# JiuTongBro/MultiView_Inpaint

Hardware: AMD Instinct MI355X
Metric: Mpix/s fwd+bwd @1.5M Gauss 1080p (higher is better)
Workload: dtype f32; 1 GPU; rasterizer-with-depth fwd+bwd, one 1920x1080 view per GPU per step, N=1500000 Gaussians, sh_degree 3 (BASELINE.json configs[2] size, SURVEY.md §8d scene); gaussians=1500000, visible=1312313, num_rendered_D=14779663, tiles=8160, tile_list_max=2266, parallelism=views x1

## Files before the change

### include/mvi_raster.h

```cpp
#ifndef MVI_RASTER_H
#define MVI_RASTER_H

#include <stddef.h>
#include <stdint.h>

#ifdef __cplusplus
extern "C" {
#endif

#define MVI_OK 0
#define MVI_EINVAL (-1)
#define MVI_EHIP (-2)
#define MVI_ENOMEM (-3)

#define MVI_TILE 16

typedef struct mvi_raster_settings {
    int32_t image_height;
    int32_t image_width;
    float tanfovx;
    float tanfovy;
    float scale_modifier;
    int32_t sh_degree;
    int32_t prefiltered;
    const float* bg;
    const float* viewmatrix;
    const float* projmatrix;
    const float* campos;
} mvi_raster_settings;

size_t mvi_raster_geom_bytes(int32_t P);
size_t mvi_raster_image_bytes(int32_t image_width, int32_t image_height);
size_t mvi_raster_binning_bytes(int64_t num_rendered, int32_t image_width, int32_t image_height);

int mvi_raster_forward_geom(const mvi_raster_settings* s, int32_t P, int32_t M,
                            const float* means3D, const float* shs, const float* colors_precomp,
                            const float* opacities, const float* scales, const float* rotations,
                            const float* cov3D_precomp, void* geom, size_t geom_bytes,
                            int32_t* radii, int64_t* num_rendered_host, void* stream);

int mvi_raster_forward_render(const mvi_raster_settings* s, int32_t P, int64_t num_rendered,
                              const int32_t* radii, void* geom, size_t geom_bytes, void* binning, size_t binning_bytes,
                              void* image, size_t image_bytes, float* out_color, float* out_depth,
                              void* stream);
int mvi_raster_forward_render_prepare(const mvi_raster_settings* s, int32_t P, int64_t num_rendered,
                                      const int32_t* radii, void* geom, size_t geom_bytes, void* binning,
                                      size_t binning_bytes, void* image, size_t image_bytes, float* out_color,
                                      float* out_depth, float* grad_rows_scratch, void* stream);

int mvi_raster_backward(const mvi_raster_settings* s, int32_t P, int32_t M, int64_t num_rendered,
                        const float* means3D, const float* shs, const float* colors_precomp,
                        const float* scales, const float* rotations, const float* cov3D_precomp,
                        const int32_t* radii, const void* geom, const void* binning,
                        const void* image, const float* dL_dout_color, float* dL_dmeans3D,
                        float* dL_dmeans2D, float* dL_dopacity, float* dL_dshs, float* dL_dcolors,
                        float* dL_dscales, float* dL_drotations, float* dL_dcov3D,
                        float* grad_rows_scratch, int32_t grad_rows_prezeroed, void* stream);

int mvi_raster_forward_geom_raw(const mvi_raster_settings* s, int32_t P, int32_t M, const float* xyz,
                                const float* features_dc, const float* features_rest, const float* raw_opacity,
                                const float* raw_scaling, const float* raw_rotation, void* geom, size_t geom_bytes,
                                int32_t* radii, int64_t* num_rendered_host, void* stream);
int mvi_raster_backward_raw(const mvi_raster_settings* s, int32_t P, int32_t M, int64_t num_rendered, const float* xyz,
                            const float* features_dc, const float* features_rest, const float* raw_opacity,
                            const float* raw_scaling, const float* raw_rotation, const int32_t* radii, const void* geom,
                            const void* binning, const void* image, const float* dL_dout_color, float* dL_dxyz,
                            float* dL_dmeans2D, float* dL_draw_opacity, float* dL_dfeatures_dc, float* dL_dfeatures_rest,
                            float* dL_draw_scaling, float* dL_draw_rotation, float* grad_rows_scratch, 
                            int32_t grad_rows_prezeroed, void* stream);
int mvi_raster_backward_raw_factor(const mvi_raster_settings* s, int32_t P, int32_t M, int64_t num_rendered, const float* xyz,
                                   const float* features_dc, const float* features_rest, const float* raw_opacity,
                                   const float* raw_scaling, const float* raw_rotation, const int32_t* radii, const void* geom,
                                   const void* binning, const void* image, const float* dL_dout_color, float* dL_dxyz,
                                   float* dL_dmeans2D, float* dL_draw_opacity, float* dL_dsh_color_factor,
                                   float* dL_draw_scaling, float* dL_draw_rotation, float* grad_rows_scratch,
                                   int32_t grad_rows_prezeroed, void* stream);

int mvi_raster_sh_backward_views(int32_t P, int32_t M, int32_t sh_degree, int32_t n_views, const float* means3D,
                                 const float* campos, int64_t campos_stride, const float* dL_dcolors,
                                 int64_t colors_view_stride, float* dL_dshs, void* stream);

int mvi_raster_mark_visible(int32_t P, const float* means3D, const float* viewmatrix,
                            const float* projmatrix, uint8_t* visible, void* stream);

int mvi_raster_backward_render(const mvi_raster_settings* s, int32_t P, int64_t num_rendered, const int32_t* radii,
                               const void* geom, const void* binning, const void* image, const float* dL_dout_color,
                               float* grad_rows_scratch, float* dL_dcolor_factor, int32_t sh_input,
                               int32_t grad_rows_prezeroed, void* stream);
int mvi_raster_backward_geom(const mvi_raster_settings* s, int32_t P, int32_t M, const float* means3D, const float* shs,
                             const float* colors_precomp, const float* scales, const float* rotations,
                             const float* cov3D_precomp, const int32_t* radii, const void* geom,
                             const float* grad_rows_scratch, float* dL_dmeans3D, float* dL_dmeans2D, float* dL_dopacity,
                             float* dL_dshs, float* dL_dcolors, float* dL_dscales, float* dL_drotations, float* dL_dcov3D,
                             void* stream);

int mvi_raster_backward_geom_range(const mvi_raster_settings* s, int32_t P, int32_t M, int32_t first, int32_t count,
                                   const float* means3D, const float* shs, const float* colors_precomp, const float* scales,
                                   const float* rotations, const float* cov3D_precomp, const int32_t* radii, const void* geom,
                                   const float* grad_rows_scratch, float* dL_dmeans3D, float* dL_dmeans2D, float* dL_dopacity,
                                   float* dL_dshs, float* dL_dcolors, float* dL_dscales, float* dL_drotations, float* dL_dcov3D,
                                   void* stream);

typedef struct mvi_raster_views {
    const float* depths;
    const float* means2D;
    const float* cov3D_a;
    const float* cov3D_b;
    const float* conic_opacity;
    const float* rgbd;
    const uint32_t* tiles_touched;
    const uint8_t* clamped;
    const void* tile_ids_sorted;
    const uint32_t* point_list;
    const uint32_t* ranges;
    const float* final_T;
    const uint32_t* n_contrib;
    int32_t tile_id_bytes;
    const uint8_t* grad_support;
} mvi_raster_views;
int mvi_raster_get_views(int32_t P, int64_t num_rendered, int32_t image_width, int32_t image_height,
                         const void* geom, const void* binning, const void* image,
                         mvi_raster_views* out);
int mvi_raster_materialize_tile_ids(int32_t P, int64_t num_rendered, int32_t image_width, int32_t image_height,
                                    void* binning, const void* image, void* stream);

#define MVI_RASTER_NSTAGES 8
int mvi_raster_timing_enable(int enable);
int mvi_raster_timing_enable_stages(uint32_t stage_mask);
int mvi_raster_timing_read(float* ms_sum_host, int32_t* calls_host);
const char* mvi_raster_stage_name(int stage);

int mvi_raster_color_mode(int deferred);
int mvi_raster_resolve_colors(const mvi_raster_settings* s, int32_t P, void* geom, size_t geom_bytes, void* stream);

int mvi_raster_binning_version(int version);
int mvi_raster_backward_mode(int dense);
int mvi_raster_dev_stamps(int pass, void* device_buffer);
int mvi_raster_dev_wave_sum9(const float* in, float* out, int n_waves, void* stream);

const char* mvi_raster_last_error(void);
const char* mvi_version(void);

#ifdef __cplusplus
}
#endif
#endif
```

### multiview_inpaint_amd/_lib.py

```python
import ctypes as C
import os
import re

_HERE = os.path.dirname(os.path.abspath(__file__))
LIB_PATH = os.environ.get("MVI_HIP_LIB") or os.path.join(_HERE, "csrc", "libmvi_hip.so")
LIB_OVERRIDDEN = bool(os.environ.get("MVI_HIP_LIB"))
if LIB_OVERRIDDEN:
    import sys as _sys
    _sys.stderr.write(f"[mvi] MVI_HIP_LIB is set: every kernel comes from {LIB_PATH}, not from the in-tree build\n")
INCLUDE_DIR = os.path.normpath(os.path.join(_HERE, "..", "include"))


class RasterSettings(C.Structure):
    _fields_ = [
        ("image_height", C.c_int32), ("image_width", C.c_int32),
        ("tanfovx", C.c_float), ("tanfovy", C.c_float), ("scale_modifier", C.c_float),
        ("sh_degree", C.c_int32), ("prefiltered", C.c_int32),
        ("bg", C.c_void_p), ("viewmatrix", C.c_void_p), ("projmatrix", C.c_void_p), ("campos", C.c_void_p),
    ]


class RasterViews(C.Structure):
    _fields_ = [(n, C.c_void_p) for n in (
        "depths", "means2D", "cov3D_a", "cov3D_b", "conic_opacity", "rgbd", "tiles_touched", "clamped",
        "tile_ids_sorted", "point_list", "ranges", "final_T", "n_contrib")] + [("tile_id_bytes", C.c_int32),
                                                                                   ("grad_support", C.c_void_p)]


class AdamGroup(C.Structure):
    _fields_ = [("param", C.c_void_p), ("grad", C.c_void_p), ("exp_avg", C.c_void_p), ("exp_avg_sq", C.c_void_p),
                ("n", C.c_int64), ("lr", C.c_float)]


class CompactTensor(C.Structure):
    _fields_ = [("in_", C.c_void_p), ("out", C.c_void_p), ("width", C.c_int32), ("packed_stride", C.c_int32)]


def declared_symbols():
    names = []
    for fn in sorted(os.listdir(INCLUDE_DIR)):
        if fn.endswith(".h"):
            src = open(os.path.join(INCLUDE_DIR, fn)).read()
            src = re.sub(r"/\*.*?\*/", "", src, flags=re.S)
            names += re.findall(r"\b(mvi_[a-z0-9_]+)\s*\(", src)
    return sorted(set(names))


def raster_source_digest():
    import hashlib
    h = hashlib.sha1()
    d = os.path.join(_HERE, "csrc")
    for fn in sorted(os.listdir(d)):
        if fn.startswith("raster_") and fn.endswith((".hip", ".h")):
            h.update(fn.encode())
            h.update(open(os.path.join(d, fn), "rb").read())
    return h.hexdigest()[:16]


_lib = None


def lib():
    global _lib
    if _lib is not None:
        return _lib
    if not os.path.exists(LIB_PATH):
        raise RuntimeError(
            f"{LIB_PATH} is missing: the HIP extension is not built. Run `python -m multiview_inpaint_amd.build` "
            "(hipcc --offload-arch=gfx950). There is no CPU or PyTorch fallback for this path.")
    L = C.CDLL(LIB_PATH)
    missing = [s for s in declared_symbols() if not hasattr(L, s)]
    if missing:
        raise RuntimeError(f"{LIB_PATH} does not export {missing}; rebuild it")
    vp, i32, i64, sz = C.c_void_p, C.c_int32, C.c_int64, C.c_size_t
    L.mvi_raster_last_error.restype = C.c_char_p
    L.mvi_version.restype = C.c_char_p
    L.mvi_raster_geom_bytes.restype = sz
    L.mvi_raster_geom_bytes.argtypes = [i32]
    L.mvi_raster_image_bytes.restype = sz
    L.mvi_raster_image_bytes.argtypes = [i32, i32]
    L.mvi_raster_binning_bytes.restype = sz
    L.mvi_raster_binning_bytes.argtypes = [i64, i32, i32]
    L.mvi_raster_forward_geom.restype = C.c_int
    L.mvi_raster_forward_geom.argtypes = [C.POINTER(RasterSettings), i32, i32] + [vp] * 7 + [vp, sz, vp, C.POINTER(i64), vp]
    L.mvi_raster_forward_render.restype = C.c_int
    L.mvi_raster_forward_render.argtypes = [C.POINTER(RasterSettings), i32, i64, vp, vp, sz, vp, sz, vp, sz, vp, vp, vp]
    L.mvi_raster_forward_render_prepare.restype = C.c_int
    L.mvi_raster_forward_render_prepare.argtypes = [C.POINTER(RasterSettings), i32, i64, vp, vp, sz, vp, sz, vp, sz, vp, vp, vp, vp]
    L.mvi_raster_backward.restype = C.c_int
    L.mvi_raster_backward.argtypes = [C.POINTER(RasterSettings), i32, i32, i64] + [vp] * 20 + [i32, vp]
    L.mvi_raster_backward_render.restype = C.c_int
    L.mvi_raster_backward_render.argtypes = [C.POINTER(RasterSettings), i32, i64] + [vp] * 7 + [i32, i32, vp]
    L.mvi_raster_backward_geom.restype = C.c_int
    L.mvi_raster_backward_geom.argtypes = [C.POINTER(RasterSettings), i32, i32] + [vp] * 18
    L.mvi_raster_backward_geom_range.restype = C.c_int
    L.mvi_raster_backward_geom_range.argtypes = [C.POINTER(RasterSettings), i32, i32, i32, i32] + [vp] * 18
    L.mvi_raster_forward_geom_raw.restype = C.c_int
    L.mvi_raster_forward_geom_raw.argtypes = [C.POINTER(RasterSettings), i32, i32] + [vp] * 6 + [vp, sz, vp, C.POINTER(i64), vp]
    L.mvi_raster_backward_raw.restype = C.c_int
    L.mvi_raster_backward_raw.argtypes = [C.POINTER(RasterSettings), i32, i32, i64] + [vp] * 19 + [i32, vp]
    L.mvi_raster_backward_raw_factor.restype = C.c_int
    L.mvi_raster_backward_raw_factor.argtypes = [C.POINTER(RasterSettings), i32, i32, i64] + [vp] * 18 + [i32, vp]
    L.mvi_raster_sh_backward_views.restype = C.c_int
    L.mvi_raster_sh_backward_views.argtypes = [i32, i32, i32, i32, vp, vp, i64, vp, i64, vp, vp]
    L.mvi_raster_mark_visible.restype = C.c_int
    L.mvi_raster_mark_visible.argtypes = [i32, vp, vp, vp, vp, vp]
    L.mvi_raster_get_views.restype = C.c_int
    L.mvi_raster_get_views.argtypes = [i32, i64, i32, i32, vp, vp, vp, C.POINTER(RasterViews)]
    L.mvi_raster_materialize_tile_ids.restype = C.c_int
    L.mvi_raster_materialize_tile_ids.argtypes = [i32, i64, i32, i32, vp, vp, vp]
    L.mvi_raster_timing_enable.restype = C.c_int
    L.mvi_raster_timing_enable.argtypes = [C.c_int]
    L.mvi_raster_timing_enable_stages.restype = C.c_int
    L.mvi_raster_timing_enable_stages.argtypes = [C.c_uint32]
    L.mvi_raster_timing_read.restype = C.c_int
    L.mvi_raster_timing_read.argtypes = [C.POINTER(C.c_float), C.POINTER(C.c_int32)]
    L.mvi_raster_stage_name.restype = C.c_char_p
    L.mvi_raster_stage_name.argtypes = [C.c_int]
    L.mvi_raster_binning_version.restype = C.c_int
    L.mvi_raster_binning_version.argtypes = [C.c_int]
    L.mvi_raster_backward_mode.restype = C.c_int
    L.mvi_raster_backward_mode.argtypes = [C.c_int]
    L.mvi_raster_color_mode.restype = C.c_int
    L.mvi_raster_color_mode.argtypes = [C.c_int]
    L.mvi_raster_resolve_colors.restype = C.c_int
    L.mvi_raster_resolve_colors.argtypes = [C.POINTER(RasterSettings), i32, vp, sz, vp]
    L.mvi_raster_dev_stamps.restype = C.c_int
    L.mvi_raster_dev_stamps.argtypes = [C.c_int, vp]
    L.mvi_raster_dev_wave_sum9.restype = C.c_int
    L.mvi_raster_dev_wave_sum9.argtypes = [vp, vp, C.c_int, vp]
    _bind_unet_ops(L)
    _bind_train_ops(L)
    _bind_box_region(L)
    _lib = L
    return L


def _bind_unet_ops(L):
    try:
        from . import _unet_ops_bind
    except ImportError:
        return
    _unet_ops_bind.bind(L)


def _bind_train_ops(L):
    vp, i32, sz, f32 = C.c_void_p, C.c_int32, C.c_size_t, C.c_float
    L.mvi_photometric_loss_workspace_bytes.restype = sz
    L.mvi_photometric_loss_workspace_bytes.argtypes = [i32, i32]
    L.mvi_photometric_loss.restype = C.c_int
    L.mvi_photometric_loss.argtypes = [vp, vp, vp, i32, i32, f32, f32, vp, vp, vp, sz, vp]
    L.mvi_photometric_loss_stats.restype = C.c_int
    L.mvi_photometric_loss_stats.argtypes = [vp, vp, vp, i32, i32, vp, vp, sz, vp]
    L.mvi_photometric_loss_grad2.restype = C.c_int
    L.mvi_photometric_loss_grad2.argtypes = [vp, vp, vp, i32, i32, vp, vp, vp, sz, vp]
    L.mvi_train_last_error.restype = C.c_char_p
    L.mvi_knn3_mean_dist2.restype = C.c_int
    L.mvi_knn3_mean_dist2.argtypes = [vp, i32, vp, vp]
    L.mvi_adam_step.restype = C.c_int
    L.mvi_adam_step.argtypes = [C.POINTER(AdamGroup), i32, C.c_double, C.c_double, C.c_double, i32, vp]
    L.mvi_compact_workspace_bytes.restype = sz
    L.mvi_compact_workspace_bytes.argtypes = [i32]
    L.mvi_compact_plan.restype = C.c_int
    L.mvi_compact_plan.argtypes = [vp, i32, vp, sz, vp, vp]
    L.mvi_compact_gather.restype = C.c_int
    L.mvi_compact_gather.argtypes = [C.POINTER(CompactTensor), i32, i32, C.c_uint32, vp, vp]
    L.mvi_support_pack_bits.restype = C.c_int
    L.mvi_support_pack_bits.argtypes = [vp, i32, vp, vp]
    L.mvi_support_union_bits.restype = C.c_int
    L.mvi_support_union_bits.argtypes = [vp, i32, i32, vp, vp]
    for f in (L.mvi_compact_gather_window, L.mvi_compact_scatter_window):
        f.restype = C.c_int
        f.argtypes = [C.POINTER(CompactTensor), i32, i32, vp, C.c_uint32, C.c_uint32, vp, vp]
    L.mvi_gaussian_activations.restype = C.c_int
    L.mvi_gaussian_activations.argtypes = [i32, i32] + [vp] * 10
    L.mvi_gaussian_activations_backward.restype = C.c_int
    L.mvi_gaussian_activations_backward.argtypes = [i32, i32] + [vp] * 13


def _bind_box_region(L):
    vp, i32, i64 = C.c_void_p, C.c_int32, C.c_int64
    L.mvi_box_region_last_error.restype = C.c_char_p
    L.mvi_mesh_intersect.restype = C.c_int
    L.mvi_mesh_intersect.argtypes = [vp, vp, i64, vp, i32, vp, vp, vp, vp, vp]
    L.mvi_mesh_points_inside.restype = C.c_int
    L.mvi_mesh_points_inside.argtypes = [vp, i64, vp, i32, vp, vp]
    L.mvi_mesh_view_masks.restype = C.c_int
    L.mvi_mesh_view_masks.argtypes = [vp, vp, vp, i32, i32, i32, vp, i32, vp, vp, vp, vp, vp, vp]


def check(rc, what):
    if rc != 0:
        msg = lib().mvi_raster_last_error().decode(errors="replace")
        if rc == -1:
            raise Exception(msg)
        raise RuntimeError(f"{what} failed ({rc}): {msg}")
```

### multiview_inpaint_amd/csrc/raster_api.hip

```cpp
#include <cstdio>
#include <cstdlib>
#include <cstring>
#include <mutex>
#include <vector>

#include "raster_common.h"

static thread_local char g_err[512] = "";
static int g_dense_backward = [] { const char* e = getenv("MVI_RASTER_DENSE_BACKWARD"); return (e && e[0] == '1') ? 1 : 0; }();
static int g_defer_colors = [] { const char* e = getenv("MVI_RASTER_EAGER_COLORS"); return (e && e[0] == '1') ? 0 : 1; }();
namespace {
struct SegmentHint { const void* geom; int32_t P; int64_t segments; uint64_t stamp; };
constexpr int kSegmentHints = 64;
SegmentHint g_seg_hints[kSegmentHints] = {};
uint64_t g_seg_clock = 0;
std::mutex g_seg_mutex;
void remember_segments(const void* geom, int32_t P, int64_t segments) {
    std::lock_guard<std::mutex> lock(g_seg_mutex);
    int slot = 0;
    for (int i = 0; i < kSegmentHints; ++i) {
        if (g_seg_hints[i].geom == geom) { slot = i; break; }
        if (g_seg_hints[i].stamp < g_seg_hints[slot].stamp) slot = i;
    }
    g_seg_hints[slot] = {geom, P, segments, ++g_seg_clock};
}
int64_t recall_segments(const void* geom, int32_t P) {
    std::lock_guard<std::mutex> lock(g_seg_mutex);
    for (int i = 0; i < kSegmentHints; ++i)
        if (g_seg_hints[i].geom == geom && g_seg_hints[i].stamp) return g_seg_hints[i].P == P ? g_seg_hints[i].segments : 0;
    return 0;
}
}

namespace {
struct Rec { int stage; hipEvent_t a, b; };
uint32_t g_timing_mask = 0;
std::vector<Rec> g_recs;
std::vector<hipEvent_t> g_pool;
hipEvent_t g_open[MVI_RASTER_NSTAGES];
hipEvent_t get_event() {
    if (!g_pool.empty()) { hipEvent_t e = g_pool.back(); g_pool.pop_back(); return e; }
    hipEvent_t e; (void)hipEventCreate(&e); return e;
}
}
namespace mvi {
void stage_begin(int stage, hipStream_t st) {
    if (!((g_timing_mask >> stage) & 1u)) return;
    g_open[stage] = get_event();
    (void)hipEventRecord(g_open[stage], st);
}
void stage_end(int stage, hipStream_t st) {
    if (!((g_timing_mask >> stage) & 1u)) return;
    hipEvent_t b = get_event();
    (void)hipEventRecord(b, st);
    g_recs.push_back({stage, g_open[stage], b});
}
}

static int fail(int code, const char* fmt, const char* a = "", long long b = 0, long long c = 0) {
    snprintf(g_err, sizeof(g_err), fmt, a, b, c);
    return code;
}
static int hip_fail(const char* where, hipError_t e) {
    snprintf(g_err, sizeof(g_err), "%s: %s", where, hipGetErrorString(e));
    return MVI_EHIP;
}

static int make_frame(const mvi_raster_settings* s, int P, int M, mvi::Frame& f) {
    if (!s) return fail(MVI_EINVAL, "settings is NULL%s");
    if (s->image_width < 0 || s->image_height < 0 || P < 0)
        return fail(MVI_EINVAL, "negative size%s (P=%lld, W=%lld)", "", P, s->image_width);
    if (s->sh_degree < 0 || s->sh_degree > 3) return fail(MVI_EINVAL, "sh_degree must be 0..3%s (got %lld)", "", s->sh_degree);
    if (!s->bg || !s->viewmatrix || !s->projmatrix || !s->campos)
        return fail(MVI_EINVAL, "bg/viewmatrix/projmatrix/campos must be device pointers%s");
    f.P = P; f.M = M; f.deg = s->sh_degree; f.W = s->image_width; f.H = s->image_height;
    f.gx = (f.W + mvi::kTile - 1) / mvi::kTile;
    f.gy = (f.H + mvi::kTile - 1) / mvi::kTile;
    f.tanfovx = s->tanfovx; f.tanfovy = s->tanfovy;
    f.fx = (float)f.W / (2.0f * s->tanfovx);
    f.fy = (float)f.H / (2.0f * s->tanfovy);
    f.scale_modifier = s->scale_modifier;
    f.view = s->viewmatrix; f.proj = s->projmatrix; f.campos = s->campos; f.bg = s->bg;
    f.bin_v2 = mvi::binning_v2_ok(f.gx, f.gy) ? 1 : 0;
    f.defer_colors = g_defer_colors;
    return MVI_OK;
}

extern "C" {

const char* mvi_raster_last_error(void) { return g_err; }

int mvi_raster_timing_enable(int enable) { g_timing_mask = enable ? (1u << MVI_RASTER_NSTAGES) - 1u : 0u; return MVI_OK; }
int mvi_raster_timing_enable_stages(uint32_t stage_mask) { g_timing_mask = stage_mask & ((1u << MVI_RASTER_NSTAGES) - 1u); return MVI_OK; }
int mvi_raster_timing_read(float* ms_sum, int32_t* calls) {
    if (!ms_sum || !calls) return fail(MVI_EINVAL, "NULL timing outputs%s");
    for (auto& r : g_recs) {
        hipError_t e = hipEventSynchronize(r.b);
        if (e != hipSuccess) return hip_fail("timing sync", e);
        float ms = 0.f;
        (void)hipEventElapsedTime(&ms, r.a, r.b);
        ms_sum[r.stage] += ms;
        calls[r.stage] += 1;
        g_pool.push_back(r.a);
        g_pool.push_back(r.b);
    }
    g_recs.clear();
    return MVI_OK;
}
const char* mvi_raster_stage_name(int i) {
    static const char* n[MVI_RASTER_NSTAGES] = {"preprocess_forward", "scan_block_sums", "duplicate_keys", "radix_sort",
                                                "tile_ranges", "render_forward", "render_backward", "preprocess_backward"};
    return (i >= 0 && i < MVI_RASTER_NSTAGES) ? n[i] : "";
}
int mvi_raster_dev_stamps(int pass, void* device_buffer) { mvi::set_dev_stamps(pass, device_buffer); return MVI_OK; }
int mvi_raster_dev_wave_sum9(const float* in, float* out, int n_waves, void* stream) {
    if (n_waves < 0 || (n_waves > 0 && (!in || !out))) return fail(MVI_EINVAL, "wave_sum9: NULL buffer or negative n_waves%s");
    if (mvi::launch_wave_sum9_probe(in, out, n_waves, (hipStream_t)stream)) return hip_fail("wave_sum9 probe", hipGetLastError());
    return MVI_OK;
}
int mvi_raster_backward_mode(int dense) {
    const int old = g_dense_backward;
    if (dense == 0 || dense == 1) g_dense_backward = dense;
    return old;
}
int mvi_raster_binning_version(int version) { return mvi::set_binning_version(version); }
int mvi_raster_color_mode(int deferred) {
    const int old = g_defer_colors;
    if (deferred == 0 || deferred == 1) g_defer_colors = deferred;
    return old;
}
int mvi_raster_resolve_colors(const mvi_raster_settings* s, int32_t P, void* geom, size_t geom_bytes, void* stream) {
    mvi::Frame f;
    if (int rc = make_frame(s, P, 0, f)) return rc;
    if (P == 0) return MVI_OK;
    if (!geom) return fail(MVI_EINVAL, "geom is NULL%s");
    mvi::GeomView g = mvi::carve_geom(geom, P);
    if (geom_bytes < g.bytes) return fail(MVI_ENOMEM, "geom scratch too small%s", "");
    if (mvi::launch_resolve_colors(f, g, (hipStream_t)stream)) return hip_fail("resolve_colors", hipGetLastError());
    return MVI_OK;
}
const char* mvi_version(void) { return "multiview_inpaint_amd 0.1.0 (gfx950)"; }

size_t mvi_raster_geom_bytes(int32_t P) { return mvi::carve_geom(nullptr, P).bytes; }
size_t mvi_raster_image_bytes(int32_t W, int32_t H) { return mvi::carve_image(nullptr, W, H).bytes; }
size_t mvi_raster_binning_bytes(int64_t D, int32_t W, int32_t H) { return mvi::carve_binning(nullptr, D, W, H).bytes; }

static int forward_geom_impl(const mvi_raster_settings* s, mvi::Frame& f, int32_t P, int32_t M, const float* means3D,
                             const float* shs, const float* colors_precomp, const float* opacities,
                             const float* scales, const float* rotations, const float* cov3D_precomp,
                             void* geom, size_t geom_bytes, int32_t* radii, int64_t* num_rendered_host,
                             void* stream);

int mvi_raster_forward_geom(const mvi_raster_settings* s, int32_t P, int32_t M, const float* means3D,
                            const float* shs, const float* colors_precomp, const float* opacities,
                            const float* scales, const float* rotations, const float* cov3D_precomp,
                            void* geom, size_t geom_bytes, int32_t* radii, int64_t* num_rendered_host,
                            void* stream) {
    mvi::Frame f;
    if (int rc = make_frame(s, P, M, f)) return rc;
    return forward_geom_impl(s, f, P, M, means3D, shs, colors_precomp, opacities, scales, rotations, cov3D_precomp, geom,
                             geom_bytes, radii, num_rendered_host, stream);
}

int mvi_raster_forward_geom_raw(const mvi_raster_settings* s, int32_t P, int32_t M, const float* xyz,
                                const float* features_dc, const float* features_rest, const float* raw_opacity,
                                const float* raw_scaling, const float* raw_rotation, void* geom, size_t geom_bytes,
                                int32_t* radii, int64_t* num_rendered_host, void* stream) {
    mvi::Frame f;
    if (int rc = make_frame(s, P, M, f)) return rc;
    if (P > 0 && (!features_dc || (M > 1 && !features_rest) || !raw_scaling || !raw_rotation))
        return fail(MVI_EINVAL, "NULL raw parameter pointer%s");
    f.raw = 1;
    f.shs_rest = features_rest;
    return forward_geom_impl(s, f, P, M, xyz, features_dc, nullptr, raw_opacity, raw_scaling, raw_rotation, nullptr, geom,
                             geom_bytes, radii, num_rendered_host, stream);
}

static int forward_geom_impl(const mvi_raster_settings* s, mvi::Frame& f, int32_t P, int32_t M, const float* means3D,
                             const float* shs, const float* colors_precomp, const float* opacities,
                             const float* scales, const float* rotations, const float* cov3D_precomp,
                             void* geom, size_t geom_bytes, int32_t* radii, int64_t* num_rendered_host,
                             void* stream) {
    if (!num_rendered_host) return fail(MVI_EINVAL, "num_rendered_host is NULL%s");
    *num_rendered_host = 0;
    if (P == 0) return MVI_OK;
    if ((shs == nullptr) == (colors_precomp == nullptr))
        return fail(MVI_EINVAL, "Please provide excatly one of either SHs or precomputed colors!%s");
    if (((scales == nullptr) || (rotations == nullptr)) == (cov3D_precomp == nullptr))
        return fail(MVI_EINVAL, "Please provide exactly one of either scale/rotation pair or precomputed 3D covariance!%s");
    if (!means3D || !opacities || !geom || !radii) return fail(MVI_EINVAL, "NULL means3D/opacities/geom/radii%s");
    if (shs && M < (s->sh_degree + 1) * (s->sh_degree + 1))
        return fail(MVI_EINVAL, "shs holds %s%lld coefficients per channel, sh_degree needs %lld", "", M,
                    (s->sh_degree + 1) * (s->sh_degree + 1));
    mvi::GeomView g = mvi::carve_geom(geom, P);
    if (geom_bytes < g.bytes) return fail(MVI_ENOMEM, "geom scratch too small%s: %lld < %lld", "", (long long)geom_bytes, (long long)g.bytes);
    hipStream_t st = (hipStream_t)stream;
    {
        mvi::StageTimer tm(mvi::kStPreFwd, st);
        if (mvi::launch_preprocess_forward(f, means3D, shs, colors_precomp, opacities, scales, rotations,
                                           cov3D_precomp, g, radii, st))
            return hip_fail("preprocess_forward", hipGetLastError());
    }
    struct Readback { unsigned long long* host = nullptr; unsigned long long* dev = nullptr; hipEvent_t ev = nullptr; };
    constexpr int kMaxDevices = 64;
    static thread_local Readback readbacks[kMaxDevices];
    hipError_t e;
    int device = -1;
    if ((e = hipGetDevice(&device)) != hipSuccess) return hip_fail("hipGetDevice", e);
    if (device < 0 || device >= kMaxDevices) return fail(MVI_EINVAL, "device index out of range%s: %lld", "", (long long)device);
    Readback& rb = readbacks[device];
    if (!rb.host) {
        unsigned long long* h = nullptr;
        if ((e = hipHostMalloc((void**)&h, 2 * sizeof(unsigned long long), hipHostMallocMapped | hipHostMallocPortable)) != hipSuccess) return hip_fail("hipHostMalloc", e);
        if ((e = hipHostGetDevicePointer((void**)&rb.dev, h, 0)) != hipSuccess) { (void)hipHostFree(h); return hip_fail("hipHostGetDevicePointer", e); }
        if ((e = hipEventCreateWithFlags(&rb.ev, hipEventDisableTiming)) != hipSuccess) { (void)hipHostFree(h); return hip_fail("hipEventCreate", e); }
        rb.host = h;
    }
    unsigned long long* const pinned = rb.host;
    unsigned long long* const pinned_dev = rb.dev;
    const hipEvent_t ev = rb.ev;
    {
        mvi::StageTimer tm(mvi::kStScan, st);
        if (f.bin_v2 ? mvi::launch_binning2_totals(g, P, pinned_dev, st) : mvi::launch_scan_block_sums(g, P, pinned_dev, st))
            return hip_fail("scan_block_sums", hipGetLastError());
    }
    if ((e = hipEventRecord(ev, st)) != hipSuccess) return hip_fail("event record", e);
    if (f.bin_v2 ? mvi::launch_binning2_level1(f, g, st) : mvi::launch_binning_level1(f, g, st))
        return hip_fail("binning level 1", hipGetLastError());
    e = hipEventSynchronize(ev);
    if (e != hipSuccess) return hip_fail("forward_geom sync", e);
    const unsigned long long total = *pinned;
    if (total > 0xFFFFFFFFull)
        return fail(MVI_EINVAL, "num_rendered exceeds the 32-bit pair offsets%s: %lld pairs", "", (long long)total);
    *num_rendered_host = (int64_t)total;
    if (f.bin_v2) remember_segments(geom, P, (int64_t)pinned[1]);
    return MVI_OK;
}

static int forward_render_impl(const mvi_raster_settings* s, int32_t P, int64_t D, const int32_t* radii,
                               void* geom, size_t geom_bytes, void* binning, size_t binning_bytes, void* image,
                               size_t image_bytes, float* out_color, float* out_depth, float* grad_rows_to_zero, void* stream) {
    mvi::Frame f;
    if (int rc = make_frame(s, P, 0, f)) return rc;
    if (!image || !out_color || !out_depth) return fail(MVI_EINVAL, "NULL image/out_color/out_depth%s");
    if (D < 0 || D > 0xFFFFFFFFll) return fail(MVI_EINVAL, "num_rendered out of range%s: %lld", "", D);
    if (D > 0 && (!geom || !binning || !radii)) return fail(MVI_EINVAL, "NULL geom/binning/radii with num_rendered > 0%s");
    mvi::GeomView g = mvi::carve_geom(geom, P);
    mvi::ImageView im = mvi::carve_image(image, f.W, f.H);
    mvi::BinningView b = mvi::carve_binning(binning, D, f.W, f.H);
    if (image_bytes < im.bytes) return fail(MVI_ENOMEM, "image scratch too small%s: %lld < %lld", "", (long long)image_bytes, (long long)im.bytes);
    if (D > 0 && binning_bytes < b.bytes) return fail(MVI_ENOMEM, "binning scratch too small%s: %lld < %lld", "", (long long)binning_bytes, (long long)b.bytes);
    if (D > 0 && geom_bytes < g.bytes) return fail(MVI_ENOMEM, "geom scratch too small%s", "");
    hipStream_t st = (hipStream_t)stream;
    const int64_t segments = recall_segments(geom, P);
    if (f.bin_v2 ? mvi::launch_binning2(f, g, b, im, D, segments, st) : mvi::launch_binning(f, g, b, im, D, st))
        return hip_fail("binning", hipGetLastError());
    {
        mvi::StageTimer tm(mvi::kStRenderFwd, st);
        if (mvi::launch_render_forward(f, g, b, im, D, out_color, out_depth, st, grad_rows_to_zero))
            return hip_fail("render_forward", hipGetLastError());
    }
    return MVI_OK;
}

int mvi_raster_forward_render(const mvi_raster_settings* s, int32_t P, int64_t D, const int32_t* radii,
                              void* geom, size_t geom_bytes, void* binning, size_t binning_bytes, void* image,
                              size_t image_bytes, float* out_color, float* out_depth, void* stream) {
    return forward_render_impl(s, P, D, radii, geom, geom_bytes, binning, binning_bytes, image, image_bytes, out_color, out_depth,
                               nullptr, stream);
}

int mvi_raster_forward_render_prepare(const mvi_raster_settings* s, int32_t P, int64_t D, const int32_t* radii,
                                      void* geom, size_t geom_bytes, void* binning, size_t binning_bytes, void* image,
                                      size_t image_bytes, float* out_color, float* out_depth, float* grad_rows_scratch,
                                      void* stream) {
    return forward_render_impl(s, P, D, radii, geom, geom_bytes, binning, binning_bytes, image, image_bytes, out_color, out_depth,
                               grad_rows_scratch, stream);
}

static int backward_render_impl(mvi::Frame& f, int32_t P, int64_t D, const int32_t* radii, const void* geom, const void* binning,
                                const void* image, const float* dL_dout_color, float* grad_rows, float* dL_dcolor_factor,
                                int sh_input, int rows_prezeroed, void* stream, const mvi::ZeroRegions* zero_outputs = nullptr);
static int backward_impl(mvi::Frame& f, int32_t P, int64_t D, const float* means3D, const float* shs,
                         const float* colors_precomp, const float* scales, const float* rotations,
                         const float* cov3D_precomp, const int32_t* radii, const void* geom, const void* binning,
                         const void* image, const float* dL_dout_color, float* dL_dmeans3D, float* dL_dmeans2D,
                         float* dL_dopacity, float* dL_dshs, float* dL_dcolors, float* dL_dscales, float* dL_drotations,
                         float* dL_dcov3D, float* dL_dconic_scratch, void* stream, mvi::RawBackwardExtra rawx);

int mvi_raster_backward(const mvi_raster_settings* s, int32_t P, int32_t M, int64_t D, const float* means3D,
                        const float* shs, const float* colors_precomp, const float* scales,
                        const float* rotations, const float* cov3D_precomp, const int32_t* radii,
                        const void* geom, const void* binning, const void* image,
                        const float* dL_dout_color, float* dL_dmeans3D, float* dL_dmeans2D,
                        float* dL_dopacity, float* dL_dshs, float* dL_dcolors, float* dL_dscales,
                        float* dL_drotations, float* dL_dcov3D, float* dL_dconic_scratch, int32_t grad_rows_prezeroed,
                        void* stream) {
    mvi::Frame f;
    if (int rc = make_frame(s, P, M, f)) return rc;
    mvi::RawBackwardExtra rawx;
    rawx.rows_prezeroed = grad_rows_prezeroed;
    return backward_impl(f, P, D, means3D, shs, colors_precomp, scales, rotations, cov3D_precomp, radii, geom, binning, image,
                         dL_dout_color, dL_dmeans3D, dL_dmeans2D, dL_dopacity, dL_dshs, dL_dcolors, dL_dscales, dL_drotations,
                         dL_dcov3D, dL_dconic_scratch, stream, rawx);
}

int mvi_raster_backward_raw(const mvi_raster_settings* s, int32_t P, int32_t M, int64_t D, const float* xyz,
                            const float* features_dc, const float* features_rest, const float* raw_opacity,
                            const float* raw_scaling, const float* raw_rotation, const int32_t* radii, const void* geom,
                            const void* binning, const void* image, const float* dL_dout_color, float* dL_dxyz,
                            float* dL_dmeans2D, float* dL_draw_opacity, float* dL_dfeatures_dc, float* dL_dfeatures_rest,
                            float* dL_draw_scaling, float* dL_draw_rotation, float* grad_rows_scratch,
                            int32_t grad_rows_prezeroed, void* stream) {
    mvi::Frame f;
    if (int rc = make_frame(s, P, M, f)) return rc;
    if (P > 0 && (!features_dc || (M > 1 && (!features_rest || !dL_dfeatures_rest)) || !raw_opacity || !dL_dfeatures_dc))
        return fail(MVI_EINVAL, "NULL raw parameter / gradient pointer%s");
    f.raw = 1;
    f.shs_rest = features_rest;
    mvi::RawBackwardExtra rawx;
    rawx.raw_opacity = raw_opacity;
    rawx.dL_dshs_rest = dL_dfeatures_rest;
    rawx.rows_prezeroed = grad_rows_prezeroed;
    return backward_impl(f, P, D, xyz, features_dc, nullptr, raw_scaling, raw_rotation, nullptr, radii, geom, binning, image,
                         dL_dout_color, dL_dxyz, dL_dmeans2D, dL_draw_opacity, dL_dfeatures_dc, nullptr, dL_draw_scaling,
                         dL_draw_rotation, nullptr, grad_rows_scratch, stream, rawx);
}

int mvi_raster_backward_raw_factor(const mvi_raster_settings* s, int32_t P, int32_t M, int64_t D, const float* xyz,
                                   const float* features_dc, const float* features_rest, const float* raw_opacity,
                                   const float* raw_scaling, const float* raw_rotation, const int32_t* radii, const void* geom,
                                   const void* binning, const void* image, const float* dL_dout_color, float* dL_dxyz,
                                   float* dL_dmeans2D, float* dL_draw_opacity, float* dL_dsh_color_factor, float* dL_draw_scaling,
                                   float* dL_draw_rotation, float* grad_rows_scratch, int32_t grad_rows_prezeroed, void* stream) {
    mvi::Frame f;
    if (int rc = make_frame(s, P, M, f)) return rc;
    if (P > 0 && (!features_dc || (M > 1 && !features_rest) || !raw_opacity || !dL_dsh_color_factor))
        return fail(MVI_EINVAL, "NULL raw parameter / colour factor pointer%s");
    f.raw = 1;
    f.shs_rest = features_rest;
    mvi::RawBackwardExtra rawx;
    rawx.raw_opacity = raw_opacity;
    rawx.dL_dshs_rest = nullptr;
    rawx.rows_prezeroed = grad_rows_prezeroed;
    return backward_impl(f, P, D, xyz, features_dc, nullptr, raw_scaling, raw_rotation, nullptr, radii, geom, binning, image,
                         dL_dout_color, dL_dxyz, dL_dmeans2D, dL_draw_opacity, nullptr, dL_dsh_color_factor, dL_draw_scaling,
                         dL_draw_rotation, nullptr, grad_rows_scratch, stream, rawx);
}

static int backward_impl(mvi::Frame& f, int32_t P, int64_t D, const float* means3D, const float* shs,
                         const float* colors_precomp, const float* scales, const float* rotations,
                         const float* cov3D_precomp, const int32_t* radii, const void* geom, const void* binning,
                         const void* image, const float* dL_dout_color, float* dL_dmeans3D, float* dL_dmeans2D,
                         float* dL_dopacity, float* dL_dshs, float* dL_dcolors, float* dL_dscales, float* dL_drotations,
                         float* dL_dcov3D, float* dL_dconic_scratch, void* stream, mvi::RawBackwardExtra rawx) {
    if (P == 0) return MVI_OK;
    if ((shs == nullptr) == (colors_precomp == nullptr))
        return fail(MVI_EINVAL, "Please provide excatly one of either SHs or precomputed colors!%s");
    if (((scales == nullptr) || (rotations == nullptr)) == (cov3D_precomp == nullptr))
        return fail(MVI_EINVAL, "Please provide exactly one of either scale/rotation pair or precomputed 3D covariance!%s");
    if (!means3D || !radii || !geom || !image || !dL_dout_color || !dL_dmeans3D || !dL_dmeans2D || !dL_dopacity ||
        !dL_dconic_scratch)
        return fail(MVI_EINVAL, "NULL required pointer in backward%s");
    if (shs && !dL_dshs && !dL_dcolors)
        return fail(MVI_EINVAL, "dL_dshs and dL_dcolors are both NULL but shs was a forward input%s");
    if (colors_precomp && !dL_dcolors) return fail(MVI_EINVAL, "dL_dcolors is NULL but colors_precomp was a forward input%s");
    if (cov3D_precomp ? !dL_dcov3D : (!dL_dscales || !dL_drotations))
        return fail(MVI_EINVAL, "missing covariance gradient output%s");
    if (D > 0 && !binning) return fail(MVI_EINVAL, "NULL binning with num_rendered > 0%s");
    const bool dense_bwd = g_dense_backward != 0;
    mvi::GeomView g = mvi::carve_geom(const_cast<void*>(geom), P);
    hipStream_t st = (hipStream_t)stream;
    if (!dense_bwd) {
        mvi::ZeroRegions z;
        const size_t n = (size_t)P, Mz = (size_t)f.M;
        z.add(dL_dmeans3D, 3 * n);
        z.add(dL_dmeans2D, 3 * n);
        z.add(dL_dopacity, n);
        if (dL_dcolors) z.add(dL_dcolors, 3 * n);
        if (shs && dL_dshs) z.add(dL_dshs, f.raw ? 3 * n : 3 * Mz * n);
        if (f.raw && rawx.dL_dshs_rest && Mz > 1) z.add(rawx.dL_dshs_rest, (3 * Mz - 3) * n);
        if (cov3D_precomp) z.add(dL_dcov3D, 6 * n);
        else { z.add(dL_dscales, 3 * n); z.add(dL_drotations, 4 * n); }
        if (z.overflow) return fail(MVI_EINVAL, "more gradient outputs than the render backward can zero on the side%s (kMaxZero)");
        if (int rc = backward_render_impl(f, P, D, radii, geom, binning, image, dL_dout_color, dL_dconic_scratch, nullptr, 0,
                                          rawx.rows_prezeroed, stream, &z)) return rc;
        mvi::StageTimer tm(mvi::kStPreBwd, st);
        if (mvi::launch_preprocess_backward_sparse(f, means3D, shs, scales, rotations, cov3D_precomp, g, dL_dconic_scratch,
                                                   dL_dmeans3D, dL_dmeans2D, dL_dopacity, dL_dcolors, dL_dshs, dL_dcov3D,
                                                   dL_dscales, dL_drotations, st, rawx))
            return hip_fail("preprocess_backward (sparse)", hipGetLastError());
        return MVI_OK;
    }
    if (int rc = backward_render_impl(f, P, D, radii, geom, binning, image, dL_dout_color, dL_dconic_scratch, nullptr, 0,
                                      rawx.rows_prezeroed, stream)) return rc;
    mvi::StageTimer tm(mvi::kStPreBwd, st);
    if (mvi::launch_preprocess_backward(f, means3D, shs, scales, rotations, cov3D_precomp, radii, g, dL_dconic_scratch,
                                        dL_dmeans3D, dL_dmeans2D, dL_dopacity, dL_dcolors,
                                        dL_dshs, dL_dcov3D, dL_dscales, dL_drotations, st, rawx))
        return hip_fail("preprocess_backward", hipGetLastError());
    return MVI_OK;
}

static int backward_render_impl(mvi::Frame& f, int32_t P, int64_t D, const int32_t* radii, const void* geom, const void* binning,
                                const void* image, const float* dL_dout_color, float* grad_rows, float* dL_dcolor_factor,
                                int sh_input, int rows_prezeroed, void* stream, const mvi::ZeroRegions* zero_outputs) {
    if (P == 0) return MVI_OK;
    if (!radii || !geom || !image || !dL_dout_color || !grad_rows) return fail(MVI_EINVAL, "NULL required pointer in backward%s");
    if (D > 0 && !binning) return fail(MVI_EINVAL, "NULL binning with num_rendered > 0%s");
    mvi::GeomView g = mvi::carve_geom(const_cast<void*>(geom), P);
    mvi::ImageView im = mvi::carve_image(const_cast<void*>(image), f.W, f.H);
    mvi::BinningView b = mvi::carve_binning(const_cast<void*>(binning), D, f.W, f.H);
    hipStream_t st = (hipStream_t)stream;
    if (!rows_prezeroed) {
        mvi::ZeroRegions z;
        z.add(grad_rows, (size_t)mvi::kGradRow * (size_t)P);
        z.add(g.touched, ((size_t)P + 15) / 16 * 4);
        z.add(g.touched_count, 1);
        if (mvi::launch_zero_regions(z, st)) return hip_fail("zero grad rows", hipGetLastError());
    }
    {
        mvi::StageTimer tm(mvi::kStRenderBwd, st);
        if (mvi::launch_render_backward(f, g, b, im, D, dL_dout_color, grad_rows, st, zero_outputs))
            return hip_fail("render_backward", hipGetLastError());
    }
    if (dL_dcolor_factor && mvi::launch_color_factors(P, radii, grad_rows, sh_input ? g.clamped : nullptr, dL_dcolor_factor, st))
        return hip_fail("color_factors", hipGetLastError());
    return MVI_OK;
}

int mvi_raster_backward_render(const mvi_raster_settings* s, int32_t P, int64_t D, const int32_t* radii, const void* geom,
                               const void* binning, const void* image, const float* dL_dout_color, float* grad_rows_scratch,
                               float* dL_dcolor_factor, int32_t sh_input, int32_t grad_rows_prezeroed, void* stream) {
    mvi::Frame f;
    if (int rc = make_frame(s, P, 0, f)) return rc;
    return backward_render_impl(f, P, D, radii, geom, binning, image, dL_dout_color, grad_rows_scratch, dL_dcolor_factor,
                                sh_input, grad_rows_prezeroed, stream);
}

static int backward_geom_range_impl(const mvi_raster_settings* s, int32_t P, int32_t M, int32_t first, int32_t count,
                                    const float* means3D, const float* shs, const float* colors_precomp, const float* scales,
                                    const float* rotations, const float* cov3D_precomp, const int32_t* radii, const void* geom,
                                    const float* grad_rows_scratch, float* dL_dmeans3D, float* dL_dmeans2D, float* dL_dopacity,
                                    float* dL_dshs, float* dL_dcolors, float* dL_dscales, float* dL_drotations, float* dL_dcov3D,
                                    void* stream) {
    mvi::Frame f;
    if (int rc = make_frame(s, P, M, f)) return rc;
    if (first < 0 || count < 0 || (int64_t)first + count > P || (first % 64) != 0)
        return fail(MVI_EINVAL, "backward range out of bounds or not 64-aligned%s: first %lld count %lld", "", (long long)first, (long long)count);
    if (P == 0 || count == 0) return MVI_OK;
    if ((shs == nullptr) == (colors_precomp == nullptr))
        return fail(MVI_EINVAL, "Please provide excatly one of either SHs or precomputed colors!%s");
    if (((scales == nullptr) || (rotations == nullptr)) == (cov3D_precomp == nullptr))
        return fail(MVI_EINVAL, "Please provide exactly one of either scale/rotation pair or precomputed 3D covariance!%s");
    if (!means3D || !radii || !geom || !grad_rows_scratch || !dL_dmeans3D || !dL_dmeans2D || !dL_dopacity)
        return fail(MVI_EINVAL, "NULL required pointer in backward%s");
    if (shs && !dL_dshs && !dL_dcolors)
        return fail(MVI_EINVAL, "dL_dshs and dL_dcolors are both NULL but shs was a forward input%s");
    if (colors_precomp && !dL_dcolors) return fail(MVI_EINVAL, "dL_dcolors is NULL but colors_precomp was a forward input%s");
    if (cov3D_precomp ? !dL_dcov3D : (!dL_dscales || !dL_drotations))
        return fail(MVI_EINVAL, "missing covariance gradient output%s");
    mvi::GeomView g = mvi::carve_geom(const_cast<void*>(geom), P);
    const size_t o = (size_t)first;
    g.depths += o; g.xy += o; g.cov_a += o; g.cov_b += o; g.conic_opacity += o; g.rgbd += o; g.tiles_touched += o; g.rect += o;
    g.clamped += o;
    auto at = [o](auto* p, size_t w) { return p ? p + o * w : p; };
    f.P = count;
    hipStream_t st = (hipStream_t)stream;
    mvi::StageTimer tm(mvi::kStPreBwd, st);
    if (mvi::launch_preprocess_backward(f, at(means3D, 3), at(shs, 3 * (size_t)M), at(scales, 3), at(rotations, 4), at(cov3D_precomp, 6),
                                        at(radii, 1), g, at(grad_rows_scratch, 16), at(dL_dmeans3D, 3), at(dL_dmeans2D, 3),
                                        at(dL_dopacity, 1), at(dL_dcolors, 3), at(dL_dshs, 3 * (size_t)M), at(dL_dcov3D, 6),
                                        at(dL_dscales, 3), at(dL_drotations, 4), st, mvi::RawBackwardExtra()))
        return hip_fail("preprocess_backward", hipGetLastError());
    return MVI_OK;
}

int mvi_raster_backward_geom(const mvi_raster_settings* s, int32_t P, int32_t M, const float* means3D, const float* shs,
                             const float* colors_precomp, const float* scales, const float* rotations,
                             const float* cov3D_precomp, const int32_t* radii, const void* geom,
                             const float* grad_rows_scratch, float* dL_dmeans3D, float* dL_dmeans2D, float* dL_dopacity,
                             float* dL_dshs, float* dL_dcolors, float* dL_dscales, float* dL_drotations, float* dL_dcov3D,
                             void* stream) {
    return backward_geom_range_impl(s, P, M, 0, P, means3D, shs, colors_precomp, scales, rotations, cov3D_precomp, radii, geom,
                                    grad_rows_scratch, dL_dmeans3D, dL_dmeans2D, dL_dopacity, dL_dshs, dL_dcolors, dL_dscales,
                                    dL_drotations, dL_dcov3D, stream);
}

int mvi_raster_backward_geom_range(const mvi_raster_settings* s, int32_t P, int32_t M, int32_t first, int32_t count,
                                   const float* means3D, const float* shs, const float* colors_precomp, const float* scales,
                                   const float* rotations, const float* cov3D_precomp, const int32_t* radii, const void* geom,
                                   const float* grad_rows_scratch, float* dL_dmeans3D, float* dL_dmeans2D, float* dL_dopacity,
                                   float* dL_dshs, float* dL_dcolors, float* dL_dscales, float* dL_drotations, float* dL_dcov3D,
                                   void* stream) {
    return backward_geom_range_impl(s, P, M, first, count, means3D, shs, colors_precomp, scales, rotations, cov3D_precomp, radii,
                                    geom, grad_rows_scratch, dL_dmeans3D, dL_dmeans2D, dL_dopacity, dL_dshs, dL_dcolors, dL_dscales,
                                    dL_drotations, dL_dcov3D, stream);
}

int mvi_raster_sh_backward_views(int32_t P, int32_t M, int32_t sh_degree, int32_t n_views, const float* means3D,
                                 const float* campos, int64_t campos_stride, const float* dL_dcolors,
                                 int64_t colors_view_stride, float* dL_dshs, void* stream) {
    if (P < 0 || M < 1 || M > 16 || sh_degree < 0 || (sh_degree + 1) * (sh_degree + 1) > M || n_views < 1)
        return fail(MVI_EINVAL, "bad shape for sh_backward_views (need 1 <= (deg+1)^2 <= M <= 16, n_views >= 1)%s");
    if (P == 0) return MVI_OK;
    if (!means3D || !campos || !dL_dcolors || !dL_dshs) return fail(MVI_EINVAL, "NULL pointer in sh_backward_views%s");
    if (campos_stride < 3 || colors_view_stride < 3 * (int64_t)P)
        return fail(MVI_EINVAL, "sh_backward_views: campos_stride must be >= 3 and colors_view_stride >= 3 P%s");
    if (mvi::launch_sh_backward_views(P, M, sh_degree, n_views, means3D, campos, campos_stride, dL_dcolors,
                                      colors_view_stride, dL_dshs, (hipStream_t)stream))
        return hip_fail("sh_backward_views", hipGetLastError());
    return MVI_OK;
}

int mvi_raster_mark_visible(int32_t P, const float* means3D, const float* viewmatrix, const float* projmatrix,
                            uint8_t* visible, void* stream) {
    if (P < 0 || (P > 0 && (!means3D || !viewmatrix || !visible))) return fail(MVI_EINVAL, "bad arguments to mark_visible%s");
    if (mvi::launch_mark_visible(P, means3D, viewmatrix, visible, (hipStream_t)stream)) return hip_fail("mark_visible", hipGetLastError());
    return MVI_OK;
}

int mvi_raster_get_views(int32_t P, int64_t D, int32_t W, int32_t H, const void* geom, const void* binning,
                         const void* image, mvi_raster_views* out) {
    if (!out) return fail(MVI_EINVAL, "views is NULL%s");
    memset(out, 0, sizeof(*out));
    if (geom) {
        mvi::GeomView g = mvi::carve_geom(const_cast<void*>(geom), P);
        out->depths = g.depths; out->means2D = reinterpret_cast<const float*>(g.xy);
        out->cov3D_a = reinterpret_cast<const float*>(g.cov_a); out->cov3D_b = reinterpret_cast<const float*>(g.cov_b);
        out->conic_opacity = reinterpret_cast<const float*>(g.conic_opacity); out->rgbd = reinterpret_cast<const float*>(g.rgbd);
        out->tiles_touched = g.tiles_touched; out->clamped = g.clamped;
        out->grad_support = g.touched;
    }
    if (binning) {
        mvi::BinningView b = mvi::carve_binning(const_cast<void*>(binning), D, W, H);
        int fin = b.passes & 1;
        out->tile_ids_sorted = b.keys[fin]; out->point_list = b.vals[fin];
        out->tile_id_bytes = b.key_bytes;
    }
    if (image) {
        mvi::ImageView im = mvi::carve_image(const_cast<void*>(image), W, H);
        out->ranges = im.ranges; out->final_T = im.final_T; out->n_contrib = im.n_contrib;
    }
    return MVI_OK;
}

int mvi_raster_materialize_tile_ids(int32_t P, int64_t D, int32_t W, int32_t H, void* binning, const void* image, void* stream) {
    if (P < 0 || D < 0 || W < 0 || H < 0) return fail(MVI_EINVAL, "negative size in materialize_tile_ids%s");
    if (P == 0 || D == 0) return MVI_OK;
    if (!binning || !image) return fail(MVI_EINVAL, "NULL scratch in materialize_tile_ids%s");
    const int tiles = ((W + mvi::kTile - 1) / mvi::kTile) * ((H + mvi::kTile - 1) / mvi::kTile);
    mvi::BinningView b = mvi::carve_binning(binning, D, W, H);
    mvi::ImageView im = mvi::carve_image(const_cast<void*>(image), W, H);
    if (mvi::launch_tile_ids_from_ranges(tiles, b, im, D, (hipStream_t)stream)) return hip_fail("materialize_tile_ids", hipGetLastError());
    return MVI_OK;
}

}
```

### multiview_inpaint_amd/csrc/raster_common.h

```cpp
#pragma once
#include <hip/hip_runtime.h>
#include <stdint.h>
#include <stddef.h>
#include <type_traits>

#include "../../include/mvi_raster.h"

namespace mvi {

constexpr int kTile = MVI_TILE;
constexpr int kBlock = 256;
constexpr int kPB = 64;
constexpr float kNearZ = 0.2f;
constexpr float kLowpass = 0.3f;
constexpr float kFrustumClamp = 1.3f;
constexpr float kLambdaFloor = 0.1f;
constexpr float kAlphaMax = 0.99f;
constexpr float kAlphaMin = 1.0f / 255.0f;
constexpr float kTEps = 0.0001f;
constexpr float kDepthSentinel = 15.0f;

constexpr int kSortItems = 8;
constexpr int kSortWavesP = 4;
constexpr int kSortWavesD = 8;
constexpr int kCountTiles = 4;
__host__ __device__ inline int sort_blocks(int64_t n, int waves) {
    const int tile = 512 * waves;
    int b = (int)((n + tile - 1) / tile);
    return (b + kCountTiles - 1) / kCountTiles * kCountTiles;
}

struct Frame {
    int P, M, deg, W, H, gx, gy;
    float tanfovx, tanfovy, fx, fy, scale_modifier;
    const float* view;
    const float* proj;
    const float* campos;
    const float* bg;
    const float* shs_rest = nullptr;
    int raw = 0;
    int bin_v2 = 0;
    int defer_colors = 0;
};

constexpr int kDsThreads = 256;
constexpr int kDsItems = 8;
constexpr int kDsTile = kDsThreads * kDsItems;
constexpr int kDsSuper = 16;
constexpr int kExThreads = 512;
constexpr int kExItems = 4;
constexpr int kExChunk = kExThreads * kExItems;
constexpr int kEx2Items = 3;
constexpr int kEx2Chunk = kExThreads * kEx2Items;
constexpr int kEx2SmallNB = 80;
constexpr int kEx2SmallCap = 7168;
bool binning_v2_enabled();
void set_dev_stamps(int pass, void* buf);
int set_binning_version(int v);
inline bool binning_v2_ok(int gx, int gy) { return gx <= 256 && gy <= 256 && binning_v2_enabled(); }

struct ColorSource {
    const float* means3D;
    const float* shs;
    const float* shs_rest;
    int32_t M, deg, raw;
    int32_t deferred;
    int32_t vec16;
};

struct GeomView {
    float* depths;
    float2* xy;
    float4* cov_a;
    float2* cov_b;
    float4* conic_opacity;
    float4* rgbd;
    uint32_t* tiles_touched;
    uint2* rect;
    uint8_t* clamped;
    uint8_t* front;
    struct ColorSource* color_src;
    uint32_t* touched_list;
    uint32_t* touched_count;
    uint8_t* touched;
    uint32_t* block_sums;
    uint32_t* block_offsets;
    uint32_t* dkeys[2];
    uint32_t* dvals[2];
    uint32_t* dhist;
    uint32_t* dtot;
    uint32_t* perm_sums;
    uint32_t* perm_offsets;
    uint2* rect_sorted;
    uint32_t* col_table;
    uint32_t* col_tot;
    uint32_t* seg_sums;
    uint32_t* chunk_first;
    uint32_t* col_start;
    uint32_t* arrivals;
    uint32_t* ds_table;
    uint32_t* ds_super[2];
    int nds, nsuper;
    int nblk1;
    int nsortP;
    size_t bytes;
};
struct ImageView {
    uint32_t* ranges;
    float* final_T;
    uint32_t* n_contrib;
    size_t bytes;
};
struct BinningView {
    void* keys[2];
    int key_bytes;
    uint32_t* vals[2];
    uint32_t* block_hist;
    uint32_t* digit_tot;
    int nsort;
    int passes;
    int key_bits;
    int v2;
    uint32_t* col_rel;
    size_t bytes;
};

inline size_t align256(size_t x) { return (x + 255) & ~size_t(255); }

inline GeomView carve_geom(void* base, int P) {
    GeomView g;
    char* p = (char*)base;
    size_t o = 0;
    size_t n = (size_t)(P > 0 ? P : 1);
    int nblk = (int)((n + kBlock - 1) / kBlock);
    auto take = [&](size_t b) { char* r = p ? p + o : nullptr; o += align256(b); return r; };
    g.depths = (float*)take(4 * n);
    g.xy = (float2*)take(8 * n);
    g.cov_a = (float4*)take(16 * n);
    g.cov_b = (float2*)take(8 * n);
    g.conic_opacity = (float4*)take(16 * n);
    g.rgbd = (float4*)take(16 * n);
    g.tiles_touched = (uint32_t*)take(4 * n);
    g.rect = (uint2*)take(8 * n);
    g.clamped = (uint8_t*)take(n);
    g.touched = (uint8_t*)take(n);
    g.touched_list = (uint32_t*)take(4 * n);
    g.touched_count = (uint32_t*)take(4);
    g.front = (uint8_t*)take(n);
    g.color_src = (ColorSource*)take(sizeof(ColorSource));
    const size_t npre = (n + kPB - 1) / kPB;
    g.block_sums = (uint32_t*)take(4 * npre);
    g.block_offsets = (uint32_t*)take(4 * (npre + 1));
    g.nsortP = sort_blocks(n, kSortWavesP);
    for (int i = 0; i < 2; ++i) { g.dkeys[i] = (uint32_t*)take(4 * n); g.dvals[i] = (uint32_t*)take(4 * n); }
    g.dhist = (uint32_t*)take(4 * 256 * (size_t)g.nsortP);
    g.dtot = (uint32_t*)take(4 * 256);
    g.perm_sums = (uint32_t*)take(4 * (size_t)nblk);
    g.perm_offsets = (uint32_t*)take(4 * (size_t)(nblk + 1));
    g.rect_sorted = (uint2*)take(8 * n);
    g.nblk1 = (int)((n + kExChunk - 1) / kExChunk);
    g.col_table = (uint32_t*)take(4 * 256 * (size_t)g.nblk1);
    g.col_tot = (uint32_t*)take(4 * 256);
    g.seg_sums = (uint32_t*)take(4 * npre);
    g.chunk_first = (uint32_t*)take(4 * 257);
    g.col_start = (uint32_t*)take(4 * 257);
    g.arrivals = (uint32_t*)take(4);
    g.nds = (int)((n + kDsTile - 1) / kDsTile);
    g.nsuper = (g.nds + kDsSuper - 1) / kDsSuper;
    g.ds_table = (uint32_t*)take(4 * 256 * (size_t)g.nds);
    g.ds_super[0] = (uint32_t*)take(4 * 256 * (size_t)g.nsuper);
    g.ds_super[1] = (uint32_t*)take(4 * 256 * (size_t)g.nsuper);
    g.bytes = o;
    return g;
}
inline ImageView carve_image(void* base, int W, int H) {
    ImageView v;
    char* p = (char*)base;
    size_t o = 0;
    size_t tiles = (size_t)((W + kTile - 1) / kTile) * ((H + kTile - 1) / kTile);
    size_t px = (size_t)W * H;
    auto take = [&](size_t b) { char* r = p ? p + o : nullptr; o += align256(b); return r; };
    v.ranges = (uint32_t*)take(8 * (tiles ? tiles : 1));
    v.final_T = (float*)take(4 * (px ? px : 1));
    v.n_contrib = (uint32_t*)take(4 * (px ? px : 1));
    v.bytes = o;
    return v;
}
inline int tile_bits(int W, int H) {
    unsigned tiles = (unsigned)(((W + kTile - 1) / kTile) * ((H + kTile - 1) / kTile));
    int b = 0;
    while ((1u << b) < tiles && b < 31) ++b;
    return b > 0 ? b : 1;
}
inline BinningView carve_binning(void* base, int64_t D, int W, int H) {
    BinningView v;
    char* p = (char*)base;
    size_t o = 0;
    size_t n = (size_t)(D > 0 ? D : 1);
    v.nsort = sort_blocks(n, kSortWavesD);
    v.key_bits = tile_bits(W, H);
    v.passes = (v.key_bits + 7) / 8;
    auto take = [&](size_t b) { char* r = p ? p + o : nullptr; o += align256(b); return r; };
    const unsigned tiles = (unsigned)(((W + kTile - 1) / kTile) * ((H + kTile - 1) / kTile));
    v.key_bytes = tiles <= 65536u ? 2 : 4;
    const int gx = (W + kTile - 1) / kTile, gy = (H + kTile - 1) / kTile;
    v.v2 = binning_v2_ok(gx, gy) ? 1 : 0;
    v.col_rel = nullptr;
    if (v.v2) {
        v.nsort = (int)((n / kEx2Chunk + (size_t)gx + 1 + 3) / 4 * 4);
        v.passes = 1;
        v.key_bytes = 2;
    }
    v.keys[0] = take((size_t)v.key_bytes * n);
    v.keys[1] = take((size_t)v.key_bytes * n);
    v.vals[0] = (uint32_t*)take(4 * n);
    v.vals[1] = (uint32_t*)take(4 * n);
    v.block_hist = (uint32_t*)take(4 * 256 * (size_t)v.nsort);
    v.digit_tot = (uint32_t*)take(4 * 256);
    if (v.v2) v.col_rel = (uint32_t*)take(4 * (size_t)gy * (size_t)(gx + 1));
    v.bytes = o;
    return v;
}

__device__ __forceinline__ float affine3(float m0, float m1, float m2, float m3, float x, float y, float z) {
    return __builtin_fmaf(m2, z, __builtin_fmaf(m1, y, __builtin_fmaf(m0, x, m3)));
}
__device__ __forceinline__ float dot3(float a0, float a1, float a2, float b0, float b1, float b2) {
#pragma clang fp contract(off)
    return __builtin_fmaf(a2, b2, __builtin_fmaf(a1, b1, a0 * b0));
}

__device__ __forceinline__ void tile_rect(float px, float py, int radius, int gx, int gy, int& x0,
                                          int& y0, int& x1, int& y1) {
#pragma clang fp contract(off)
    x0 = min(gx, max(0, (int)((px - (float)radius) / (float)kTile)));
    y0 = min(gy, max(0, (int)((py - (float)radius) / (float)kTile)));
    x1 = min(gx, max(0, (int)((px + (float)radius + (float)(kTile - 1)) / (float)kTile)));
    y1 = min(gy, max(0, (int)((py + (float)radius + (float)(kTile - 1)) / (float)kTile)));
}

__device__ constexpr float SH_C0 = 0.28209479177387814f;
__device__ constexpr float SH_C1 = 0.4886025119029199f;
__device__ constexpr float SH_C2[5] = {1.0925484305920792f, -1.0925484305920792f, 0.31539156525252005f,
                                       -1.0925484305920792f, 0.5462742152960396f};
__device__ constexpr float SH_C3[7] = {-0.5900435899266435f, 2.890611442640554f, -0.4570457994644658f,
                                       0.3731763325901154f,  -0.4570457994644658f, 1.445305721320277f,
                                       -0.5900435899266435f};

__device__ __forceinline__ void sh_basis(int deg, float x, float y, float z, float* b) {
#pragma clang fp contract(off)
    b[0] = SH_C0;
    if (deg > 0) {
        b[1] = -SH_C1 * y;
        b[2] = SH_C1 * z;
        b[3] = -SH_C1 * x;
        if (deg > 1) {
            float xx = x * x, yy = y * y, zz = z * z, xy = x * y, yz = y * z, xz = x * z;
            b[4] = SH_C2[0] * xy;
            b[5] = SH_C2[1] * yz;
            b[6] = SH_C2[2] * (2.0f * zz - xx - yy);
            b[7] = SH_C2[3] * xz;
            b[8] = SH_C2[4] * (xx - yy);
            if (deg > 2) {
                b[9] = SH_C3[0] * y * (3.0f * xx - yy);
                b[10] = SH_C3[1] * xy * z;
                b[11] = SH_C3[2] * y * (4.0f * zz - xx - yy);
                b[12] = SH_C3[3] * z * (2.0f * zz - 3.0f * xx - 3.0f * yy);
                b[13] = SH_C3[4] * x * (4.0f * zz - xx - yy);
                b[14] = SH_C3[5] * z * (xx - yy);
                b[15] = SH_C3[6] * x * (xx - 3.0f * yy);
            }
        }
    }
}

__device__ __forceinline__ void sh_direction(float px, float py, float pz, const float* __restrict__ campos, float& dx, float& dy,
                                             float& dz) {
#pragma clang fp contract(off)
    dx = px - campos[0]; dy = py - campos[1]; dz = pz - campos[2];
    const float len = sqrtf(dot3(dx, dy, dz, dx, dy, dz));
    dx = dx / len; dy = dy / len; dz = dz / len;
}
__device__ __forceinline__ void sh_first(float b0, float c0, float c1, float c2, float& r0, float& r1, float& r2) {
#pragma clang fp contract(off)
    r0 = b0 * c0; r1 = b0 * c1; r2 = b0 * c2;
}
__device__ __forceinline__ void sh_next(float bk, float c0, float c1, float c2, float& r0, float& r1, float& r2) {
    r0 = __builtin_fmaf(bk, c0, r0); r1 = __builtin_fmaf(bk, c1, r1); r2 = __builtin_fmaf(bk, c2, r2);
}
__device__ __forceinline__ void sh_finish(float& r0, float& r1, float& r2, uint32_t& clamp_bits) {
#pragma clang fp contract(off)
    r0 += 0.5f; r1 += 0.5f; r2 += 0.5f;
    clamp_bits = (r0 < 0.0f ? 1u : 0u) | (r1 < 0.0f ? 2u : 0u) | (r2 < 0.0f ? 4u : 0u);
    r0 = fmaxf(r0, 0.0f); r1 = fmaxf(r1, 0.0f); r2 = fmaxf(r2, 0.0f);
}
template <typename Coef>
__device__ __forceinline__ void sh_rgb(int deg, float px, float py, float pz, const float* __restrict__ campos, Coef coef,
                                       float& r0, float& r1, float& r2, uint32_t& clamp_bits) {
    float dx, dy, dz, bs[16];
    sh_direction(px, py, pz, campos, dx, dy, dz);
    sh_basis(deg, dx, dy, dz, bs);
    const int nb = (deg + 1) * (deg + 1);
    sh_first(bs[0], coef(0, 0), coef(0, 1), coef(0, 2), r0, r1, r2);
    for (int k = 1; k < nb; ++k) sh_next(bs[k], coef(k, 0), coef(k, 1), coef(k, 2), r0, r1, r2);
    sh_finish(r0, r1, r2, clamp_bits);
}

template <int DEG>
__device__ __forceinline__ float4 resolve_color_deg(const ColorSource& cs, const float* __restrict__ campos, uint32_t id, float depth,
                                                    float4* rgbd, uint8_t* clamped) {
    constexpr int NB = (DEG + 1) * (DEG + 1), KC = 8;
    const size_t si = (size_t)id;
    const float* row = cs.raw ? cs.shs_rest + si * (size_t)(3 * cs.M - 3) - 3 : cs.shs + si * (size_t)(3 * cs.M);
    float dx, dy, dz, bs[NB > 1 ? NB : 1], r0 = 0.f, r1 = 0.f, r2 = 0.f;
    sh_direction(cs.means3D[3 * si], cs.means3D[3 * si + 1], cs.means3D[3 * si + 2], campos, dx, dy, dz);
    {
        float b16[16];
        sh_basis(DEG, dx, dy, dz, b16);
#pragma unroll
        for (int k = 0; k < NB; ++k) bs[k] = b16[k];
    }
#pragma unroll
    for (int k0 = 0; k0 < NB; k0 += KC) {
        constexpr int kMaxF = 3 * KC;
        const int nk = NB - k0 < KC ? NB - k0 : KC;
        float v[kMaxF];
        if (!cs.raw && cs.vec16) {
#pragma unroll
            for (int q = 0; q < kMaxF / 4; ++q) {
                if (4 * q < 3 * nk) {
                    const float4 t = reinterpret_cast<const float4*>(row + 3 * k0)[q];
                    v[4 * q] = t.x; v[4 * q + 1] = t.y; v[4 * q + 2] = t.z; v[4 * q + 3] = t.w;
                }
            }
        } else {
#pragma unroll
            for (int j = 0; j < kMaxF; ++j)
                if (j < 3 * nk) v[j] = (cs.raw && k0 == 0 && j < 3) ? cs.shs[3 * si + j] : row[3 * k0 + j];
        }
#pragma unroll
        for (int k = 0; k < KC; ++k) {
            if (k < nk) {
                if (k0 + k == 0) sh_first(bs[0], v[0], v[1], v[2], r0, r1, r2);
                else sh_next(bs[k0 + k], v[3 * k], v[3 * k + 1], v[3 * k + 2], r0, r1, r2);
            }
        }
        __builtin_amdgcn_sched_barrier(0);
    }
    uint32_t bits;
    sh_finish(r0, r1, r2, bits);
    const float4 out = make_float4(r0, r1, r2, depth);
    rgbd[si] = out;
    clamped[si] = (uint8_t)bits;
    return out;
}
__device__ __forceinline__ float4 resolve_color(const ColorSource& cs, const float* __restrict__ campos, uint32_t id, float depth,
                                             float4* rgbd, uint8_t* clamped) {
    switch (cs.deg) {
        case 0: return resolve_color_deg<0>(cs, campos, id, depth, rgbd, clamped);
        case 1: return resolve_color_deg<1>(cs, campos, id, depth, rgbd, clamped);
        case 2: return resolve_color_deg<2>(cs, campos, id, depth, rgbd, clamped);
        default: return resolve_color_deg<3>(cs, campos, id, depth, rgbd, clamped);
    }
}
__device__ __forceinline__ float4 resolve_color_small(const ColorSource& cs, const float* __restrict__ campos, uint32_t id,
                                                      float depth, float4* rgbd, uint8_t* clamped) {
    const size_t si = (size_t)id;
    const float* c0p = cs.shs + (cs.raw ? 3 * si : si * (size_t)(3 * cs.M));
    const float* row = cs.raw ? cs.shs_rest + si * (size_t)(3 * cs.M - 3) - 3 : cs.shs + si * (size_t)(3 * cs.M);
    float dx, dy, dz, bs[16], r0, r1, r2;
    sh_direction(cs.means3D[3 * si], cs.means3D[3 * si + 1], cs.means3D[3 * si + 2], campos, dx, dy, dz);
    sh_basis(cs.deg, dx, dy, dz, bs);
    struct F3 { float a, b, c; };
    {
        const F3 t = *reinterpret_cast<const F3*>(c0p);
        sh_first(bs[0], t.a, t.b, t.c, r0, r1, r2);
    }
    auto band = [&](auto first_c, auto last_c) __attribute__((always_inline)) {
        constexpr int kFirst = decltype(first_c)::value, kLast = decltype(last_c)::value;
        F3 t[kLast - kFirst + 1];
#pragma unroll
        for (int k = kFirst; k <= kLast; ++k) t[k - kFirst] = *reinterpret_cast<const F3*>(row + 3 * k);
#pragma unroll
        for (int k = kFirst; k <= kLast; ++k) sh_next(bs[k], t[k - kFirst].a, t[k - kFirst].b, t[k - kFirst].c, r0, r1, r2);
    };
    using std::integral_constant;
    if (cs.deg > 0) {
        band(integral_constant<int, 1>{}, integral_constant<int, 3>{});
        if (cs.deg > 1) {
            band(integral_constant<int, 4>{}, integral_constant<int, 6>{});
            __builtin_amdgcn_sched_barrier(0);
            band(integral_constant<int, 7>{}, integral_constant<int, 8>{});
            if (cs.deg > 2) {
                band(integral_constant<int, 9>{}, integral_constant<int, 12>{});
                __builtin_amdgcn_sched_barrier(0);
                band(integral_constant<int, 13>{}, integral_constant<int, 15>{});
            }
        }
    }
    uint32_t bits;
    sh_finish(r0, r1, r2, bits);
    const float4 out = make_float4(r0, r1, r2, depth);
    rgbd[si] = out;
    clamped[si] = (uint8_t)bits;
    return out;
}
__device__ __forceinline__ bool color_pending(float4 cd) { return cd.x < 0.0f || cd.y < 0.0f || cd.z < 0.0f; }

template <int CTRL, int ROW_MASK>
__device__ __forceinline__ float dpp_add(float v) {
    int t = __builtin_amdgcn_update_dpp(0, __float_as_int(v), CTRL, ROW_MASK, 0xf, true);
    return v + __int_as_float(t);
}
__device__ __forceinline__ float wave_sum_to_lane63(float v) {
    v = dpp_add<0xb1, 0xf>(v);
    v = dpp_add<0x4e, 0xf>(v);
    v = dpp_add<0x114, 0xf>(v);
    v = dpp_add<0x118, 0xf>(v);
    v = dpp_add<0x142, 0xa>(v);
    v = dpp_add<0x143, 0xc>(v);
    return v;
}
__device__ __forceinline__ float row_sum_to_lane15(float v) {
    v = dpp_add<0xb1, 0xf>(v);
    v = dpp_add<0x4e, 0xf>(v);
    v = dpp_add<0x114, 0xf>(v);
    v = dpp_add<0x118, 0xf>(v);
    return v;
}
__device__ __forceinline__ uint32_t wave_sum_u32(uint32_t v) {
    for (int o = 32; o > 0; o >>= 1) v += __shfl_xor(v, o);
    return v;
}

enum Stage { kStPreFwd = 0, kStScan, kStDup, kStSort, kStRanges, kStRenderFwd, kStRenderBwd, kStPreBwd };
void stage_begin(int stage, hipStream_t st);
void stage_end(int stage, hipStream_t st);
struct StageTimer {
    int stage; hipStream_t st;
    StageTimer(int s, hipStream_t q) : stage(s), st(q) { stage_begin(stage, st); }
    ~StageTimer() { stage_end(stage, st); }
};

constexpr int kMaxZero = 10;
struct ZeroRegions {
    float* head[kMaxZero];
    uint4* body[kMaxZero];
    float* tail[kMaxZero];
    uint32_t n_head[kMaxZero], n_body[kMaxZero], n_tail[kMaxZero];
    int n = 0;
    bool overflow = false;
    void add(void* ptr, size_t words) {
        if (!ptr || !words) return;
        if (n >= kMaxZero) { overflow = true; return; }
        float* p = (float*)ptr;
        const size_t mis = ((uintptr_t)p & 15u) / 4u;
        size_t h = mis ? 4 - mis : 0;
        if (h > words) h = words;
        const size_t b = (words - h) / 4, t = words - h - 4 * b;
        head[n] = p; n_head[n] = (uint32_t)h;
        body[n] = (uint4*)(p + h); n_body[n] = (uint32_t)b;
        tail[n] = p + h + 4 * b; n_tail[n] = (uint32_t)t;
        ++n;
    }
};
__device__ __forceinline__ void zero_share(const ZeroRegions& z, int tid, int nthreads) {
    for (int r = 0; r < z.n; ++r) {
        const uint32_t per = (z.n_body[r] + gridDim.x - 1) / gridDim.x;
        const size_t z0 = (size_t)blockIdx.x * per;
        typedef uint32_t zero_u32x4 __attribute__((ext_vector_type(4)));
        const zero_u32x4 zz = {0u, 0u, 0u, 0u};
        for (uint32_t i = tid; i < per && z0 + i < z.n_body[r]; i += nthreads)
            asm volatile("global_store_dwordx4 %0, %1, off sc1" ::"v"(z.body[r] + z0 + i), "v"(zz) : "memory");
        if (blockIdx.x == 0) {
            if (tid < (int)z.n_head[r]) z.head[r][tid] = 0.f;
            if (tid < (int)z.n_tail[r]) z.tail[r][tid] = 0.f;
        }
    }
}
int launch_zero_regions(const ZeroRegions& z, hipStream_t st);

int launch_preprocess_forward(const Frame& f, const float* means3D, const float* shs,
                              const float* colors_precomp, const float* opacities, const float* scales,
                              const float* rotations, const float* cov3D_precomp, GeomView g,
                              int32_t* radii, hipStream_t st);
struct RawBackwardExtra { const float* raw_opacity = nullptr; float* dL_dshs_rest = nullptr; int rows_prezeroed = 0; };
int launch_preprocess_backward_sparse(const Frame& f, const float* means3D, const float* shs, const float* scales,
                                      const float* rotations, const float* cov3D_precomp, GeomView g, const float* grad_rows,
                                      float* dL_dmeans3D, float* dL_dmeans2D, float* dL_dopacity, float* dL_dcolors,
                                      float* dL_dshs, float* dL_dcov3D, float* dL_dscales, float* dL_drots, hipStream_t st,
                                      RawBackwardExtra raw);
int launch_preprocess_backward(const Frame& f, const float* means3D, const float* shs,
                               const float* scales, const float* rotations, const float* cov3D_precomp,
                               const int32_t* radii, GeomView g, const float* grad_rows, float* dL_dmeans3D,
                               float* dL_dmeans2D, float* dL_dopacity, float* dL_dcolors, float* dL_dshs,
                               float* dL_dcov3D, float* dL_dscales, float* dL_drots, hipStream_t st,
                               RawBackwardExtra raw = RawBackwardExtra());
int launch_scan_block_sums(GeomView g, int P, unsigned long long* total_host_devptr, hipStream_t st);
int launch_binning_level1(const Frame& f, GeomView g, hipStream_t st);
int launch_binning(const Frame& f, GeomView g, BinningView b, ImageView im, int64_t D, hipStream_t st);
int launch_zero_fill(void* p, size_t bytes, hipStream_t st);
int launch_tile_ids_from_ranges(int tiles, BinningView b, ImageView im, int64_t D, hipStream_t st);
int launch_binning2_totals(GeomView g, int P, unsigned long long* totals_host_devptr, hipStream_t st);
int launch_binning2_level1(const Frame& f, GeomView g, hipStream_t st);
int launch_binning2(const Frame& f, GeomView g, BinningView b, ImageView im, int64_t D, int64_t segments, hipStream_t st);
int launch_render_forward(const Frame& f, GeomView g, BinningView b, ImageView im, int64_t D,
                          float* out_color, float* out_depth, hipStream_t st, float* zero_rows = nullptr);
int launch_resolve_colors(const Frame& f, GeomView g, hipStream_t st);
int launch_render_backward(const Frame& f, GeomView g, BinningView b, ImageView im, int64_t D,
                           const float* dL_dpix, float* grad_rows, hipStream_t st, const ZeroRegions* zero = nullptr);
int launch_wave_sum9_probe(const float* in, float* out, int n_waves, hipStream_t st);
constexpr int kGradRow = 16;
int launch_sh_backward_views(int P, int M, int deg, int n_views, const float* means3D, const float* campos,
                             int64_t campos_stride, const float* gcol, int64_t gcol_stride, float* dL_dshs, hipStream_t st);
int launch_mark_visible(int P, const float* means3D, const float* view, uint8_t* visible, hipStream_t st);
int launch_color_factors(int P, const int32_t* radii, const float* grad_rows, const uint8_t* clamped, float* out, hipStream_t st);

}
```

### multiview_inpaint_amd/csrc/raster_preprocess.hip

```cpp
#include "raster_common.h"
#include "raster_scan.h"

namespace mvi {

__device__ __forceinline__ void stage_in(const float* __restrict__ src, float* lds, int n_rec, int rec, int stride) {
    const int total = n_rec * rec;
    if ((rec & 3) == 0) {
        constexpr int kStageUnroll = 6;
        const int rv = rec >> 2;
        const int nvec = total >> 2;
        const float4* s4 = reinterpret_cast<const float4*>(src);
        for (int v0 = threadIdx.x; v0 < nvec; v0 += kPB * kStageUnroll) {
            float4 x[kStageUnroll];
#pragma unroll
            for (int u = 0; u < kStageUnroll; ++u) {
                const int v = v0 + u * kPB;
                if (v < nvec) x[u] = s4[v];
            }
#pragma unroll
            for (int u = 0; u < kStageUnroll; ++u) {
                const int v = v0 + u * kPB;
                if (v < nvec) {
                    float* d = lds + (v / rv) * stride + (v % rv) * 4;
                    d[0] = x[u].x; d[1] = x[u].y; d[2] = x[u].z; d[3] = x[u].w;
                }
            }
        }
    } else {
        for (int e = threadIdx.x; e < total; e += kPB) lds[(e / rec) * stride + (e % rec)] = src[e];
    }
}
__device__ __forceinline__ void stage_out(float* __restrict__ dst, const float* lds, int n_rec, int rec, int stride) {
    const int total = n_rec * rec;
    if ((rec & 3) == 0) {
        const int rv = rec >> 2;
        float4* d4 = reinterpret_cast<float4*>(dst);
        for (int v = threadIdx.x; v < (total >> 2); v += kPB) {
            const float* s_ = lds + (v / rv) * stride + (v % rv) * 4;
            d4[v] = make_float4(s_[0], s_[1], s_[2], s_[3]);
        }
    } else {
        for (int e = threadIdx.x; e < total; e += kPB) dst[e] = lds[(e / rec) * stride + (e % rec)];
    }
}
__device__ __forceinline__ void stage_in_split(const float* __restrict__ src, float* lds, int n_rec, int rec, int stride) {
    const int total = n_rec * rec, nvec = total >> 2;
    const float inv = 1.0f / (float)rec;
    auto put = [&](int e, float v) {
        const int r = (int)(((float)e + 0.5f) * inv);
        lds[r * stride + (e - r * rec)] = v;
    };
    constexpr int kU = 6;
    const float4* s4 = reinterpret_cast<const float4*>(src);
    for (int v0 = threadIdx.x; v0 < nvec; v0 += kPB * kU) {
        float4 x[kU];
#pragma unroll
        for (int u = 0; u < kU; ++u) { const int v = v0 + u * kPB; if (v < nvec) x[u] = s4[v]; }
#pragma unroll
        for (int u = 0; u < kU; ++u) {
            const int v = v0 + u * kPB;
            if (v < nvec) { put(4 * v, x[u].x); put(4 * v + 1, x[u].y); put(4 * v + 2, x[u].z); put(4 * v + 3, x[u].w); }
        }
    }
    for (int e = 4 * nvec + threadIdx.x; e < total; e += kPB) put(e, src[e]);
}
__device__ __forceinline__ void stage_out_split(float* __restrict__ dst, const float* lds, int n_rec, int rec, int stride) {
    const int total = n_rec * rec, nvec = total >> 2;
    const float inv = 1.0f / (float)rec;
    auto get = [&](int e) {
        const int r = (int)(((float)e + 0.5f) * inv);
        return lds[r * stride + (e - r * rec)];
    };
    float4* d4 = reinterpret_cast<float4*>(dst);
    for (int v = threadIdx.x; v < nvec; v += kPB) d4[v] = make_float4(get(4 * v), get(4 * v + 1), get(4 * v + 2), get(4 * v + 3));
    for (int e = 4 * nvec + threadIdx.x; e < total; e += kPB) dst[e] = get(e);
}
__device__ __forceinline__ void stage_sh_in(const Frame& f, const float* shs, float* s_sh, int blk0, int n_rec, int stride) {
    if (!f.raw) { stage_in(shs + (size_t)blk0 * f.M * 3, s_sh, n_rec, 3 * f.M, stride); return; }
    stage_in(shs + (size_t)blk0 * 3, s_sh, n_rec, 3, stride);
    if (f.M > 1) stage_in_split(f.shs_rest + (size_t)blk0 * (3 * f.M - 3), s_sh + 3, n_rec, 3 * f.M - 3, stride);
}
__device__ __forceinline__ float sigmoidf_(float x) { return 1.0f / (1.0f + expf(-x)); }

__host__ __device__ inline int sh_stride(int M) { return 3 * M + 1 - ((3 * M) & 1); }


__device__ __forceinline__ void quat_to_rot(float r, float x, float y, float z, float R[3][3]) {
#pragma clang fp contract(off)
    R[0][0] = __builtin_fmaf(-2.0f, __builtin_fmaf(y, y, z * z), 1.0f);
    R[0][1] = 2.0f * __builtin_fmaf(x, y, -(r * z));
    R[0][2] = 2.0f * __builtin_fmaf(x, z, r * y);
    R[1][0] = 2.0f * __builtin_fmaf(x, y, r * z);
    R[1][1] = __builtin_fmaf(-2.0f, __builtin_fmaf(x, x, z * z), 1.0f);
    R[1][2] = 2.0f * __builtin_fmaf(y, z, -(r * x));
    R[2][0] = 2.0f * __builtin_fmaf(x, z, -(r * y));
    R[2][1] = 2.0f * __builtin_fmaf(y, z, r * x);
    R[2][2] = __builtin_fmaf(-2.0f, __builtin_fmaf(x, x, y * y), 1.0f);
}

struct Ewa {
    float Tm[2][3];
    float tx, ty, tz, xmul, ymul;
};

__device__ __forceinline__ void ewa_setup(const Frame& f, const float* V, float vx, float vy, float vz, Ewa& e) {
#pragma clang fp contract(off)
    float limx = kFrustumClamp * f.tanfovx, limy = kFrustumClamp * f.tanfovy;
    float txtz = vx / vz, tytz = vy / vz;
    e.xmul = (txtz < -limx || txtz > limx) ? 0.0f : 1.0f;
    e.ymul = (tytz < -limy || tytz > limy) ? 0.0f : 1.0f;
    e.tx = fminf(limx, fmaxf(-limx, txtz)) * vz;
    e.ty = fminf(limy, fmaxf(-limy, tytz)) * vz;
    e.tz = vz;
    float J00 = f.fx / vz, J02 = -(f.fx * e.tx) / (vz * vz);
    float J11 = f.fy / vz, J12 = -(f.fy * e.ty) / (vz * vz);
#pragma unroll
    for (int j = 0; j < 3; ++j) {
        e.Tm[0][j] = __builtin_fmaf(J02, V[2 + 4 * j], J00 * V[0 + 4 * j]);
        e.Tm[1][j] = __builtin_fmaf(J12, V[2 + 4 * j], J11 * V[1 + 4 * j]);
    }
}

__device__ __forceinline__ void cov2d_from_cov3d(const Ewa& e, const float* c6, float& a, float& b, float& c) {
#pragma clang fp contract(off)
    float S[3][3] = {{c6[0], c6[1], c6[2]}, {c6[1], c6[3], c6[4]}, {c6[2], c6[4], c6[5]}};
    float t0[3], t1[3];
#pragma unroll
    for (int j = 0; j < 3; ++j) {
        t0[j] = dot3(e.Tm[0][0], e.Tm[0][1], e.Tm[0][2], S[0][j], S[1][j], S[2][j]);
        t1[j] = dot3(e.Tm[1][0], e.Tm[1][1], e.Tm[1][2], S[0][j], S[1][j], S[2][j]);
    }
    a = dot3(t0[0], t0[1], t0[2], e.Tm[0][0], e.Tm[0][1], e.Tm[0][2]) + kLowpass;
    b = dot3(t0[0], t0[1], t0[2], e.Tm[1][0], e.Tm[1][1], e.Tm[1][2]);
    c = dot3(t1[0], t1[1], t1[2], e.Tm[1][0], e.Tm[1][1], e.Tm[1][2]) + kLowpass;
}

__global__ __launch_bounds__(kPB) void preprocess_forward_kernel(
    Frame f, const float* __restrict__ means3D, const float* __restrict__ shs,
    const float* __restrict__ colors_precomp, const float* __restrict__ opacities,
    const float* __restrict__ scales, const float* __restrict__ rotations,
    const float* __restrict__ cov3D_precomp, GeomView g, int32_t* __restrict__ radii, int defer_colors, int sh_vec16) {
#pragma clang fp contract(off)
    extern __shared__ __attribute__((aligned(16))) float s_dyn[];
    __shared__ uint32_t s_sum;
    const int tid = threadIdx.x;
    const int blk0 = blockIdx.x * kPB;
    const int i = blk0 + tid;
    const int n_rec = min(kPB, f.P - blk0);
    const bool eager_sh = shs && !defer_colors;
    const int shs_w = eager_sh ? sh_stride(f.M) : 0;
    float* s_sh = s_dyn;
    float* s_mean = s_dyn + (size_t)kPB * shs_w;
    float* s_scale = s_mean + 3 * kPB;
    if (tid == 0) s_sum = 0;
    if (blockIdx.x == 0 && tid == 0) {
        ColorSource cs;
        cs.means3D = means3D; cs.shs = shs; cs.shs_rest = f.shs_rest; cs.M = f.M; cs.deg = f.deg; cs.raw = f.raw;
        cs.deferred = (shs && defer_colors) ? 1 : 0; cs.vec16 = sh_vec16;
        *g.color_src = cs;
    }
    if (eager_sh) stage_sh_in(f, shs, s_sh, blk0, n_rec, shs_w);
    stage_in(means3D + (size_t)blk0 * 3, s_mean, n_rec, 3, 3);
    if (scales) stage_in(scales + (size_t)blk0 * 3, s_scale, n_rec, 3, 3);
    float4 q = make_float4(1.f, 0.f, 0.f, 0.f);
    float opac = 0.f;
    if (i < f.P) {
        if (!cov3D_precomp) q = *reinterpret_cast<const float4*>(rotations + 4 * (size_t)i);
        opac = opacities[i];
        if (f.raw) {
            const float nq = fmaxf(sqrtf(q.x * q.x + q.y * q.y + q.z * q.z + q.w * q.w), 1e-12f);
            q = make_float4(q.x / nq, q.y / nq, q.z / nq, q.w / nq);
            opac = sigmoidf_(opac);
        }
    }
    __syncthreads();
    float V[16], PM[16];
#pragma unroll
    for (int k = 0; k < 16; ++k) { V[k] = f.view[k]; PM[k] = f.proj[k]; }

    uint32_t touched = 0;
    uint2 rect = make_uint2(0u, 0u);
    float depth_key = 0.0f;
    int rad_out = 0;
    if (i < f.P) {
        do {
            float px = s_mean[3 * tid], py = s_mean[3 * tid + 1], pz = s_mean[3 * tid + 2];
            float vx = affine3(V[0], V[4], V[8], V[12], px, py, pz);
            float vy = affine3(V[1], V[5], V[9], V[13], px, py, pz);
            float vz = affine3(V[2], V[6], V[10], V[14], px, py, pz);
            if (vz <= kNearZ) break;
            float hx = affine3(PM[0], PM[4], PM[8], PM[12], px, py, pz);
            float hy = affine3(PM[1], PM[5], PM[9], PM[13], px, py, pz);
            float hw = affine3(PM[3], PM[7], PM[11], PM[15], px, py, pz);
            float pw = 1.0f / (hw + 0.0000001f);
            float ndx = hx * pw, ndy = hy * pw;

            float c6[6];
            if (cov3D_precomp) {
#pragma unroll
                for (int k = 0; k < 6; ++k) c6[k] = cov3D_precomp[6 * (size_t)i + k];
            } else {
                float R[3][3], Mx[3][3];
                quat_to_rot(q.x, q.y, q.z, q.w, R);
                float sa[3] = {s_scale[3 * tid], s_scale[3 * tid + 1], s_scale[3 * tid + 2]};
                if (f.raw) { sa[0] = expf(sa[0]); sa[1] = expf(sa[1]); sa[2] = expf(sa[2]); }
                float s[3] = {f.scale_modifier * sa[0], f.scale_modifier * sa[1], f.scale_modifier * sa[2]};
#pragma unroll
                for (int r = 0; r < 3; ++r)
#pragma unroll
                    for (int j = 0; j < 3; ++j) Mx[r][j] = R[r][j] * s[j];
                c6[0] = dot3(Mx[0][0], Mx[0][1], Mx[0][2], Mx[0][0], Mx[0][1], Mx[0][2]);
                c6[1] = dot3(Mx[0][0], Mx[0][1], Mx[0][2], Mx[1][0], Mx[1][1], Mx[1][2]);
                c6[2] = dot3(Mx[0][0], Mx[0][1], Mx[0][2], Mx[2][0], Mx[2][1], Mx[2][2]);
                c6[3] = dot3(Mx[1][0], Mx[1][1], Mx[1][2], Mx[1][0], Mx[1][1], Mx[1][2]);
                c6[4] = dot3(Mx[1][0], Mx[1][1], Mx[1][2], Mx[2][0], Mx[2][1], Mx[2][2]);
                c6[5] = dot3(Mx[2][0], Mx[2][1], Mx[2][2], Mx[2][0], Mx[2][1], Mx[2][2]);
            }
            g.cov_a[i] = make_float4(c6[0], c6[1], c6[2], c6[3]);
            g.cov_b[i] = make_float2(c6[4], c6[5]);

            Ewa e;
            ewa_setup(f, V, vx, vy, vz, e);
            float a, b, c;
            cov2d_from_cov3d(e, c6, a, b, c);
            float det = __builtin_fmaf(a, c, -(b * b));
            if (det == 0.0f) break;
            float det_inv = 1.0f / det;
            float mid = 0.5f * (a + c);
            float disc = sqrtf(fmaxf(kLambdaFloor, __builtin_fmaf(mid, mid, -det)));
            float lam1 = mid + disc, lam2 = mid - disc;
            int rad = (int)ceilf(3.0f * sqrtf(fmaxf(lam1, lam2)));
            if (rad <= 0) break;
            float pix_x = ((ndx + 1.0f) * (float)f.W - 1.0f) * 0.5f;
            float pix_y = ((ndy + 1.0f) * (float)f.H - 1.0f) * 0.5f;
            int x0, y0, x1, y1;
            tile_rect(pix_x, pix_y, rad, f.gx, f.gy, x0, y0, x1, y1);
            if ((x1 - x0) * (y1 - y0) == 0) break;

            float r0, r1, r2;
            uint32_t clamp_bits = 0;
            if (colors_precomp) {
                r0 = colors_precomp[3 * (size_t)i]; r1 = colors_precomp[3 * (size_t)i + 1]; r2 = colors_precomp[3 * (size_t)i + 2];
            } else if (eager_sh) {
                const float* sh = s_sh + (size_t)tid * shs_w;
                sh_rgb(f.deg, px, py, pz, f.campos, [&](int k, int c) { return sh[3 * k + c]; }, r0, r1, r2, clamp_bits);
            } else {
                r0 = r1 = r2 = -1.0f;
            }
            g.clamped[i] = (uint8_t)clamp_bits;
            g.rgbd[i] = make_float4(r0, r1, r2, vz);
            g.depths[i] = vz;
            depth_key = vz;
            g.xy[i] = make_float2(pix_x, pix_y);
            g.conic_opacity[i] = make_float4(c * det_inv, -b * det_inv, a * det_inv, opac);
            rad_out = rad;
            touched = (uint32_t)((x1 - x0) * (y1 - y0));
            rect = make_uint2((uint32_t)x0 | ((uint32_t)y0 << 16), (uint32_t)(x1 - x0) | ((uint32_t)(y1 - y0) << 16));
        } while (false);
        radii[i] = rad_out;
        if (defer_colors) g.front[i] = 0;
        g.tiles_touched[i] = touched;
        g.rect[i] = rect;
        g.dkeys[0][i] = touched ? __float_as_uint(depth_key) : 0xFFFFFFFFu;
        if (!f.bin_v2) g.dvals[0][i] = (uint32_t)i;
    }
    uint32_t wsum = wave_sum_u32(touched);
    if ((tid & 63) == 0 && wsum) atomicAdd(&s_sum, wsum);
    if (f.bin_v2) {
        const uint32_t segs = wave_sum_u32(touched ? (rect.y & 0xFFFFu) : 0u);
        static_assert(kPB == 64, "one wave per block");
        if (tid == 0) g.seg_sums[blockIdx.x] = segs;
    }
    __syncthreads();
    if (tid == 0) g.block_sums[blockIdx.x] = s_sum;
}

int launch_preprocess_forward(const Frame& f, const float* means3D, const float* shs,
                              const float* colors_precomp, const float* opacities, const float* scales,
                              const float* rotations, const float* cov3D_precomp, GeomView g,
                              int32_t* radii, hipStream_t st) {
    if (f.P <= 0) return 0;
    int nblk = (f.P + kPB - 1) / kPB;
    const int defer = (shs && f.defer_colors) ? 1 : 0;
    const int vec16 = (shs && !f.raw && (f.M & 3) == 0 && ((uintptr_t)shs & 15u) == 0) ? 1 : 0;
    size_t lds = sizeof(float) * ((size_t)kPB * ((shs && !defer) ? sh_stride(f.M) : 0) + 6 * kPB);
    if (lds > 64 * 1024 &&
        hipFuncSetAttribute((const void*)preprocess_forward_kernel, hipFuncAttributeMaxDynamicSharedMemorySize, (int)lds) != hipSuccess)
        return MVI_EHIP;
    hipLaunchKernelGGL(preprocess_forward_kernel, dim3(nblk), dim3(kPB), lds, st, f, means3D, shs,
                       colors_precomp, opacities, scales, rotations, cov3D_precomp, g, radii, defer, vec16);
    return hipGetLastError() == hipSuccess ? 0 : MVI_EHIP;
}

__device__ __forceinline__ void sh_basis_grad(int deg, float x, float y, float z, float* dx, float* dy, float* dz) {
#pragma unroll
    for (int k = 0; k < 16; ++k) dx[k] = dy[k] = dz[k] = 0.0f;
    if (deg > 0) {
        dy[1] = -SH_C1; dz[2] = SH_C1; dx[3] = -SH_C1;
        if (deg > 1) {
            float xx = x * x, yy = y * y, zz = z * z;
            dx[4] = SH_C2[0] * y; dy[4] = SH_C2[0] * x;
            dy[5] = SH_C2[1] * z; dz[5] = SH_C2[1] * y;
            dx[6] = SH_C2[2] * (-2.0f * x); dy[6] = SH_C2[2] * (-2.0f * y); dz[6] = SH_C2[2] * (4.0f * z);
            dx[7] = SH_C2[3] * z; dz[7] = SH_C2[3] * x;
            dx[8] = SH_C2[4] * (2.0f * x); dy[8] = SH_C2[4] * (-2.0f * y);
            if (deg > 2) {
                dx[9] = SH_C3[0] * (6.0f * x * y); dy[9] = SH_C3[0] * (3.0f * xx - 3.0f * yy);
                dx[10] = SH_C3[1] * (y * z); dy[10] = SH_C3[1] * (x * z); dz[10] = SH_C3[1] * (x * y);
                dx[11] = SH_C3[2] * (-2.0f * x * y); dy[11] = SH_C3[2] * (4.0f * zz - xx - 3.0f * yy);
                dz[11] = SH_C3[2] * (8.0f * y * z);
                dx[12] = SH_C3[3] * (-6.0f * x * z); dy[12] = SH_C3[3] * (-6.0f * y * z);
                dz[12] = SH_C3[3] * (6.0f * zz - 3.0f * xx - 3.0f * yy);
                dx[13] = SH_C3[4] * (4.0f * zz - 3.0f * xx - yy); dy[13] = SH_C3[4] * (-2.0f * x * y);
                dz[13] = SH_C3[4] * (8.0f * x * z);
                dx[14] = SH_C3[5] * (2.0f * x * z); dy[14] = SH_C3[5] * (-2.0f * y * z);
                dz[14] = SH_C3[5] * (xx - yy);
                dx[15] = SH_C3[6] * (3.0f * xx - 3.0f * yy); dy[15] = SH_C3[6] * (-6.0f * x * y);
            }
        }
    }
}

__device__ __forceinline__ void backward_cov_and_mean(const Frame& f, float px, float py, float pz, const float* gr,
                                                  float4 ca, float2 cb, float* dm, float* g6) {
    float V[16], PM[16];
#pragma unroll
    for (int k = 0; k < 16; ++k) { V[k] = f.view[k]; PM[k] = f.proj[k]; }
    float vx = affine3(V[0], V[4], V[8], V[12], px, py, pz);
    float vy = affine3(V[1], V[5], V[9], V[13], px, py, pz);
    float vz = affine3(V[2], V[6], V[10], V[14], px, py, pz);
    float c6[6] = {ca.x, ca.y, ca.z, ca.w, cb.x, cb.y};
    Ewa e;
    ewa_setup(f, V, vx, vy, vz, e);
    float a, b, c;
    cov2d_from_cov3d(e, c6, a, b, c);
    float denom = a * c - b * b;
    float d2inv = 1.0f / (denom * denom + 0.0000001f);
    const float4 gc = make_float4(gr[2], gr[3], gr[4], gr[5]);
    float da = 0, db = 0, dc = 0;
    if (d2inv != 0.0f) {
        da = d2inv * (-c * c * gc.x + b * c * gc.y + (denom - a * c) * gc.z);
        dc = d2inv * (-a * a * gc.z + a * b * gc.y + (denom - a * c) * gc.x);
        db = d2inv * (2.0f * b * c * gc.x - (denom + 2.0f * b * b) * gc.y + 2.0f * a * b * gc.z);
        const float(*Tm)[3] = e.Tm;
        g6[0] = Tm[0][0] * Tm[0][0] * da + Tm[0][0] * Tm[1][0] * db + Tm[1][0] * Tm[1][0] * dc;
        g6[3] = Tm[0][1] * Tm[0][1] * da + Tm[0][1] * Tm[1][1] * db + Tm[1][1] * Tm[1][1] * dc;
        g6[5] = Tm[0][2] * Tm[0][2] * da + Tm[0][2] * Tm[1][2] * db + Tm[1][2] * Tm[1][2] * dc;
        g6[1] = 2 * Tm[0][0] * Tm[0][1] * da + (Tm[0][0] * Tm[1][1] + Tm[0][1] * Tm[1][0]) * db +
                2 * Tm[1][0] * Tm[1][1] * dc;
        g6[2] = 2 * Tm[0][0] * Tm[0][2] * da + (Tm[0][0] * Tm[1][2] + Tm[0][2] * Tm[1][0]) * db +
                2 * Tm[1][0] * Tm[1][2] * dc;
        g6[4] = 2 * Tm[0][2] * Tm[0][1] * da + (Tm[0][1] * Tm[1][2] + Tm[0][2] * Tm[1][1]) * db +
                2 * Tm[1][1] * Tm[1][2] * dc;
    }
    float S[3][3] = {{c6[0], c6[1], c6[2]}, {c6[1], c6[3], c6[4]}, {c6[2], c6[4], c6[5]}};
    float dJ00 = 0, dJ02 = 0, dJ11 = 0, dJ12 = 0;
#pragma unroll
    for (int k = 0; k < 3; ++k) {
        float st0 = S[k][0] * e.Tm[0][0] + S[k][1] * e.Tm[0][1] + S[k][2] * e.Tm[0][2];
        float st1 = S[k][0] * e.Tm[1][0] + S[k][1] * e.Tm[1][1] + S[k][2] * e.Tm[1][2];
        float dT0 = 2.0f * da * st0 + db * st1;
        float dT1 = 2.0f * dc * st1 + db * st0;
        dJ00 += dT0 * V[0 + 4 * k];
        dJ02 += dT0 * V[2 + 4 * k];
        dJ11 += dT1 * V[1 + 4 * k];
        dJ12 += dT1 * V[2 + 4 * k];
    }
    float tz = 1.0f / e.tz, tz2 = tz * tz, tz3 = tz2 * tz;
    float dtx = e.xmul * -f.fx * tz2 * dJ02;
    float dty = e.ymul * -f.fy * tz2 * dJ12;
    float dtz = -f.fx * tz2 * dJ00 - f.fy * tz2 * dJ11 + (2 * f.fx * e.tx) * tz3 * dJ02 +
                (2 * f.fy * e.ty) * tz3 * dJ12;
    dm[0] = V[0] * dtx + V[1] * dty + V[2] * dtz;
    dm[1] = V[4] * dtx + V[5] * dty + V[6] * dtz;
    dm[2] = V[8] * dtx + V[9] * dty + V[10] * dtz;

    float hx = affine3(PM[0], PM[4], PM[8], PM[12], px, py, pz);
    float hy = affine3(PM[1], PM[5], PM[9], PM[13], px, py, pz);
    float hw = affine3(PM[3], PM[7], PM[11], PM[15], px, py, pz);
    float mw = 1.0f / (hw + 0.0000001f);
    float mul1 = hx * mw * mw, mul2 = hy * mw * mw;
    float g2x = gr[0], g2y = gr[1];
    dm[0] += (PM[0] * mw - PM[3] * mul1) * g2x + (PM[1] * mw - PM[3] * mul2) * g2y;
    dm[1] += (PM[4] * mw - PM[7] * mul1) * g2x + (PM[5] * mw - PM[7] * mul2) * g2y;
    dm[2] += (PM[8] * mw - PM[11] * mul1) * g2x + (PM[9] * mw - PM[11] * mul2) * g2y;

}

__device__ __forceinline__ void backward_scale_rot(const Frame& f, const float* g6, float4 qrot, const float* sa_in, float* ds,
                                                   float* dq) {
    float4 q = qrot;
    float nq = 1.0f;
    if (f.raw) {
        nq = fmaxf(sqrtf(q.x * q.x + q.y * q.y + q.z * q.z + q.w * q.w), 1e-12f);
        q = make_float4(q.x / nq, q.y / nq, q.z / nq, q.w / nq);
    }
    float R[3][3];
    quat_to_rot(q.x, q.y, q.z, q.w, R);
    float sa[3] = {sa_in[0], sa_in[1], sa_in[2]};
    if (f.raw) { sa[0] = expf(sa[0]); sa[1] = expf(sa[1]); sa[2] = expf(sa[2]); }
    float s[3] = {f.scale_modifier * sa[0], f.scale_modifier * sa[1], f.scale_modifier * sa[2]};
    float Gf[3][3] = {{g6[0], 0.5f * g6[1], 0.5f * g6[2]},
                      {0.5f * g6[1], g6[3], 0.5f * g6[4]},
                      {0.5f * g6[2], 0.5f * g6[4], g6[5]}};
    float dR[3][3];
#pragma unroll
    for (int j = 0; j < 3; ++j) {
        float acc_s = 0;
#pragma unroll
        for (int r = 0; r < 3; ++r) {
            float dMrj = 2.0f * (Gf[r][0] * R[0][j] + Gf[r][1] * R[1][j] + Gf[r][2] * R[2][j]) * s[j];
            acc_s += dMrj * R[r][j];
            dR[r][j] = dMrj * s[j];
        }
        ds[j] = acc_s * f.scale_modifier;
    }
    float qr = q.x, qx = q.y, qy = q.z, qz = q.w;
    dq[0] = 2.0f * (-qz * dR[0][1] + qy * dR[0][2] + qz * dR[1][0] - qx * dR[1][2] - qy * dR[2][0] + qx * dR[2][1]);
    dq[1] = 2.0f * (qy * dR[0][1] + qz * dR[0][2] + qy * dR[1][0] - 2 * qx * dR[1][1] - qr * dR[1][2] +
                    qz * dR[2][0] + qr * dR[2][1] - 2 * qx * dR[2][2]);
    dq[2] = 2.0f * (-2 * qy * dR[0][0] + qx * dR[0][1] + qr * dR[0][2] + qx * dR[1][0] + qz * dR[1][2] -
                    qr * dR[2][0] + qz * dR[2][1] - 2 * qy * dR[2][2]);
    dq[3] = 2.0f * (-2 * qz * dR[0][0] - qr * dR[0][1] + qx * dR[0][2] + qr * dR[1][0] - 2 * qz * dR[1][1] +
                    qy * dR[1][2] + qx * dR[2][0] + qy * dR[2][1]);
    if (f.raw) {
        ds[0] *= sa[0]; ds[1] *= sa[1]; ds[2] *= sa[2];
        const float dot = q.x * dq[0] + q.y * dq[1] + q.z * dq[2] + q.w * dq[3];
        const float inq = 1.0f / nq;
        dq[0] = (dq[0] - q.x * dot) * inq; dq[1] = (dq[1] - q.y * dot) * inq;
        dq[2] = (dq[2] - q.z * dot) * inq; dq[3] = (dq[3] - q.w * dot) * inq;
    }
}

__global__ __launch_bounds__(kPB) void preprocess_backward_kernel(
    Frame f, const float* __restrict__ means3D, const float* __restrict__ shs,
    const float* __restrict__ scales, const float* __restrict__ rotations,
    const float* __restrict__ cov3D_precomp, const int32_t* __restrict__ radii, GeomView g,
    const float* __restrict__ grad_rows, float* __restrict__ dL_dmeans3D, float* __restrict__ dL_dmeans2D,
    float* __restrict__ dL_dopacity, float* __restrict__ dL_dcolors, float* __restrict__ dL_dshs,
    float* __restrict__ dL_dcov3D, float* __restrict__ dL_dscales, float* __restrict__ dL_drots, RawBackwardExtra rawx) {
    extern __shared__ __attribute__((aligned(16))) float s_dyn[];
    const int tid = threadIdx.x;
    const int blk0 = blockIdx.x * kPB;
    const int i = blk0 + tid;
    const int n_rec = min(kPB, f.P - blk0);
    const int shs_w = shs ? sh_stride(f.M) : 0;
    float* s_sh = s_dyn;
    float* s_mean = s_dyn + (size_t)kPB * shs_w;
    float* s_scale = s_mean + 3 * kPB;
    float* s_dmean = s_scale + 3 * kPB;
    float* s_dm2d = s_dmean + 3 * kPB;
    float* s_dscale = s_dm2d + 3 * kPB;
    if (shs) stage_sh_in(f, shs, s_sh, blk0, n_rec, shs_w);
    stage_in(means3D + (size_t)blk0 * 3, s_mean, n_rec, 3, 3);
    if (scales) stage_in(scales + (size_t)blk0 * 3, s_scale, n_rec, 3, 3);
    const bool in_range = i < f.P;
    const float raw_o = (f.raw && in_range) ? rawx.raw_opacity[i] : 0.0f;
    const bool live = in_range && radii[i] > 0;
    float gr[9] = {0, 0, 0, 0, 0, 0, 0, 0, 0};
    float4 ca = make_float4(0.f, 0.f, 0.f, 0.f), qrot = make_float4(1.f, 0.f, 0.f, 0.f);
    float2 cb = make_float2(0.f, 0.f);
    uint32_t cl_bits = 0;
    if (live) {
        const float4* row = reinterpret_cast<const float4*>(grad_rows + (size_t)i * kGradRow);
        float4 a = row[0], b4 = row[1];
        gr[0] = a.x; gr[1] = a.y; gr[2] = a.z; gr[3] = a.w; gr[4] = b4.x; gr[5] = b4.y; gr[6] = b4.z; gr[7] = b4.w;
        gr[8] = grad_rows[(size_t)i * kGradRow + 8];
        ca = g.cov_a[i];
        cb = g.cov_b[i];
        if (!cov3D_precomp) qrot = *reinterpret_cast<const float4*>(rotations + 4 * (size_t)i);
        if (shs) cl_bits = g.clamped[i];
    }
    __syncthreads();
    s_dm2d[3 * tid] = gr[0]; s_dm2d[3 * tid + 1] = gr[1]; s_dm2d[3 * tid + 2] = 0.0f;
    if (in_range) {
        float go = gr[5];
        if (f.raw) { const float o = sigmoidf_(raw_o); go *= o * (1.0f - o); }
        dL_dopacity[i] = go;
        if (dL_dcolors) {
            const uint32_t cl = cl_bits;
            dL_dcolors[3 * (size_t)i] = (cl & 1u) ? 0.0f : gr[6];
            dL_dcolors[3 * (size_t)i + 1] = (cl & 2u) ? 0.0f : gr[7];
            dL_dcolors[3 * (size_t)i + 2] = (cl & 4u) ? 0.0f : gr[8];
        }
    }
    float dm[3] = {0, 0, 0};
    float g6[6] = {0, 0, 0, 0, 0, 0};
    const int nb = (f.deg + 1) * (f.deg + 1);
    if (live) {
        const float px = s_mean[3 * tid], py = s_mean[3 * tid + 1], pz = s_mean[3 * tid + 2];
        backward_cov_and_mean(f, px, py, pz, gr, ca, cb, dm, g6);

        if (shs) {
            float ox = px - f.campos[0], oy = py - f.campos[1], oz = pz - f.campos[2];
            float len = sqrtf(ox * ox + oy * oy + oz * oz);
            float dx = ox / len, dy = oy / len, dz = oz / len;
            float bs[16], bx[16], by[16], bz[16];
            sh_basis(f.deg, dx, dy, dz, bs);
            sh_basis_grad(f.deg, dx, dy, dz, bx, by, bz);
            float* sh = s_sh + (size_t)tid * shs_w;
            const uint32_t cl = cl_bits;
            float gcol[3];
#pragma unroll
            for (int ch = 0; ch < 3; ++ch) gcol[ch] = ((cl >> ch) & 1u) ? 0.0f : gr[6 + ch];
            float ddx = 0, ddy = 0, ddz = 0;
            for (int k = 0; k < nb; ++k) {
#pragma unroll
                for (int ch = 0; ch < 3; ++ch) {
                    float w = sh[3 * k + ch] * gcol[ch];
                    sh[3 * k + ch] = bs[k] * gcol[ch];
                    ddx += bx[k] * w; ddy += by[k] * w; ddz += bz[k] * w;
                }
            }
            for (int k = 3 * nb; k < 3 * f.M; ++k) sh[k] = 0.0f;
            float dotp = dx * ddx + dy * ddy + dz * ddz;
            dm[0] += (ddx - dx * dotp) / len;
            dm[1] += (ddy - dy * dotp) / len;
            dm[2] += (ddz - dz * dotp) / len;
        }
    } else if (shs) {
        float* dsh = s_sh + (size_t)tid * shs_w;
        for (int k = 0; k < 3 * f.M; ++k) dsh[k] = 0.0f;
    }
    s_dmean[3 * tid] = dm[0]; s_dmean[3 * tid + 1] = dm[1]; s_dmean[3 * tid + 2] = dm[2];

    if (cov3D_precomp) {
        if (in_range) {
#pragma unroll
            for (int k = 0; k < 6; ++k) dL_dcov3D[6 * (size_t)i + k] = g6[k];
        }
    } else {
        float ds[3] = {0, 0, 0}, dq[4] = {0, 0, 0, 0};
        if (live) {
            const float sa_in[3] = {s_scale[3 * tid], s_scale[3 * tid + 1], s_scale[3 * tid + 2]};
            backward_scale_rot(f, g6, qrot, sa_in, ds, dq);
        }
        s_dscale[3 * tid] = ds[0]; s_dscale[3 * tid + 1] = ds[1]; s_dscale[3 * tid + 2] = ds[2];
        if (in_range) *reinterpret_cast<float4*>(dL_drots + 4 * (size_t)i) = make_float4(dq[0], dq[1], dq[2], dq[3]);
    }
    __syncthreads();
    stage_out(dL_dmeans3D + (size_t)blk0 * 3, s_dmean, n_rec, 3, 3);
    stage_out(dL_dmeans2D + (size_t)blk0 * 3, s_dm2d, n_rec, 3, 3);
    if (!cov3D_precomp) stage_out(dL_dscales + (size_t)blk0 * 3, s_dscale, n_rec, 3, 3);
    if (shs && dL_dshs) {
        if (!f.raw) {
            stage_out(dL_dshs + (size_t)blk0 * f.M * 3, s_sh, n_rec, 3 * f.M, shs_w);
        } else {
            stage_out(dL_dshs + (size_t)blk0 * 3, s_sh, n_rec, 3, shs_w);
            if (f.M > 1) stage_out_split(rawx.dL_dshs_rest + (size_t)blk0 * (3 * f.M - 3), s_sh + 3, n_rec, 3 * f.M - 3, shs_w);
        }
    }
}

constexpr int kSparseBlock = 64;
__global__ __launch_bounds__(kSparseBlock) void preprocess_backward_sparse_kernel(
    Frame f, const float* __restrict__ means3D, const float* __restrict__ shs, const float* __restrict__ scales,
    const float* __restrict__ rotations, const float* __restrict__ cov3D_precomp, GeomView g,
    const float* __restrict__ grad_rows, float* __restrict__ dL_dmeans3D, float* __restrict__ dL_dmeans2D,
    float* __restrict__ dL_dopacity, float* __restrict__ dL_dcolors, float* __restrict__ dL_dshs,
    float* __restrict__ dL_dcov3D, float* __restrict__ dL_dscales, float* __restrict__ dL_drots, RawBackwardExtra rawx,
    int vec_ok) {
    const uint32_t n_touched = *g.touched_count;
    for (uint32_t slot = blockIdx.x * (uint32_t)kSparseBlock + threadIdx.x; slot < n_touched; slot += gridDim.x * (uint32_t)kSparseBlock) {
    const int i = (int)g.touched_list[slot];
    const size_t si = (size_t)i;
    float gr[9];
    {
        const float4* row = reinterpret_cast<const float4*>(grad_rows + si * kGradRow);
        const float4 a = row[0], b4 = row[1];
        gr[0] = a.x; gr[1] = a.y; gr[2] = a.z; gr[3] = a.w; gr[4] = b4.x; gr[5] = b4.y; gr[6] = b4.z; gr[7] = b4.w;
        gr[8] = grad_rows[si * kGradRow + 8];
    }
    const float4 ca = g.cov_a[i];
    const float2 cb = g.cov_b[i];
    const uint32_t cl = shs ? g.clamped[i] : 0u;
    const float px = means3D[3 * si], py = means3D[3 * si + 1], pz = means3D[3 * si + 2];
    dL_dmeans2D[3 * si] = gr[0];
    dL_dmeans2D[3 * si + 1] = gr[1];
    {
        float go = gr[5];
        if (f.raw) { const float o = sigmoidf_(rawx.raw_opacity[i]); go *= o * (1.0f - o); }
        dL_dopacity[i] = go;
    }
    if (dL_dcolors) {
        dL_dcolors[3 * si] = (cl & 1u) ? 0.0f : gr[6];
        dL_dcolors[3 * si + 1] = (cl & 2u) ? 0.0f : gr[7];
        dL_dcolors[3 * si + 2] = (cl & 4u) ? 0.0f : gr[8];
    }
    float dm[3] = {0, 0, 0};
    float g6[6] = {0, 0, 0, 0, 0, 0};
    backward_cov_and_mean(f, px, py, pz, gr, ca, cb, dm, g6);
    if (shs) {
        const int M = f.M, nb = (f.deg + 1) * (f.deg + 1);
        float ox = px - f.campos[0], oy = py - f.campos[1], oz = pz - f.campos[2];
        float len = sqrtf(ox * ox + oy * oy + oz * oz);
        float dx = ox / len, dy = oy / len, dz = oz / len;
        float bs[16], bx[16], by[16], bz[16];
        sh_basis(f.deg, dx, dy, dz, bs);
        sh_basis_grad(f.deg, dx, dy, dz, bx, by, bz);
        float gcol[3];
#pragma unroll
        for (int ch = 0; ch < 3; ++ch) gcol[ch] = ((cl >> ch) & 1u) ? 0.0f : gr[6 + ch];
        const float* in0 = f.raw ? shs + 3 * si : shs + si * M * 3;
        const float* in_rest = f.raw ? f.shs_rest + si * (3 * M - 3) - 3 : in0;
        float* out0 = dL_dshs ? (f.raw ? dL_dshs + 3 * si : dL_dshs + si * M * 3) : nullptr;
        float* out_rest = dL_dshs ? (f.raw ? rawx.dL_dshs_rest + si * (3 * M - 3) - 3 : out0) : nullptr;
        float ddx = 0, ddy = 0, ddz = 0;
        auto row16 = [&](float (&rowv)[48]) __attribute__((always_inline)) {
#pragma unroll
            for (int k = 0; k < 16; ++k) {
#pragma unroll
                for (int ch = 0; ch < 3; ++ch) {
                    const float w = k < nb ? rowv[3 * k + ch] * gcol[ch] : 0.f;
                    rowv[3 * k + ch] = k < nb ? bs[k] * gcol[ch] : 0.f;
                    ddx += bx[k] * w; ddy += by[k] * w; ddz += bz[k] * w;
                }
            }
        };
        if (!f.raw && M == 16 && (vec_ok & 1)) {
            float rowv[48];
            const float4* in4 = reinterpret_cast<const float4*>(in0);
#pragma unroll
            for (int v = 0; v < 12; ++v) { const float4 t = in4[v]; rowv[4 * v] = t.x; rowv[4 * v + 1] = t.y; rowv[4 * v + 2] = t.z; rowv[4 * v + 3] = t.w; }
            row16(rowv);
            if (out0) {
                float4* out4 = reinterpret_cast<float4*>(out0);
#pragma unroll
                for (int v = 0; v < 12; ++v) out4[v] = make_float4(rowv[4 * v], rowv[4 * v + 1], rowv[4 * v + 2], rowv[4 * v + 3]);
            }
        } else if (!f.raw && M == 16) {
            struct W4 { float a, b, c, d; };
            float rowv[48];
#pragma unroll
            for (int v = 0; v < 12; ++v) {
                const W4 t = *reinterpret_cast<const W4*>(in0 + 4 * v);
                rowv[4 * v] = t.a; rowv[4 * v + 1] = t.b; rowv[4 * v + 2] = t.c; rowv[4 * v + 3] = t.d;
            }
            row16(rowv);
            if (out0) {
#pragma unroll
                for (int v = 0; v < 12; ++v) *reinterpret_cast<W4*>(out0 + 4 * v) = W4{rowv[4 * v], rowv[4 * v + 1], rowv[4 * v + 2], rowv[4 * v + 3]};
            }
        } else if (f.raw && M == 16) {
            struct W3 { float a, b, c; };
            struct W4 { float a, b, c, d; };
            float rowv[48];
            const float* rp = f.shs_rest + si * 45;
            const W3 t0 = *reinterpret_cast<const W3*>(in0);
            rowv[0] = t0.a; rowv[1] = t0.b; rowv[2] = t0.c;
#pragma unroll
            for (int v = 0; v < 11; ++v) {
                const W4 t = *reinterpret_cast<const W4*>(rp + 4 * v);
                rowv[3 + 4 * v] = t.a; rowv[4 + 4 * v] = t.b; rowv[5 + 4 * v] = t.c; rowv[6 + 4 * v] = t.d;
            }
            rowv[47] = rp[44];
            row16(rowv);
            if (out0) {
                float* op = rawx.dL_dshs_rest + si * 45;
                *reinterpret_cast<W3*>(out0) = W3{rowv[0], rowv[1], rowv[2]};
#pragma unroll
                for (int v = 0; v < 11; ++v)
                    *reinterpret_cast<W4*>(op + 4 * v) = W4{rowv[3 + 4 * v], rowv[4 + 4 * v], rowv[5 + 4 * v], rowv[6 + 4 * v]};
                op[44] = rowv[47];
            }
        } else {
#pragma unroll
            for (int k = 0; k < 16; ++k) {
                if (k < nb) {
                    const float* in = k == 0 ? in0 : in_rest + 3 * k;
                    float* out = k == 0 ? out0 : out_rest + 3 * k;
#pragma unroll
                    for (int ch = 0; ch < 3; ++ch) {
                        const float w = in[ch] * gcol[ch];
                        if (out0) out[ch] = bs[k] * gcol[ch];
                        ddx += bx[k] * w; ddy += by[k] * w; ddz += bz[k] * w;
                    }
                }
            }
        }
        float dotp = dx * ddx + dy * ddy + dz * ddz;
        dm[0] += (ddx - dx * dotp) / len;
        dm[1] += (ddy - dy * dotp) / len;
        dm[2] += (ddz - dz * dotp) / len;
    }
    dL_dmeans3D[3 * si] = dm[0]; dL_dmeans3D[3 * si + 1] = dm[1]; dL_dmeans3D[3 * si + 2] = dm[2];
    if (cov3D_precomp) {
#pragma unroll
        for (int k = 0; k < 6; ++k) dL_dcov3D[6 * si + k] = g6[k];
    } else {
        const float4 qrot = (vec_ok & 2) ? *reinterpret_cast<const float4*>(rotations + 4 * si)
                                         : make_float4(rotations[4 * si], rotations[4 * si + 1], rotations[4 * si + 2], rotations[4 * si + 3]);
        const float sa_in[3] = {scales[3 * si], scales[3 * si + 1], scales[3 * si + 2]};
        float ds[3] = {0, 0, 0}, dq[4] = {0, 0, 0, 0};
        backward_scale_rot(f, g6, qrot, sa_in, ds, dq);
        dL_dscales[3 * si] = ds[0]; dL_dscales[3 * si + 1] = ds[1]; dL_dscales[3 * si + 2] = ds[2];
        dL_drots[4 * si] = dq[0]; dL_drots[4 * si + 1] = dq[1]; dL_drots[4 * si + 2] = dq[2]; dL_drots[4 * si + 3] = dq[3];
    }
    }
}

constexpr int kCompactThreads = 1024, kCompactPer = 16;
__global__ __launch_bounds__(kCompactThreads) void compact_touched_kernel(int P, const uint8_t* __restrict__ touched,
                                                                         uint32_t* __restrict__ list, uint32_t* __restrict__ count) {
    __shared__ uint32_t s_wave[kCompactThreads / 64];
    __shared__ uint32_t s_base;
    const int tid = threadIdx.x;
    const int i0 = (blockIdx.x * kCompactThreads + tid) * kCompactPer;
    uint4 w = make_uint4(0u, 0u, 0u, 0u);
    if (i0 < P) w = *reinterpret_cast<const uint4*>(touched + i0);
    const uint32_t ww[4] = {w.x, w.y, w.z, w.w};
    uint32_t mine = 0;
#pragma unroll
    for (int q = 0; q < 4; ++q)
        mine += ((ww[q] & 0xFFu) != 0) + ((ww[q] & 0xFF00u) != 0) + ((ww[q] & 0xFF0000u) != 0) + ((ww[q] >> 24) != 0);
    uint32_t total;
    const uint32_t off = block_excl_scan<kCompactThreads / 64>(mine, tid, s_wave, &total);
    if (total == 0) return;
    if (tid == 0) s_base = atomicAdd(count, total);
    __syncthreads();
    uint32_t dst = s_base + off;
#pragma unroll
    for (int q = 0; q < 4; ++q)
#pragma unroll
        for (int k = 0; k < 4; ++k)
            if (((ww[q] >> (8 * k)) & 0xFFu) && i0 + 4 * q + k < P) list[dst++] = (uint32_t)(i0 + 4 * q + k);
}

int launch_preprocess_backward_sparse(const Frame& f, const float* means3D, const float* shs, const float* scales,
                                      const float* rotations, const float* cov3D_precomp, GeomView g, const float* grad_rows,
                                      float* dL_dmeans3D, float* dL_dmeans2D, float* dL_dopacity, float* dL_dcolors,
                                      float* dL_dshs, float* dL_dcov3D, float* dL_dscales, float* dL_drots, hipStream_t st,
                                      RawBackwardExtra rawx) {
    if (f.P <= 0) return 0;
    constexpr int kPerBlock = kCompactThreads * kCompactPer;
    hipLaunchKernelGGL(compact_touched_kernel, dim3((f.P + kPerBlock - 1) / kPerBlock), dim3(kCompactThreads), 0, st, f.P, g.touched,
                       g.touched_list, g.touched_count);
    const int sparse_blocks = min((f.P + kSparseBlock - 1) / kSparseBlock, 2048);
    auto al16 = [](const void* p) { return ((uintptr_t)p & 15u) == 0; };
    const int vec_ok = ((al16(shs) && al16(dL_dshs)) ? 1 : 0) | (al16(rotations) ? 2 : 0);
    hipLaunchKernelGGL(preprocess_backward_sparse_kernel, dim3(sparse_blocks), dim3(kSparseBlock), 0, st, f, means3D, shs, scales,
                       rotations, cov3D_precomp, g, grad_rows, dL_dmeans3D, dL_dmeans2D, dL_dopacity, dL_dcolors, dL_dshs,
                       dL_dcov3D, dL_dscales, dL_drots, rawx, vec_ok);
    return hipGetLastError() == hipSuccess ? 0 : MVI_EHIP;
}

int launch_preprocess_backward(const Frame& f, const float* means3D, const float* shs,
                               const float* scales, const float* rotations, const float* cov3D_precomp,
                               const int32_t* radii, GeomView g, const float* grad_rows, float* dL_dmeans3D,
                               float* dL_dmeans2D, float* dL_dopacity, float* dL_dcolors, float* dL_dshs,
                               float* dL_dcov3D, float* dL_dscales, float* dL_drots, hipStream_t st, RawBackwardExtra rawx) {
    if (f.P <= 0) return 0;
    int nblk = (f.P + kPB - 1) / kPB;
    size_t lds = sizeof(float) * ((size_t)kPB * (shs ? sh_stride(f.M) : 0) + 15 * kPB);
    if (lds > 64 * 1024 &&
        hipFuncSetAttribute((const void*)preprocess_backward_kernel, hipFuncAttributeMaxDynamicSharedMemorySize, (int)lds) != hipSuccess)
        return MVI_EHIP;
    hipLaunchKernelGGL(preprocess_backward_kernel, dim3(nblk), dim3(kPB), lds, st, f, means3D, shs, scales,
                       rotations, cov3D_precomp, radii, g, grad_rows, dL_dmeans3D, dL_dmeans2D, dL_dopacity,
                       dL_dcolors, dL_dshs, dL_dcov3D, dL_dscales, dL_drots, rawx);
    return hipGetLastError() == hipSuccess ? 0 : MVI_EHIP;
}

__global__ __launch_bounds__(kPB) void sh_backward_views_kernel(int P, int M, int deg, int n_views,
                                                                    const float* __restrict__ means3D,
                                                                    const float* __restrict__ campos,
                                                                    int64_t campos_stride,
                                                                    const float* __restrict__ gcol,
                                                                    int64_t gcol_stride,
                                                                    float* __restrict__ dL_dshs) {
    extern __shared__ __attribute__((aligned(16))) float s_dyn[];
    const int tid = threadIdx.x;
    const int blk0 = blockIdx.x * kPB;
    const int i = blk0 + tid;
    const int n_rec = min(kPB, P - blk0);
    const int w = sh_stride(M);
    const int nb = (deg + 1) * (deg + 1);
    float acc[16][3];
#pragma unroll
    for (int k = 0; k < 16; ++k) acc[k][0] = acc[k][1] = acc[k][2] = 0.0f;
    if (i < P) {
        const float px = means3D[3 * (size_t)i], py = means3D[3 * (size_t)i + 1], pz = means3D[3 * (size_t)i + 2];
        for (int v = 0; v < n_views; ++v) {
            const float* gc = gcol + (size_t)v * gcol_stride + (size_t)i * 3;
            const float* cp = campos + (size_t)v * campos_stride;
            const float c0 = gc[0], c1 = gc[1], c2 = gc[2];
            if (c0 == 0.0f && c1 == 0.0f && c2 == 0.0f) continue;
            const float ox = px - cp[0], oy = py - cp[1], oz = pz - cp[2];
            const float len = sqrtf(ox * ox + oy * oy + oz * oz);
            float bs[16];
            sh_basis(deg, ox / len, oy / len, oz / len, bs);
#pragma unroll
            for (int k = 0; k < 16; ++k)
                if (k < nb) { acc[k][0] += bs[k] * c0; acc[k][1] += bs[k] * c1; acc[k][2] += bs[k] * c2; }
        }
    }
    float* row = s_dyn + (size_t)tid * w;
#pragma unroll
    for (int k = 0; k < 16; ++k)
        if (k < M) { row[3 * k] = acc[k][0]; row[3 * k + 1] = acc[k][1]; row[3 * k + 2] = acc[k][2]; }
    __syncthreads();
    stage_out(dL_dshs + (size_t)blk0 * M * 3, s_dyn, n_rec, 3 * M, w);
}

int launch_sh_backward_views(int P, int M, int deg, int n_views, const float* means3D, const float* campos,
                             int64_t campos_stride, const float* gcol, int64_t gcol_stride, float* dL_dshs, hipStream_t st) {
    if (P <= 0) return 0;
    const size_t lds = sizeof(float) * (size_t)kPB * sh_stride(M);
    hipLaunchKernelGGL(sh_backward_views_kernel, dim3((P + kPB - 1) / kPB), dim3(kPB), lds, st, P, M, deg, n_views,
                       means3D, campos, campos_stride, gcol, gcol_stride, dL_dshs);
    return hipGetLastError() == hipSuccess ? 0 : MVI_EHIP;
}

__global__ void mark_visible_kernel(int P, const float* __restrict__ means3D, const float* __restrict__ view,
                                    uint8_t* __restrict__ visible) {
    int i = blockIdx.x * kPB + threadIdx.x;
    if (i >= P) return;
    float vz = affine3(view[2], view[6], view[10], view[14], means3D[3 * i], means3D[3 * i + 1], means3D[3 * i + 2]);
    visible[i] = vz > kNearZ;
}
__global__ __launch_bounds__(256) void color_factor_kernel(int P, const int32_t* __restrict__ radii,
                                                           const float* __restrict__ grad_rows,
                                                           const uint8_t* __restrict__ clamped, float* __restrict__ out) {
    const int i = blockIdx.x * 256 + threadIdx.x;
    if (i >= P) return;
    float r = 0.f, g_ = 0.f, b = 0.f;
    if (radii[i] > 0) {
        const float* row = grad_rows + (size_t)i * kGradRow;
        const uint32_t cl = clamped ? clamped[i] : 0u;
        r = (cl & 1u) ? 0.0f : row[6];
        g_ = (cl & 2u) ? 0.0f : row[7];
        b = (cl & 4u) ? 0.0f : row[8];
    }
    out[3 * (size_t)i] = r; out[3 * (size_t)i + 1] = g_; out[3 * (size_t)i + 2] = b;
}
__global__ __launch_bounds__(256) void resolve_colors_kernel(Frame f, GeomView g) {
    const ColorSource cs = *g.color_src;
    if (!cs.deferred) return;
    const int i = blockIdx.x * 256 + threadIdx.x;
    if (i >= f.P || g.tiles_touched[i] == 0) return;
    const float4 cd = g.rgbd[i];
    if (color_pending(cd)) resolve_color(cs, f.campos, (uint32_t)i, cd.w, g.rgbd, g.clamped);
}
int launch_resolve_colors(const Frame& f, GeomView g, hipStream_t st) {
    if (f.P <= 0) return 0;
    hipLaunchKernelGGL(resolve_colors_kernel, dim3((f.P + 255) / 256), dim3(256), 0, st, f, g);
    return hipGetLastError() == hipSuccess ? 0 : MVI_EHIP;
}

int launch_color_factors(int P, const int32_t* radii, const float* grad_rows, const uint8_t* clamped, float* out, hipStream_t st) {
    if (P <= 0) return 0;
    hipLaunchKernelGGL(color_factor_kernel, dim3((P + 255) / 256), dim3(256), 0, st, P, radii, grad_rows, clamped, out);
    return hipGetLastError() == hipSuccess ? 0 : MVI_EHIP;
}

int launch_mark_visible(int P, const float* means3D, const float* view, uint8_t* visible, hipStream_t st) {
    if (P <= 0) return 0;
    hipLaunchKernelGGL(mark_visible_kernel, dim3((P + kPB - 1) / kPB), dim3(kPB), 0, st, P, means3D, view, visible);
    return hipGetLastError() == hipSuccess ? 0 : MVI_EHIP;
}

}
```

### multiview_inpaint_amd/csrc/raster_render.hip

```cpp
#include <cstdlib>

#include "raster_common.h"

namespace mvi {

__device__ __forceinline__ unsigned long long ballot64(bool p) { return __builtin_amdgcn_ballot_w64(p); }


__device__ __forceinline__ float active_t2(float4 co) {
    float t2 = 2.0f * __logf(255.0f * co.w);
    return t2 > 0.0f ? t2 * 1.001f + 0.01f : -1.0f;
}

__device__ __forceinline__ bool quad_overlap(float2 c, float4 co, float t2, float qx0, float qy0, float bw = 7.0f,
                                             float bh = 7.0f) {
    const float dxl = qx0 - c.x, dxr = dxl + bw, dyl = qy0 - c.y, dyr = dyl + bh;
    const float px = fminf(fmaxf(0.0f, dxl), dxr), py = fminf(fmaxf(0.0f, dyl), dyr);
    const float dy1 = fminf(fmaxf(-co.y * px * __builtin_amdgcn_rcpf(co.z), dyl), dyr);
    const float dx2 = fminf(fmaxf(-co.y * py * __builtin_amdgcn_rcpf(co.x), dxl), dxr);
    const float f1 = co.x * px * px + 2.0f * co.y * px * dy1 + co.z * dy1 * dy1;
    const float f2 = co.x * dx2 * dx2 + 2.0f * co.y * dx2 * py + co.z * py * py;
    const float f = px == 0.0f ? (py == 0.0f ? 0.0f : f2) : (py == 0.0f ? f1 : fminf(f1, f2));
    return f <= t2;
}

__device__ __forceinline__ int xcd_band_tile(int bid, int tiles) {
    const int q = tiles >> 3, r = tiles & 7, x = bid & 7, i = bid >> 3;
    return x * q + (x < r ? x : r) + i;
}

typedef float f2 __attribute__((ext_vector_type(2)));
__device__ __forceinline__ f2 pk_fma(f2 a, f2 b, f2 c) { return __builtin_elementwise_fma(a, b, c); }
__device__ __forceinline__ f2 splat(float v) { return f2{v, v}; }
constexpr int kB2 = 128;

__device__ __forceinline__ f2 gauss_power(float4 co, float dx, f2 dy) {
#pragma clang fp contract(off)
    const float ax = co.x * dx, bx = co.y * dx;
    const f2 cyy = (co.z * dy) * dy;
    const f2 sq = pk_fma(splat(dx), splat(ax), cyy);
    const f2 bxy = bx * dy;
    return pk_fma(sq, splat(-0.5f), -bxy);
}

__device__ __forceinline__ float gauss_power1(float4 co, float dx, float dy) {
#pragma clang fp contract(off)
    const float ax = co.x * dx, bx = co.y * dx;
    const float cyy = (co.z * dy) * dy;
    const float sq = __builtin_fmaf(dx, ax, cyy);
    const float bxy = bx * dy;
    return __builtin_fmaf(sq, -0.5f, -bxy);
}

__global__ __launch_bounds__(kBlock) void render_forward_kernel(
    Frame f, const uint32_t* __restrict__ ranges, const uint32_t* __restrict__ point_list,
    const float2* __restrict__ xy, float4* rgbd, const float4* __restrict__ conic_opacity,
    float* __restrict__ final_T, uint32_t* __restrict__ n_contrib, float* __restrict__ out_color,
    float* __restrict__ out_depth, ZeroRegions zero, const ColorSource* __restrict__ color_src, uint8_t* clamped) {
    __shared__ float2 s_xy[kBlock];
    __shared__ float s_t2[kBlock];
    __shared__ float4 s_co[kBlock];
    __shared__ float4 s_cd[kBlock];
    __shared__ float4 w_s[4][3][64];
    const int tid = threadIdx.x, wave = tid >> 6, lane = tid & 63;
    zero_share(zero, tid, kBlock);
    const int tile = xcd_band_tile(blockIdx.x, f.gx * f.gy);
    const int tile_y = tile / f.gx, tile_x = tile - tile_y * f.gx;
    const int qx0 = tile_x * kTile + 8 * (wave & 1), qy0 = tile_y * kTile + 8 * (wave >> 1);
    const int pxi = qx0 + (lane & 7), pyi = qy0 + (lane >> 3);
    const bool inside = pxi < f.W && pyi < f.H;
    const float pfx = (float)pxi, pfy = (float)pyi;
    const uint32_t r0 = ranges[2 * tile], r1 = ranges[2 * tile + 1];
    int todo = (int)(r1 - r0);
    const int rounds = (todo + kBlock - 1) / kBlock;

    float T = inside ? 1.0f : 0.0f;
    float T_out = 1.0f, C2 = 0.f, Dp = kDepthSentinel, Tc = 1.0f;
    f2 C01 = {0.f, 0.f};
    uint32_t last = 0;

    const ColorSource cs = *color_src;
    float2 n_xy = make_float2(0.f, 0.f);
    float4 n_co = make_float4(0.f, 0.f, 0.f, 0.f), n_cd = n_co;
    uint32_t n_id = 0;
    auto fetch = [&](int r) {
        const uint32_t q = r0 + (uint32_t)(r * kBlock + tid);
        if (q < r1) {
            n_id = point_list[q];
            n_xy = xy[n_id]; n_co = conic_opacity[n_id]; n_cd = rgbd[n_id];
        }
    };
    if (rounds > 0) fetch(0);
    for (int r = 0; r < rounds; ++r, todo -= kBlock) {
        if (__syncthreads_count(T <= 0.0f) == kBlock) break;
        if (cs.deferred && tid < todo && color_pending(n_cd)) n_cd = resolve_color_small(cs, f.campos, n_id, n_cd.w, rgbd, clamped);
        s_xy[tid] = n_xy;
        s_co[tid] = n_co;
        s_t2[tid] = active_t2(n_co);
        s_cd[tid] = n_cd;
        __syncthreads();
        if (r + 1 < rounds) fetch(r + 1);
        const int n = todo < kBlock ? todo : kBlock;
        for (int c = 0; c < n; c += 64) {
            if (ballot64(T > 0.0f) == 0ull) break;
            const int e = c + lane;
            const bool keep = e < n && quad_overlap(s_xy[e], s_co[e], s_t2[e], (float)qx0, (float)qy0);
            const unsigned long long mask = ballot64(keep);
            if (mask == 0ull) continue;
            if (keep) {
                const int pos = __builtin_amdgcn_mbcnt_hi((uint32_t)(mask >> 32), __builtin_amdgcn_mbcnt_lo((uint32_t)mask, 0u));
                const float2 q = s_xy[e];
                w_s[wave][0][pos] = make_float4(q.x, q.y, __uint_as_float((uint32_t)(r * kBlock + e + 1)), 0.f);
                w_s[wave][1][pos] = s_co[e];
                w_s[wave][2][pos] = s_cd[e];
            }
            const int cnt = __popcll(mask);
            float4 a = w_s[wave][0][0], co = w_s[wave][1][0], cd = w_s[wave][2][0];
            for (int k = 0; k < cnt; ++k) {
                const int kn = k + 1 < 64 ? k + 1 : 63;
                const float4* nx = &w_s[wave][0][kn];
                const float4 an = nx[0], con = nx[64], cdn = nx[128];
                float dx = a.x - pfx, dy = a.y - pfy;
                float power = gauss_power1(co, dx, dy);
                float alpha = fminf(kAlphaMax, co.w * __expf(power));
                alpha = power <= 0.0f ? alpha : 0.0f;
                const float test_T = T * (1.0f - alpha);
                const bool valid = alpha >= kAlphaMin;
                const bool contrib = valid && test_T >= kTEps;
                const float w = contrib ? alpha * T : 0.0f;
                C01 = pk_fma(f2{cd.x, cd.y}, splat(w), C01);
                C2 = __builtin_fmaf(cd.z, w, C2);
                const bool above = contrib && T > 0.5f;
                Dp = above ? cd.w : Dp;
                Tc = above ? test_T : Tc;
                T_out = contrib ? test_T : T_out;
                last = contrib ? __float_as_uint(a.z) : last;
                T = contrib ? test_T : (valid ? 0.0f : T);
                a = an; co = con; cd = cdn;
            }
        }
    }
    if (inside) {
        size_t pix = (size_t)pyi * f.W + pxi, hw = (size_t)f.H * f.W;
        final_T[pix] = T_out;
        n_contrib[pix] = last;
        out_color[pix] = C01.x + T_out * f.bg[0];
        out_color[hw + pix] = C01.y + T_out * f.bg[1];
        out_color[2 * hw + pix] = C2 + T_out * f.bg[2];
        out_depth[pix] = Tc < 0.5f ? Dp : kDepthSentinel;
    }
}

constexpr int kFrontTiles = 4;
constexpr int kFrontMax = 1024;
__global__ __launch_bounds__(kBlock) void mark_front_kernel(int tiles, const uint32_t* __restrict__ ranges,
                                                            const uint32_t* __restrict__ point_list, uint8_t* __restrict__ front,
                                                            int n_front, const ColorSource* __restrict__ color_src, int gx,
                                                            int every) {
    if (!color_src->deferred) return;
    const int tid = threadIdx.x;
    const int sx = (gx + every - 1) / every;
#pragma unroll
    for (int t = 0; t < kFrontTiles; ++t) {
        const int j = blockIdx.x * kFrontTiles + t;
        const int tile = every == 1 ? j : (j / sx) * every * gx + (j % sx) * every;
        if (tile >= tiles) break;
        const uint32_t r0 = ranges[2 * tile], r1 = ranges[2 * tile + 1];
        const uint32_t n = min(r1 - r0, (uint32_t)n_front);
        for (uint32_t e = tid; e < n; e += kBlock) front[point_list[r0 + e]] = 1;
    }
}
constexpr int kMarkedPer = 4;
__global__ __launch_bounds__(kBlock) void resolve_marked_kernel(Frame f, GeomView g) {
    const ColorSource cs = *g.color_src;
    if (!cs.deferred) return;
    __shared__ uint32_t s_id[kBlock * kMarkedPer];
    __shared__ uint32_t s_n;
    const int tid = threadIdx.x;
    if (tid == 0) s_n = 0;
    __syncthreads();
    const int i0 = (blockIdx.x * kBlock + tid) * kMarkedPer;
    if (i0 < f.P) {
        const uint32_t w = *reinterpret_cast<const uint32_t*>(g.front + i0);
#pragma unroll
        for (int k = 0; k < kMarkedPer; ++k)
            if (((w >> (8 * k)) & 0xFFu) && i0 + k < f.P) s_id[atomicAdd(&s_n, 1u)] = (uint32_t)(i0 + k);
    }
    __syncthreads();
    const uint32_t total = s_n;
    for (uint32_t i = tid; i < total; i += kBlock) {
        const uint32_t id = s_id[i];
        const float4 cd = g.rgbd[id];
        if (color_pending(cd)) resolve_color(cs, f.campos, id, cd.w, g.rgbd, g.clamped);
    }
}

int launch_zero_fill(void* p, size_t bytes, hipStream_t st);
int launch_render_forward(const Frame& f, GeomView g, BinningView b, ImageView im, int64_t D,
                          float* out_color, float* out_depth, hipStream_t st, float* zero_rows) {
    ZeroRegions z;
    if (zero_rows) {
        z.add(zero_rows, (size_t)f.P * kGradRow);
        z.add(g.touched, ((size_t)f.P + 15) / 16 * 4);
        z.add(g.touched_count, 1);
    }
    if (f.W <= 0 || f.H <= 0) return launch_zero_regions(z, st);
    const uint32_t* plist = b.vals[b.passes & 1];
    const unsigned blocks = (unsigned)(f.gx * f.gy);
    if (f.defer_colors && D > 0) {
        static const int n_front = [] { const char* e = getenv("MVI_RASTER_FRONT_ENTRIES"); const int v = e ? atoi(e) : kBlock;
                                        return v < 0 ? 0 : (v > kFrontMax ? kFrontMax : v); }();
        static const int every = [] { const char* e = getenv("MVI_RASTER_FRONT_EVERY"); const int v = e ? atoi(e) : 2; return v < 1 ? 1 : v; }();
        if (n_front > 0) {
            const unsigned sampled = (unsigned)(((f.gx + every - 1) / every) * ((f.gy + every - 1) / every));
            hipLaunchKernelGGL(mark_front_kernel, dim3((sampled + kFrontTiles - 1) / kFrontTiles), dim3(kBlock), 0, st, (int)blocks,
                               im.ranges, plist, g.front, n_front, g.color_src, f.gx, every);
            hipLaunchKernelGGL(resolve_marked_kernel, dim3((f.P + kBlock * kMarkedPer - 1) / (kBlock * kMarkedPer)), dim3(kBlock), 0, st,
                               f, g);
        }
    }
    hipLaunchKernelGGL(render_forward_kernel, dim3(blocks), dim3(kBlock), 0, st, f, im.ranges, plist, g.xy,
                       g.rgbd, g.conic_opacity, im.final_T, im.n_contrib, out_color, out_depth, z, g.color_src, g.clamped);
    return hipGetLastError() == hipSuccess ? 0 : MVI_EHIP;
}

__global__ __launch_bounds__(256) void zero_regions_kernel(ZeroRegions z) { zero_share(z, threadIdx.x, 256); }
int launch_zero_regions(const ZeroRegions& z, hipStream_t st) {
    if (z.n == 0) return 0;
    hipLaunchKernelGGL(zero_regions_kernel, dim3(2048), dim3(256), 0, st, z);
    return hipGetLastError() == hipSuccess ? 0 : MVI_EHIP;
}

constexpr int kRow = 16;

__device__ __forceinline__ constexpr int wave_sum9_moment(int lane) { return lane < 32 ? lane >> 2 : 8; }
__device__ __forceinline__ constexpr bool wave_sum9_owner(int lane) { return (lane & 3) == 0 && lane <= 32; }
#define MVI_FOLD(a, b, lo, hi, mlo, mhi)                                                                  \
    "v_add_f32_dpp " a ", " a ", " a " row_ror:" lo " row_mask:0xf bank_mask:" mlo "\n\t"                  \
    "v_add_f32_dpp " a ", " b ", " b " row_ror:" hi " row_mask:0xf bank_mask:" mhi "\n\t"
#define MVI_FULL(a, n) "v_add_f32_dpp " a ", " a ", " a " row_ror:" n " row_mask:0xf bank_mask:0xf\n\t"
__device__ __forceinline__ float wave_sum9(float m0, float m1, float m2, float m3, float m4, float m5, float m6, float m7,
                                           float m8) {
    asm("s_nop 1\n\t"
        MVI_FOLD("%0", "%2", "8", "8", "0x3", "0xc") MVI_FOLD("%1", "%3", "8", "8", "0x3", "0xc")
        MVI_FOLD("%4", "%6", "8", "8", "0x3", "0xc") MVI_FOLD("%5", "%7", "8", "8", "0x3", "0xc") MVI_FULL("%8", "8")
        MVI_FOLD("%0", "%1", "12", "4", "0x5", "0xa") MVI_FOLD("%4", "%5", "12", "4", "0x5", "0xa") MVI_FULL("%8", "4")
        : "+v"(m0), "+v"(m1), "+v"(m2), "+v"(m3), "+v"(m4), "+v"(m5), "+v"(m6), "+v"(m7), "+v"(m8));
    const auto a = __builtin_amdgcn_permlane16_swap(__float_as_uint(m0), __float_as_uint(m4), false, false);
    const auto b = __builtin_amdgcn_permlane16_swap(__float_as_uint(m8), __float_as_uint(m8), false, false);
    const float lo = __uint_as_float(a[0]) + __uint_as_float(a[1]), hi = __uint_as_float(b[0]) + __uint_as_float(b[1]);
    const auto c = __builtin_amdgcn_permlane32_swap(__float_as_uint(lo), __float_as_uint(hi), false, false);
    float s = __uint_as_float(c[0]) + __uint_as_float(c[1]);
    asm("s_nop 1\n\t"
        "v_add_f32_dpp %0, %0, %0 quad_perm:[1,0,3,2] row_mask:0xf bank_mask:0xf\n\t"
        "s_nop 1\n\t"
        "v_add_f32_dpp %0, %0, %0 quad_perm:[2,3,0,1] row_mask:0xf bank_mask:0xf"
        : "+v"(s));
    return s;
}
#undef MVI_FOLD
#undef MVI_FULL

__global__ __launch_bounds__(64) void wave_sum9_probe_kernel(const float* __restrict__ in, float* __restrict__ out) {
    const int lane = threadIdx.x;
    const float* x = in + (size_t)blockIdx.x * 9 * 64 + lane;
    const float s = wave_sum9(x[0], x[64], x[128], x[192], x[256], x[320], x[384], x[448], x[512]);
    if (wave_sum9_owner(lane)) out[blockIdx.x * 9 + wave_sum9_moment(lane)] = s;
}
int launch_wave_sum9_probe(const float* in, float* out, int n_waves, hipStream_t st) {
    if (n_waves <= 0) return 0;
    hipLaunchKernelGGL(wave_sum9_probe_kernel, dim3(n_waves), dim3(64), 0, st, in, out);
    return hipGetLastError() == hipSuccess ? 0 : MVI_EHIP;
}

#ifndef MVI_RB_WAVES
#define MVI_RB_WAVES 5
#endif
__global__ __launch_bounds__(kB2) __attribute__((amdgpu_waves_per_eu(MVI_RB_WAVES, MVI_RB_WAVES))) void render_backward_kernel(
    Frame f, const uint32_t* __restrict__ ranges, const uint32_t* __restrict__ point_list,
    const float2* __restrict__ xy, const float4* __restrict__ rgbd, const float4* __restrict__ conic_opacity,
    const float* __restrict__ final_T, const uint32_t* __restrict__ n_contrib,
    const float* __restrict__ dL_dpix, float* __restrict__ grad_rows, uint8_t* __restrict__ touched, ZeroRegions zero) {
#pragma clang fp contract(off)
    zero_share(zero, threadIdx.x, kB2);
    __shared__ float4 s_ent[3][kB2];
    __shared__ float s_acc[kB2][9];
    __shared__ uint32_t s_blast[2];
    const int tid = threadIdx.x, wave = tid >> 6, lane = tid & 63;
    const int tile = xcd_band_tile(blockIdx.x, f.gx * f.gy);
    const int tile_y = tile / f.gx, tile_x = tile - tile_y * f.gx;
    const int hx0 = tile_x * kTile, hy0 = tile_y * kTile + 8 * wave;
    const int pxi = hx0 + (lane & 15), py0 = hy0 + 2 * (lane >> 4), py1 = py0 + 1;
    const bool in0 = pxi < f.W && py0 < f.H, in1 = pxi < f.W && py1 < f.H;
    const float pfx = (float)pxi;
    const f2 pfy = {(float)py0, (float)py1};
    const uint32_t r0 = ranges[2 * tile];
    const size_t hw = (size_t)f.H * f.W, pix0 = (size_t)py0 * f.W + pxi, pix1 = pix0 + f.W;

    const f2 T_final = {in0 ? final_T[pix0] : 0.0f, in1 ? final_T[pix1] : 0.0f};
    f2 T = T_final;
    const uint32_t last0 = in0 ? n_contrib[pix0] : 0u, last1 = in1 ? n_contrib[pix1] : 0u;
    f2 A_dot = {0.f, 0.f};
    f2 dp0 = {0.f, 0.f}, dp1 = {0.f, 0.f}, dp2 = {0.f, 0.f};
    if (in0) { dp0.x = dL_dpix[pix0]; dp1.x = dL_dpix[hw + pix0]; dp2.x = dL_dpix[2 * hw + pix0]; }
    if (in1) { dp0.y = dL_dpix[pix1]; dp1.y = dL_dpix[hw + pix1]; dp2.y = dL_dpix[2 * hw + pix1]; }
    const f2 bg_dot = f.bg[0] * dp0 + f.bg[1] * dp1 + f.bg[2] * dp2;
    const f2 bg_term = -T_final * bg_dot;
    uint32_t wave_last = max(last0, last1);
    for (int o = 32; o > 0; o >>= 1) wave_last = max(wave_last, (uint32_t)__shfl_xor((int)wave_last, o));
    if (lane == 0) s_blast[wave] = wave_last;
    __syncthreads();
    const int total = (int)max(s_blast[0], s_blast[1]);
    const int rounds = (total + kB2 - 1) / kB2;
    const bool owner = wave_sum9_owner(lane);
    typedef __attribute__((address_space(3))) float lds_float;
    const uint32_t acc_lane = (uint32_t)(uintptr_t)(lds_float*)&s_acc[0][wave_sum9_moment(lane)];

    uint32_t n_id = 0;
    float2 n_xy = make_float2(0.f, 0.f);
    float4 n_co = make_float4(0.f, 0.f, 0.f, 0.f), n_cd = n_co;
    auto fetch = [&](int r) {
        const int hi_ = total - r * kB2;
        if (tid < hi_) {
            n_id = point_list[r0 + (uint32_t)(hi_ - 1 - tid)];
            n_xy = xy[n_id]; n_co = conic_opacity[n_id]; n_cd = rgbd[n_id];
        }
    };
    if (rounds > 0) fetch(0);
    for (int r = 0; r < rounds; ++r) {
        const int hi = total - r * kB2;
        const int n = hi < kB2 ? hi : kB2;
        __syncthreads();
        s_ent[0][tid] = make_float4(n_xy.x, n_xy.y, active_t2(n_co), __uint_as_float(n_id));
        s_ent[1][tid] = n_co;
        s_ent[2][tid] = n_cd;
#pragma unroll
        for (int c = 0; c < 9; ++c) s_acc[tid][c] = 0.0f;
        __syncthreads();
        if (r + 1 < rounds) fetch(r + 1);
        for (int c = 0; c < n; c += 64) {
            const int e = c + lane;
            const float4 ce = s_ent[0][e];
            const bool keep = e < n && (uint32_t)(hi - 1 - e) < wave_last &&
                              quad_overlap(make_float2(ce.x, ce.y), s_ent[1][e], ce.z, (float)hx0, (float)hy0, 15.0f, 7.0f);
            unsigned long long mask = ballot64(keep);
            while (mask != 0ull) {
                const int jc = c + __builtin_ctzll(mask);
                mask &= mask - 1;
                const float4* rec = &s_ent[0][jc];
                const float2 p = *reinterpret_cast<const float2*>(rec);
                const float4 co = rec[kB2], col = rec[2 * kB2];
                const uint32_t pos = (uint32_t)(hi - 1 - jc);
                const float dx = p.x - pfx;
                const f2 dy = splat(p.y) - pfy;
                const f2 power = gauss_power(co, dx, dy);
                const f2 G = {__expf(power.x), __expf(power.y)};
                const f2 oG = co.w * G;
                const bool act0 = pos < last0 && power.x <= 0.0f && oG.x >= kAlphaMin;
                const bool act1 = pos < last1 && power.y <= 0.0f && oG.y >= kAlphaMin;
                const f2 gm = {act0 ? oG.x : 0.0f, act1 ? oG.y : 0.0f};
                const f2 am = __builtin_elementwise_min(splat(kAlphaMax), gm);
                const unsigned long long any_active = ballot64((__float_as_uint(gm.x) | __float_as_uint(gm.y)) != 0u);
                const f2 om = splat(1.0f) - am;
                const f2 inv = {__builtin_amdgcn_rcpf(om.x), __builtin_amdgcn_rcpf(om.y)};
                const f2 Tn = T * inv;
                const f2 c_dot = pk_fma(splat(col.z), dp2, pk_fma(splat(col.y), dp1, col.x * dp0));
                const f2 dL_dalpha = pk_fma(c_dot - A_dot, Tn, bg_term * inv);
                const f2 dch = am * Tn, mw = gm * dL_dalpha;
                T = Tn;
                A_dot = pk_fma(am, c_dot, om * A_dot);
                if (any_active != 0ull) {
                    const f2 vr = dch * dp0, vg = dch * dp1, vb = dch * dp2;
                    const f2 vx = mw * dx, vy = mw * dy;
                    const f2 vxx = vx * dx, vxy = vx * dy, vyy = vy * dy;
                    float m_w = mw.x + mw.y, m_x = vx.x + vx.y, m_y = vy.x + vy.y, m_xx = vxx.x + vxx.y,
                          m_xy = vxy.x + vxy.y, m_yy = vyy.x + vyy.y, m_r = vr.x + vr.y, m_g = vg.x + vg.y, m_b = vb.x + vb.y;
                    const float sum = wave_sum9(m_w, m_x, m_y, m_xx, m_xy, m_yy, m_r, m_g, m_b);
                    uint32_t row = 36u * (uint32_t)jc;
                    asm("" : "+s"(row));
                    if (owner) __hip_atomic_fetch_add((lds_float*)(uintptr_t)(acc_lane + row), sum, __ATOMIC_RELAXED, __HIP_MEMORY_SCOPE_WORKGROUP);
                }
            }
        }
        __syncthreads();
        {
            const int e1 = wave * 64 + lane;
            if (e1 < n) {
                float* a = s_acc[e1];
                const float a0 = a[0], a1 = a[1], a2 = a[2], a3 = a[3], a4 = a[4], a5 = a[5], a6 = a[6], a7 = a[7], a8 = a[8];
                const bool any = (((__float_as_uint(a0) | __float_as_uint(a1) | __float_as_uint(a2)) |
                                   (__float_as_uint(a3) | __float_as_uint(a4) | __float_as_uint(a5)) |
                                   (__float_as_uint(a6) | __float_as_uint(a7) | __float_as_uint(a8))) & 0x7FFFFFFFu) != 0u;
                if (any) {
                    const float4 co = s_ent[1][e1];
                    a[0] = -0.5f * (float)f.W * (co.x * a1 + co.y * a2);
                    a[1] = -0.5f * (float)f.H * (co.z * a2 + co.y * a1);
                    a[2] = -0.5f * a3;
                    a[3] = -a4;
                    a[4] = -0.5f * a5;
                    a[5] = a0 / co.w;
                } else {
                    s_ent[0][e1].w = __uint_as_float(0xFFFFFFFFu);
                }
            }
            asm volatile("s_waitcnt lgkmcnt(0)" ::: "memory");
            __builtin_amdgcn_wave_barrier();
            const int comp = lane & 15;
#pragma unroll 4
            for (int it = 0; it < 16; ++it) {
                const int e = wave * 64 + it * 4 + (lane >> 4);
                const uint32_t id = e < n ? __float_as_uint(s_ent[0][e].w) : 0xFFFFFFFFu;
                if (id == 0xFFFFFFFFu || comp >= 9) continue;
                atomicAdd(&grad_rows[(size_t)id * kRow + comp], s_acc[e][comp]);
                if (comp == 0) touched[id] = 1;
            }
        }
    }
}

int launch_render_backward(const Frame& f, GeomView g, BinningView b, ImageView im, int64_t D,
                           const float* dL_dpix, float* grad_rows, hipStream_t st, const ZeroRegions* zero) {
    ZeroRegions z;
    if (zero) z = *zero;
    if (f.W <= 0 || f.H <= 0 || D <= 0) return launch_zero_regions(z, st);
    const uint32_t* plist = b.vals[b.passes & 1];
    hipLaunchKernelGGL(render_backward_kernel, dim3(f.gx * f.gy), dim3(kB2), 0, st, f, im.ranges, plist, g.xy,
                       g.rgbd, g.conic_opacity, im.final_T, im.n_contrib, dL_dpix, grad_rows, g.touched, z);
    return hipGetLastError() == hipSuccess ? 0 : MVI_EHIP;
}

}
```

### multiview_inpaint_amd/raster/__init__.py

```python
import ctypes as C
from typing import NamedTuple, Optional

import torch

from .. import _lib


class GaussianRasterizationSettings(NamedTuple):
    image_height: int
    image_width: int
    tanfovx: float
    tanfovy: float
    bg: torch.Tensor
    scale_modifier: float
    viewmatrix: torch.Tensor
    projmatrix: torch.Tensor
    sh_degree: int
    campos: torch.Tensor
    prefiltered: bool


def _ptr(t: Optional[torch.Tensor]):
    return None if t is None or t.numel() == 0 else C.c_void_p(t.data_ptr())


def _dev_f32(t: torch.Tensor, what: str) -> torch.Tensor:
    if not t.is_cuda:
        raise RuntimeError(f"{what} must be on the GPU (got {t.device}); the rasterizer has no CPU path")
    return t.detach().to(torch.float32).contiguous()


class _Frame:

    def __init__(self, rs: GaussianRasterizationSettings):
        self.keep = [_dev_f32(rs.bg, "bg").reshape(-1), _dev_f32(rs.viewmatrix, "viewmatrix").reshape(-1),
                     _dev_f32(rs.projmatrix, "projmatrix").reshape(-1), _dev_f32(rs.campos, "campos").reshape(-1)]
        if self.keep[0].numel() != 3 or self.keep[1].numel() != 16 or self.keep[2].numel() != 16 or self.keep[3].numel() != 3:
            raise Exception("bg/campos must have 3 elements, viewmatrix/projmatrix 16")
        s = _lib.RasterSettings()
        s.image_height, s.image_width = int(rs.image_height), int(rs.image_width)
        s.tanfovx, s.tanfovy, s.scale_modifier = float(rs.tanfovx), float(rs.tanfovy), float(rs.scale_modifier)
        s.sh_degree, s.prefiltered = int(rs.sh_degree), int(bool(rs.prefiltered))
        s.bg, s.viewmatrix, s.projmatrix, s.campos = (t.data_ptr() for t in self.keep)
        self.c = s


class RasterState:
    __slots__ = ("P", "M", "D", "W", "H", "geom", "binning", "image", "radii", "grad_rows", "rows_clean", "frame", "sources")

    def resolve_colors(self):
        if self.P == 0:
            return
        dev = self.geom.device
        stream = C.c_void_p(torch.cuda.current_stream(dev).cuda_stream)
        with torch.cuda.device(dev):
            _lib.check(_lib.lib().mvi_raster_resolve_colors(C.byref(self.frame.c), self.P, _ptr(self.geom), self.geom.numel(), stream),
                       "resolve_colors")

    def take_rows(self, dev):
        if getattr(self, "grad_rows", None) is not None and getattr(self, "rows_clean", False):
            self.rows_clean = False
            return self.grad_rows, 1
        return torch.empty(self.P, 16, dtype=torch.float32, device=dev), 0

    def views(self):
        L = _lib.lib()
        v = _lib.RasterViews()
        _lib.check(L.mvi_raster_get_views(self.P, self.D, self.W, self.H, _ptr(self.geom), _ptr(self.binning),
                                          _ptr(self.image), C.byref(v)), "get_views")
        return v

    def tensor(self, name, shape, dtype, _derive=True):
        v = self.views()
        addr = getattr(v, name)
        if _derive and name == "tile_ids_sorted" and self.D > 0 and self.binning is not None and self.image is not None:
            dev = self.binning.device
            with torch.cuda.device(dev):
                _lib.check(_lib.lib().mvi_raster_materialize_tile_ids(
                    self.P, self.D, self.W, self.H, _ptr(self.binning), _ptr(self.image),
                    C.c_void_p(torch.cuda.current_stream(dev).cuda_stream)), "materialize_tile_ids")
        n = 1
        for s in shape:
            n *= s
        if name == "tile_ids_sorted" and v.tile_id_bytes == 2 and torch.empty(0, dtype=dtype).element_size() == 4:
            raw = self.tensor(name, tuple(shape) + (2,), torch.uint8, _derive=False).to(torch.int32)
            return (raw[..., 0] | (raw[..., 1] << 8)).to(dtype)
        out = torch.empty(shape, dtype=dtype, device=self.geom.device)
        if n:
            nbytes = n * out.element_size()
            for buf in (self.geom, self.binning, self.image):
                if buf is not None and buf.numel() and buf.data_ptr() <= addr < buf.data_ptr() + buf.numel():
                    off = addr - buf.data_ptr()
                    out.view(torch.uint8).reshape(-1).copy_(buf[off:off + nbytes])
                    return out
            raise RuntimeError(f"view {name} not inside a scratch buffer")
        return out


def _forward_render(L, fr, st, color, depth, stream, prepare_backward, dev):
    st.grad_rows, st.rows_clean = None, False
    if prepare_backward and st.P > 0:
        st.grad_rows = torch.empty(st.P, 16, dtype=torch.float32, device=dev)
        _lib.check(L.mvi_raster_forward_render_prepare(C.byref(fr.c), st.P, st.D, _ptr(st.radii), _ptr(st.geom), st.geom.numel(),
                                                       _ptr(st.binning), st.binning.numel(), _ptr(st.image), st.image.numel(),
                                                       _ptr(color), _ptr(depth), _ptr(st.grad_rows), stream),
                   "rasterize forward (render)")
        st.rows_clean = True
        return
    _lib.check(L.mvi_raster_forward_render(C.byref(fr.c), st.P, st.D, _ptr(st.radii), _ptr(st.geom), st.geom.numel(),
                                           _ptr(st.binning), st.binning.numel(), _ptr(st.image), st.image.numel(),
                                           _ptr(color), _ptr(depth), stream), "rasterize forward (render)")


def rasterize_forward(rs: GaussianRasterizationSettings, means3D, opacities, shs=None, colors_precomp=None,
                      scales=None, rotations=None, cov3D_precomp=None, prepare_backward=False):
    L = _lib.lib()
    fr = _Frame(rs)
    dev = means3D.device
    if dev.type != "cuda":
        raise RuntimeError("means3D must be on the GPU; the rasterizer has no CPU path")
    P = int(means3D.shape[0])
    H, W = int(rs.image_height), int(rs.image_width)
    M = int(shs.shape[1]) if shs is not None and shs.numel() else 0
    st = RasterState()
    st.P, st.M, st.W, st.H = P, M, W, H
    st.frame, st.sources = fr, (means3D, shs)
    u8 = dict(dtype=torch.uint8, device=dev)
    st.geom = torch.empty(L.mvi_raster_geom_bytes(P), **u8)
    st.image = torch.empty(L.mvi_raster_image_bytes(W, H), **u8)
    st.radii = torch.empty(P, dtype=torch.int32, device=dev)
    color = torch.empty(3, H, W, dtype=torch.float32, device=dev)
    depth = torch.empty(1, H, W, dtype=torch.float32, device=dev)
    stream = C.c_void_p(torch.cuda.current_stream(dev).cuda_stream)
    D = C.c_int64(0)
    with torch.cuda.device(dev):
        _lib.check(L.mvi_raster_forward_geom(C.byref(fr.c), P, M, _ptr(means3D), _ptr(shs), _ptr(colors_precomp),
                                             _ptr(opacities), _ptr(scales), _ptr(rotations), _ptr(cov3D_precomp),
                                             _ptr(st.geom), st.geom.numel(), _ptr(st.radii), C.byref(D), stream),
                   "rasterize forward (geom)")
        st.D = int(D.value)
        st.binning = torch.empty(L.mvi_raster_binning_bytes(st.D, W, H) if st.D else 0, **u8)
        _forward_render(L, fr, st, color, depth, stream, prepare_backward, dev)
    return color, st.radii, depth, st


def rasterize_backward(rs: GaussianRasterizationSettings, st: RasterState, grad_color, means3D, shs=None,
                       colors_precomp=None, scales=None, rotations=None, cov3D_precomp=None, out=None, sh_grad="dense"):
    if sh_grad not in ("dense", "factor", "both"):
        raise ValueError(f"sh_grad must be 'dense', 'factor' or 'both', got {sh_grad!r}")
    L = _lib.lib()
    fr = _Frame(rs)
    dev = means3D.device
    P = st.P
    f32 = dict(dtype=torch.float32, device=dev)
    out = out or {}

    def buf(name, *shape):
        t = out.get(name)
        if t is None:
            return torch.empty(*shape, **f32)
        if tuple(t.shape) != shape or t.dtype != torch.float32 or not t.is_contiguous() or t.device != dev:
            raise RuntimeError(f"out[{name!r}] must be a contiguous fp32 {shape} tensor on {dev}")
        return t
    g = dict(means3D=buf("means3D", P, 3), means2D=buf("means2D", P, 3), opacities=buf("opacities", P, 1),
             shs=None, colors_precomp=None, scales=None, rotations=None, cov3D_precomp=None)
    dcolors = None
    if shs is not None:
        if sh_grad != "factor":
            g["shs"] = buf("shs", P, st.M, 3)
        if sh_grad != "dense":
            dcolors = g["sh_color_factor"] = buf("sh_color_factor", P, 3)
    else:
        dcolors = g["colors_precomp"] = buf("colors_precomp", P, 3)
    if cov3D_precomp is not None:
        g["cov3D_precomp"] = buf("cov3D_precomp", P, 6)
    else:
        g["scales"], g["rotations"] = buf("scales", P, 3), buf("rotations", P, 4)
    scratch, clean = st.take_rows(dev)
    grad_color = grad_color.to(torch.float32).contiguous()
    stream = C.c_void_p(torch.cuda.current_stream(dev).cuda_stream)
    with torch.cuda.device(dev):
        _lib.check(L.mvi_raster_backward(
            C.byref(fr.c), P, st.M, st.D, _ptr(means3D), _ptr(shs), _ptr(colors_precomp), _ptr(scales), _ptr(rotations),
            _ptr(cov3D_precomp), _ptr(st.radii), _ptr(st.geom), _ptr(st.binning), _ptr(st.image), _ptr(grad_color),
            _ptr(g["means3D"]), _ptr(g["means2D"]), _ptr(g["opacities"]), _ptr(g["shs"]), _ptr(dcolors),
            _ptr(g["scales"]), _ptr(g["rotations"]), _ptr(g["cov3D_precomp"]), _ptr(scratch), clean, stream),
            "rasterize backward")
    return g


def rasterize_backward_split(rs: GaussianRasterizationSettings, st: RasterState, grad_color, means3D, shs, scales, rotations,
                             out, after_render=None):
    L = _lib.lib()
    fr = _Frame(rs)
    dev = means3D.device
    P = st.P
    f32 = dict(dtype=torch.float32, device=dev)
    g = {k: out[k] for k in ("means3D", "means2D", "opacities", "scales", "rotations", "sh_color_factor")}
    for k, shape in (("means3D", (P, 3)), ("means2D", (P, 3)), ("opacities", (P, 1)), ("scales", (P, 3)), ("rotations", (P, 4)),
                     ("sh_color_factor", (P, 3))):
        t = g[k]
        if tuple(t.shape) != shape or t.dtype != torch.float32 or not t.is_contiguous() or t.device != dev:
            raise RuntimeError(f"out[{k!r}] must be a contiguous fp32 {shape} tensor on {dev}")
    scratch, clean = st.take_rows(dev)
    spare = torch.empty(P, 3, **f32)
    grad_color = grad_color.to(torch.float32).contiguous()
    stream = C.c_void_p(torch.cuda.current_stream(dev).cuda_stream)
    with torch.cuda.device(dev):
        _lib.check(L.mvi_raster_backward_render(C.byref(fr.c), P, st.D, _ptr(st.radii), _ptr(st.geom), _ptr(st.binning),
                                                _ptr(st.image), _ptr(grad_color), _ptr(scratch), _ptr(g["sh_color_factor"]), 1,
                                                clean, stream), "rasterize backward (render)")
        if after_render is not None:
            after_render()
        _lib.check(L.mvi_raster_backward_geom(C.byref(fr.c), P, st.M, _ptr(means3D), _ptr(shs), None, _ptr(scales),
                                              _ptr(rotations), None, _ptr(st.radii), _ptr(st.geom), _ptr(scratch),
                                              _ptr(g["means3D"]), _ptr(g["means2D"]), _ptr(g["opacities"]), None, _ptr(spare),
                                              _ptr(g["scales"]), _ptr(g["rotations"]), None, stream),
                   "rasterize backward (geom)")
    return g


def rasterize_backward_ranged(rs: GaussianRasterizationSettings, st: RasterState, grad_color, means3D, shs, scales, rotations,
                              exchange, means2D_out=None):
    L = _lib.lib()
    fr = _Frame(rs)
    dev = means3D.device
    P = st.P
    f32 = dict(dtype=torch.float32, device=dev)
    if exchange.P != P or exchange.M != st.M:
        raise RuntimeError(f"exchange was built for P={exchange.P}, M={exchange.M}; this view has P={P}, M={st.M}")
    factor = exchange.views["sh_color_factor"]
    m2d = torch.zeros(P, 3, **f32) if means2D_out is None else means2D_out
    scratch, clean = st.take_rows(dev)
    spare = torch.empty(P, 3, **f32)
    grad_color = grad_color.to(torch.float32).contiguous()
    stream = C.c_void_p(torch.cuda.current_stream(dev).cuda_stream)
    with torch.cuda.device(dev):
        _lib.check(L.mvi_raster_backward_render(C.byref(fr.c), P, st.D, _ptr(st.radii), _ptr(st.geom), _ptr(st.binning),
                                                _ptr(st.image), _ptr(grad_color), _ptr(scratch), _ptr(factor), 1, clean, stream),
                   "rasterize backward (render)")
        exchange.begin_gather(rs.campos)
        for r, (first, n) in enumerate(exchange.ranges):
            v = exchange.range_views(r)
            base = lambda t, w: C.c_void_p(t.data_ptr() - 4 * w * first)
            _lib.check(L.mvi_raster_backward_geom_range(C.byref(fr.c), P, st.M, first, n, _ptr(means3D), _ptr(shs), None, _ptr(scales),
                                                        _ptr(rotations), None, _ptr(st.radii), _ptr(st.geom), _ptr(scratch),
                                                        base(v["means3D"], 3), _ptr(m2d), base(v["opacities"], 1), None, _ptr(spare),
                                                        base(v["scales"], 3), base(v["rotations"], 4), None, stream),
                       "rasterize backward (geom range)")
            exchange.reduce_range(r)
    g = exchange.finish(means3D)
    g["means2D"] = m2d
    return g


def sh_backward_views(means3D, campos, color_factors, M, sh_degree, out=None):
    L = _lib.lib()
    dev = means3D.device
    P = means3D.shape[0]
    V = color_factors.shape[0]
    if campos.shape != (V, 3) or color_factors.shape != (V, P, 3):
        raise ValueError(f"sh_backward_views: campos {tuple(campos.shape)} / color_factors {tuple(color_factors.shape)} "
                         f"do not match V={V}, P={P}")
    for t in (means3D, campos, color_factors):
        if t.dtype != torch.float32 or t.device != dev:
            raise RuntimeError("sh_backward_views: fp32 tensors on one device required")
    if not means3D.is_contiguous():
        means3D = means3D.contiguous()
    if V > 1 and (campos.stride(1) != 1 or color_factors.stride(2) != 1 or color_factors.stride(1) != 3):
        campos, color_factors = campos.contiguous(), color_factors.contiguous()
    elif V == 1:
        campos, color_factors = campos.contiguous(), color_factors.contiguous()
    if out is None:
        out = torch.empty(P, M, 3, dtype=torch.float32, device=dev)
    elif tuple(out.shape) != (P, M, 3) or out.dtype != torch.float32 or not out.is_contiguous() or out.device != dev:
        raise RuntimeError(f"sh_backward_views: out must be a contiguous fp32 ({P}, {M}, 3) tensor on {dev}")
    stream = C.c_void_p(torch.cuda.current_stream(dev).cuda_stream)
    with torch.cuda.device(dev):
        _lib.check(L.mvi_raster_sh_backward_views(P, M, int(sh_degree), V, _ptr(means3D), _ptr(campos),
                                                  campos.stride(0) if V > 1 else 3, _ptr(color_factors),
                                                  color_factors.stride(0) if V > 1 else 3 * P, _ptr(out), stream),
                   "sh_backward_views")
    return out


def rasterize_forward_raw(rs: GaussianRasterizationSettings, xyz, features_dc, features_rest, raw_opacity, raw_scaling,
                          raw_rotation, prepare_backward=False):
    L = _lib.lib()
    fr = _Frame(rs)
    dev = xyz.device
    if dev.type != "cuda":
        raise RuntimeError("xyz must be on the GPU; the rasterizer has no CPU path")
    P, M = int(xyz.shape[0]), 1 + int(features_rest.shape[1])
    if features_dc.shape != (P, 1, 3) or features_rest.shape != (P, M - 1, 3) or raw_opacity.numel() != P or \
            raw_scaling.shape != (P, 3) or raw_rotation.shape != (P, 4):
        raise ValueError("rasterize_forward_raw: expected [P,3], [P,1,3], [P,M-1,3], [P,1], [P,3], [P,4]")
    H, W = int(rs.image_height), int(rs.image_width)
    st = RasterState()
    st.P, st.M, st.W, st.H = P, M, W, H
    st.frame, st.sources = fr, (xyz, features_dc, features_rest)
    u8 = dict(dtype=torch.uint8, device=dev)
    st.geom = torch.empty(L.mvi_raster_geom_bytes(P), **u8)
    st.image = torch.empty(L.mvi_raster_image_bytes(W, H), **u8)
    st.radii = torch.empty(P, dtype=torch.int32, device=dev)
    color = torch.empty(3, H, W, dtype=torch.float32, device=dev)
    depth = torch.empty(1, H, W, dtype=torch.float32, device=dev)
    stream = C.c_void_p(torch.cuda.current_stream(dev).cuda_stream)
    D = C.c_int64(0)
    with torch.cuda.device(dev):
        _lib.check(L.mvi_raster_forward_geom_raw(C.byref(fr.c), P, M, _ptr(xyz), _ptr(features_dc), _ptr(features_rest),
                                                 _ptr(raw_opacity), _ptr(raw_scaling), _ptr(raw_rotation), _ptr(st.geom),
                                                 st.geom.numel(), _ptr(st.radii), C.byref(D), stream),
                   "rasterize forward raw (geom)")
        st.D = int(D.value)
        st.binning = torch.empty(L.mvi_raster_binning_bytes(st.D, W, H) if st.D else 0, **u8)
        _forward_render(L, fr, st, color, depth, stream, prepare_backward, dev)
    return color, st.radii, depth, st


def rasterize_backward_raw(rs: GaussianRasterizationSettings, st: RasterState, grad_color, xyz, features_dc, features_rest,
                           raw_opacity, raw_scaling, raw_rotation, out=None, sh_grad="dense"):
    if sh_grad not in ("dense", "factor"):
        raise ValueError(f"sh_grad must be 'dense' or 'factor', got {sh_grad!r}")
    L = _lib.lib()
    fr = _Frame(rs)
    dev, P, M = xyz.device, st.P, st.M
    f32 = dict(dtype=torch.float32, device=dev)
    out = out or {}

    def buf(name, *shape):
        t = out.get(name)
        if t is None:
            return torch.empty(*shape, **f32)
        if tuple(t.shape) != shape or t.dtype != torch.float32 or not t.is_contiguous() or t.device != dev:
            raise RuntimeError(f"out[{name!r}] must be a contiguous fp32 {shape} tensor on {dev}")
        return t
    g = dict(xyz=buf("xyz", P, 3), means2D=buf("means2D", P, 3), opacity=buf("opacity", P, 1), features_dc=None, features_rest=None,
             scaling=buf("scaling", P, 3), rotation=buf("rotation", P, 4))
    scratch, clean = st.take_rows(dev)
    grad_color = grad_color.to(torch.float32).contiguous()
    stream = C.c_void_p(torch.cuda.current_stream(dev).cuda_stream)
    with torch.cuda.device(dev):
        if sh_grad == "factor":
            g["sh_color_factor"] = buf("sh_color_factor", P, 3)
            _lib.check(L.mvi_raster_backward_raw_factor(
                C.byref(fr.c), P, M, st.D, _ptr(xyz), _ptr(features_dc), _ptr(features_rest), _ptr(raw_opacity), _ptr(raw_scaling),
                _ptr(raw_rotation), _ptr(st.radii), _ptr(st.geom), _ptr(st.binning), _ptr(st.image), _ptr(grad_color),
                _ptr(g["xyz"]), _ptr(g["means2D"]), _ptr(g["opacity"]), _ptr(g["sh_color_factor"]),
                _ptr(g["scaling"]), _ptr(g["rotation"]), _ptr(scratch), clean, stream), "rasterize backward raw (factor)")
            return g
        g["features_dc"], g["features_rest"] = buf("features_dc", P, 1, 3), buf("features_rest", P, M - 1, 3)
        _lib.check(L.mvi_raster_backward_raw(
            C.byref(fr.c), P, M, st.D, _ptr(xyz), _ptr(features_dc), _ptr(features_rest), _ptr(raw_opacity), _ptr(raw_scaling),
            _ptr(raw_rotation), _ptr(st.radii), _ptr(st.geom), _ptr(st.binning), _ptr(st.image), _ptr(grad_color),
            _ptr(g["xyz"]), _ptr(g["means2D"]), _ptr(g["opacity"]), _ptr(g["features_dc"]), _ptr(g["features_rest"]),
            _ptr(g["scaling"]), _ptr(g["rotation"]), _ptr(scratch), clean, stream), "rasterize backward raw")
    return g


class _RasterizeRaw(torch.autograd.Function):
    @staticmethod
    def forward(ctx, xyz, means2D, features_dc, features_rest, raw_opacity, raw_scaling, raw_rotation, rs):
        a = [t.detach().to(torch.float32).contiguous() for t in (xyz, features_dc, features_rest, raw_opacity, raw_scaling,
                                                                  raw_rotation)]
        need = any(ctx.needs_input_grad[:7])
        color, radii, depth, st = rasterize_forward_raw(rs, *a, prepare_backward=need)
        ctx.rs, ctx.st, ctx.a = rs, st, a
        ctx.mark_non_differentiable(radii, depth)
        return color, radii, depth

    @staticmethod
    def backward(ctx, grad_color, _gr, _gd):
        st = ctx.st
        if st.P == 0:
            return tuple(torch.zeros_like(t) for t in (ctx.a[0], ctx.a[0], *ctx.a[1:])) + (None,)
        g = rasterize_backward_raw(ctx.rs, st, grad_color, *ctx.a)
        return (g["xyz"], g["means2D"], g["features_dc"], g["features_rest"], g["opacity"].view_as(ctx.a[3]), g["scaling"],
                g["rotation"], None)


def _opt(t):
    if t is None or t.numel() == 0:
        return None
    return t.to(torch.float32).contiguous()


class _Rasterize(torch.autograd.Function):
    @staticmethod
    def forward(ctx, means3D, means2D, shs, colors_precomp, opacities, scales, rotations, cov3D_precomp, rs):
        a = dict(means3D=_opt(means3D), shs=_opt(shs), colors_precomp=_opt(colors_precomp), opacities=_opt(opacities),
                 scales=_opt(scales), rotations=_opt(rotations), cov3D_precomp=_opt(cov3D_precomp))
        if a["means3D"] is None:
            a["means3D"] = means3D.to(torch.float32).reshape(0, 3)
        color, radii, depth, st = rasterize_forward(rs, a["means3D"], a["opacities"], a["shs"], a["colors_precomp"],
                                                    a["scales"], a["rotations"], a["cov3D_precomp"],
                                                    prepare_backward=any(ctx.needs_input_grad[:8]))
        ctx.rs, ctx.st, ctx.a = rs, st, a
        ctx.mark_non_differentiable(radii, depth)
        return color, radii, depth

    @staticmethod
    def backward(ctx, grad_color, _grad_radii, _grad_depth):
        a, st = ctx.a, ctx.st
        if st.P == 0:
            z = lambda t: None if t is None else torch.zeros_like(t)
            return (z(a["means3D"]), None, z(a["shs"]), z(a["colors_precomp"]), z(a["opacities"]), z(a["scales"]),
                    z(a["rotations"]), z(a["cov3D_precomp"]), None)
        g = rasterize_backward(ctx.rs, st, grad_color, a["means3D"], a["shs"], a["colors_precomp"], a["scales"],
                               a["rotations"], a["cov3D_precomp"])
        return (g["means3D"], g["means2D"], g["shs"], g["colors_precomp"], g["opacities"], g["scales"],
                g["rotations"], g["cov3D_precomp"], None)


class GaussianRasterizer(torch.nn.Module):
    def __init__(self, raster_settings: GaussianRasterizationSettings):
        super().__init__()
        self.raster_settings = raster_settings

    def markVisible(self, positions: torch.Tensor) -> torch.Tensor:
        L = _lib.lib()
        rs = self.raster_settings
        p = _dev_f32(positions, "positions")
        out = torch.zeros(p.shape[0], dtype=torch.uint8, device=p.device)
        fr = _Frame(rs)
        stream = C.c_void_p(torch.cuda.current_stream(p.device).cuda_stream)
        with torch.cuda.device(p.device):
            _lib.check(L.mvi_raster_mark_visible(p.shape[0], _ptr(p), _ptr(fr.keep[1]), _ptr(fr.keep[2]), _ptr(out), stream),
                       "mark_visible")
        return out.bool()

    def forward_raw(self, xyz, means2D, features_dc, features_rest, raw_opacity, raw_scaling, raw_rotation):
        return _RasterizeRaw.apply(xyz, means2D, features_dc, features_rest, raw_opacity, raw_scaling, raw_rotation,
                                   self.raster_settings)

    def forward(self, means3D, means2D, opacities, shs=None, colors_precomp=None, scales=None, rotations=None,
                cov3D_precomp=None):
        if (shs is None) == (colors_precomp is None):
            raise Exception("Please provide excatly one of either SHs or precomputed colors!")
        if ((scales is None or rotations is None) and cov3D_precomp is None) or \
                ((scales is not None or rotations is not None) and cov3D_precomp is not None):
            raise Exception("Please provide exactly one of either scale/rotation pair or precomputed 3D covariance!")
        empty = torch.empty(0, dtype=torch.float32, device=means3D.device)
        return _Rasterize.apply(means3D, means2D,
                                empty if shs is None else shs, empty if colors_precomp is None else colors_precomp,
                                opacities, empty if scales is None else scales, empty if rotations is None else rotations,
                                empty if cov3D_precomp is None else cov3D_precomp, self.raster_settings)
```

Measured before the change: 2359 Mpix/s.

## Recompute 3D covariance in backward and fuse touched-list compaction into sparse kernel

Forward preprocess no longer stores cov3D, depths, or tiles_touched (when bin_v2 is set). Backward recomputes the covariance from scale and rotation, and a new on-demand kernel materializes those buffers only when a caller asks for them. The separate compact_touched kernel, with its global atomic list and count, is replaced by per-block compaction inside the sparse backward kernel using a wave scan over 16-byte flag words. The aim is to cut global memory writes and reads plus one kernel launch, at the cost of extra ALU work in backward and more complex view-accessor semantics.

```diff
diff --git a/include/mvi_raster.h b/include/mvi_raster.h
--- a/include/mvi_raster.h
+++ b/include/mvi_raster.h
@@ -121,6 +121,9 @@
 int mvi_raster_get_views(int32_t P, int64_t num_rendered, int32_t image_width, int32_t image_height,
                          const void* geom, const void* binning, const void* image,
                          mvi_raster_views* out);
+int mvi_raster_materialize_geom_views(const mvi_raster_settings* s, int32_t P, const float* means3D, const float* scales,
+                                      const float* rotations, const float* cov3D_precomp, const int32_t* radii, void* geom,
+                                      void* stream);
 int mvi_raster_materialize_tile_ids(int32_t P, int64_t num_rendered, int32_t image_width, int32_t image_height,
                                     void* binning, const void* image, void* stream);
 
diff --git a/multiview_inpaint_amd/_lib.py b/multiview_inpaint_amd/_lib.py
--- a/multiview_inpaint_amd/_lib.py
+++ b/multiview_inpaint_amd/_lib.py
@@ -107,6 +107,8 @@
     L.mvi_raster_mark_visible.argtypes = [i32, vp, vp, vp, vp, vp]
     L.mvi_raster_get_views.restype = C.c_int
     L.mvi_raster_get_views.argtypes = [i32, i64, i32, i32, vp, vp, vp, C.POINTER(RasterViews)]
+    L.mvi_raster_materialize_geom_views.restype = C.c_int
+    L.mvi_raster_materialize_geom_views.argtypes = [C.POINTER(RasterSettings), i32] + [vp] * 7
     L.mvi_raster_materialize_tile_ids.restype = C.c_int
     L.mvi_raster_materialize_tile_ids.argtypes = [i32, i64, i32, i32, vp, vp, vp]
     L.mvi_raster_timing_enable.restype = C.c_int
diff --git a/multiview_inpaint_amd/csrc/raster_api.hip b/multiview_inpaint_amd/csrc/raster_api.hip
--- a/multiview_inpaint_amd/csrc/raster_api.hip
+++ b/multiview_inpaint_amd/csrc/raster_api.hip
@@ -416,7 +416,6 @@
         mvi::ZeroRegions z;
         z.add(grad_rows, (size_t)mvi::kGradRow * (size_t)P);
         z.add(g.touched, ((size_t)P + 15) / 16 * 4);
-        z.add(g.touched_count, 1);
         if (mvi::launch_zero_regions(z, st)) return hip_fail("zero grad rows", hipGetLastError());
     }
     {
@@ -446,8 +445,8 @@
                                     void* stream) {
     mvi::Frame f;
     if (int rc = make_frame(s, P, M, f)) return rc;
-    if (first < 0 || count < 0 || (int64_t)first + count > P || (first % 64) != 0)
-        return fail(MVI_EINVAL, "backward range out of bounds or not 64-aligned%s: first %lld count %lld", "", (long long)first, (long long)count);
+    if (first < 0 || count < 0 || (int64_t)first + count > P)
+        return fail(MVI_EINVAL, "backward range out of bounds%s: first %lld count %lld", "", (long long)first, (long long)count);
     if (P == 0 || count == 0) return MVI_OK;
     if ((shs == nullptr) == (colors_precomp == nullptr))
         return fail(MVI_EINVAL, "Please provide excatly one of either SHs or precomputed colors!%s");
@@ -462,8 +461,7 @@
         return fail(MVI_EINVAL, "missing covariance gradient output%s");
     mvi::GeomView g = mvi::carve_geom(const_cast<void*>(geom), P);
     const size_t o = (size_t)first;
-    g.depths += o; g.xy += o; g.cov_a += o; g.cov_b += o; g.conic_opacity += o; g.rgbd += o; g.tiles_touched += o; g.rect += o;
-    g.clamped += o;
+    g.xy += o; g.conic_opacity += o; g.rgbd += o; g.rect += o; g.clamped += o;
     auto at = [o](auto* p, size_t w) { return p ? p + o * w : p; };
     f.P = count;
     hipStream_t st = (hipStream_t)stream;
@@ -545,6 +543,21 @@
     return MVI_OK;
 }
 
+int mvi_raster_materialize_geom_views(const mvi_raster_settings* s, int32_t P, const float* means3D, const float* scales,
+                                      const float* rotations, const float* cov3D_precomp, const int32_t* radii, void* geom,
+                                      void* stream) {
+    mvi::Frame f;
+    if (int rc = make_frame(s, P, 0, f)) return rc;
+    if (P == 0) return MVI_OK;
+    if (!means3D || !radii || !geom) return fail(MVI_EINVAL, "NULL means3D/radii/geom in materialize_geom_views%s");
+    if (((scales == nullptr) || (rotations == nullptr)) == (cov3D_precomp == nullptr))
+        return fail(MVI_EINVAL, "Please provide exactly one of either scale/rotation pair or precomputed 3D covariance!%s");
+    mvi::GeomView g = mvi::carve_geom(geom, P);
+    if (mvi::launch_materialize_geom_views(f, means3D, scales, rotations, cov3D_precomp, radii, g, (hipStream_t)stream))
+        return hip_fail("materialize_geom_views", hipGetLastError());
+    return MVI_OK;
+}
+
 int mvi_raster_materialize_tile_ids(int32_t P, int64_t D, int32_t W, int32_t H, void* binning, const void* image, void* stream) {
     if (P < 0 || D < 0 || W < 0 || H < 0) return fail(MVI_EINVAL, "negative size in materialize_tile_ids%s");
     if (P == 0 || D == 0) return MVI_OK;
diff --git a/multiview_inpaint_amd/csrc/raster_common.h b/multiview_inpaint_amd/csrc/raster_common.h
--- a/multiview_inpaint_amd/csrc/raster_common.h
+++ b/multiview_inpaint_amd/csrc/raster_common.h
@@ -80,8 +80,6 @@
     uint8_t* clamped;
     uint8_t* front;
     struct ColorSource* color_src;
-    uint32_t* touched_list;
-    uint32_t* touched_count;
     uint8_t* touched;
     uint32_t* block_sums;
     uint32_t* block_offsets;
@@ -144,8 +142,7 @@
     g.rect = (uint2*)take(8 * n);
     g.clamped = (uint8_t*)take(n);
     g.touched = (uint8_t*)take(n);
-    g.touched_list = (uint32_t*)take(4 * n);
-    g.touched_count = (uint32_t*)take(4);
+    take(4 * n); take(4);
     g.front = (uint8_t*)take(n);
     g.color_src = (ColorSource*)take(sizeof(ColorSource));
     const size_t npre = (n + kPB - 1) / kPB;
@@ -507,6 +504,8 @@
 int launch_render_forward(const Frame& f, GeomView g, BinningView b, ImageView im, int64_t D,
                           float* out_color, float* out_depth, hipStream_t st, float* zero_rows = nullptr);
 int launch_resolve_colors(const Frame& f, GeomView g, hipStream_t st);
+int launch_materialize_geom_views(const Frame& f, const float* means3D, const float* scales, const float* rotations,
+                                  const float* cov3D_precomp, const int32_t* radii, GeomView g, hipStream_t st);
 int launch_render_backward(const Frame& f, GeomView g, BinningView b, ImageView im, int64_t D,
                            const float* dL_dpix, float* grad_rows, hipStream_t st, const ZeroRegions* zero = nullptr);
 int launch_wave_sum9_probe(const float* in, float* out, int n_waves, hipStream_t st);
diff --git a/multiview_inpaint_amd/csrc/raster_preprocess.hip b/multiview_inpaint_amd/csrc/raster_preprocess.hip
--- a/multiview_inpaint_amd/csrc/raster_preprocess.hip
+++ b/multiview_inpaint_amd/csrc/raster_preprocess.hip
@@ -1,5 +1,9 @@
 #include "raster_common.h"
 #include "raster_scan.h"
+
+#ifndef MVI_SPARSE_FLAGS
+#define MVI_SPARSE_FLAGS 1024
+#endif
 
 namespace mvi {
 
@@ -96,6 +100,32 @@
     R[2][0] = 2.0f * __builtin_fmaf(x, z, -(r * y));
     R[2][1] = 2.0f * __builtin_fmaf(y, z, r * x);
     R[2][2] = __builtin_fmaf(-2.0f, __builtin_fmaf(x, x, y * y), 1.0f);
+}
+
+__device__ __forceinline__ float quat_normalize(float4& q) {
+#pragma clang fp contract(off)
+    const float nq = fmaxf(sqrtf(q.x * q.x + q.y * q.y + q.z * q.z + q.w * q.w), 1e-12f);
+    q = make_float4(q.x / nq, q.y / nq, q.z / nq, q.w / nq);
+    return nq;
+}
+
+__device__ __forceinline__ void cov3d_from_scale_rot(const Frame& f, float4 q, const float* scale_in, float* c6) {
+#pragma clang fp contract(off)
+    float R[3][3], Mx[3][3];
+    quat_to_rot(q.x, q.y, q.z, q.w, R);
+    float sa[3] = {scale_in[0], scale_in[1], scale_in[2]};
+    if (f.raw) { sa[0] = expf(sa[0]); sa[1] = expf(sa[1]); sa[2] = expf(sa[2]); }
+    float s[3] = {f.scale_modifier * sa[0], f.scale_modifier * sa[1], f.scale_modifier * sa[2]};
+#pragma unroll
+    for (int r = 0; r < 3; ++r)
+#pragma unroll
+        for (int j = 0; j < 3; ++j) Mx[r][j] = R[r][j] * s[j];
+    c6[0] = dot3(Mx[0][0], Mx[0][1], Mx[0][2], Mx[0][0], Mx[0][1], Mx[0][2]);
+    c6[1] = dot3(Mx[0][0], Mx[0][1], Mx[0][2], Mx[1][0], Mx[1][1], Mx[1][2]);
+    c6[2] = dot3(Mx[0][0], Mx[0][1], Mx[0][2], Mx[2][0], Mx[2][1], Mx[2][2]);
+    c6[3] = dot3(Mx[1][0], Mx[1][1], Mx[1][2], Mx[1][0], Mx[1][1], Mx[1][2]);
+    c6[4] = dot3(Mx[1][0], Mx[1][1], Mx[1][2], Mx[2][0], Mx[2][1], Mx[2][2]);
+    c6[5] = dot3(Mx[2][0], Mx[2][1], Mx[2][2], Mx[2][0], Mx[2][1], Mx[2][2]);
 }
 
 struct Ewa {
@@ -168,8 +198,7 @@
         if (!cov3D_precomp) q = *reinterpret_cast<const float4*>(rotations + 4 * (size_t)i);
         opac = opacities[i];
         if (f.raw) {
-            const float nq = fmaxf(sqrtf(q.x * q.x + q.y * q.y + q.z * q.z + q.w * q.w), 1e-12f);
-            q = make_float4(q.x / nq, q.y / nq, q.z / nq, q.w / nq);
+            quat_normalize(q);
             opac = sigmoidf_(opac);
         }
     }
@@ -200,24 +229,8 @@
 #pragma unroll
                 for (int k = 0; k < 6; ++k) c6[k] = cov3D_precomp[6 * (size_t)i + k];
             } else {
-                float R[3][3], Mx[3][3];
-                quat_to_rot(q.x, q.y, q.z, q.w, R);
-                float sa[3] = {s_scale[3 * tid], s_scale[3 * tid + 1], s_scale[3 * tid + 2]};
-                if (f.raw) { sa[0] = expf(sa[0]); sa[1] = expf(sa[1]); sa[2] = expf(sa[2]); }
-                float s[3] = {f.scale_modifier * sa[0], f.scale_modifier * sa[1], f.scale_modifier * sa[2]};
-#pragma unroll
-                for (int r = 0; r < 3; ++r)
-#pragma unroll
-                    for (int j = 0; j < 3; ++j) Mx[r][j] = R[r][j] * s[j];
-                c6[0] = dot3(Mx[0][0], Mx[0][1], Mx[0][2], Mx[0][0], Mx[0][1], Mx[0][2]);
-                c6[1] = dot3(Mx[0][0], Mx[0][1], Mx[0][2], Mx[1][0], Mx[1][1], Mx[1][2]);
-                c6[2] = dot3(Mx[0][0], Mx[0][1], Mx[0][2], Mx[2][0], Mx[2][1], Mx[2][2]);
-                c6[3] = dot3(Mx[1][0], Mx[1][1], Mx[1][2], Mx[1][0], Mx[1][1], Mx[1][2]);
-                c6[4] = dot3(Mx[1][0], Mx[1][1], Mx[1][2], Mx[2][0], Mx[2][1], Mx[2][2]);
-                c6[5] = dot3(Mx[2][0], Mx[2][1], Mx[2][2], Mx[2][0], Mx[2][1], Mx[2][2]);
-            }
-            g.cov_a[i] = make_float4(c6[0], c6[1], c6[2], c6[3]);
-            g.cov_b[i] = make_float2(c6[4], c6[5]);
+                cov3d_from_scale_rot(f, q, s_scale + 3 * tid, c6);
+            }
 
             Ewa e;
             ewa_setup(f, V, vx, vy, vz, e);
@@ -249,7 +262,6 @@
             }
             g.clamped[i] = (uint8_t)clamp_bits;
             g.rgbd[i] = make_float4(r0, r1, r2, vz);
-            g.depths[i] = vz;
             depth_key = vz;
             g.xy[i] = make_float2(pix_x, pix_y);
             g.conic_opacity[i] = make_float4(c * det_inv, -b * det_inv, a * det_inv, opac);
@@ -259,7 +271,7 @@
         } while (false);
         radii[i] = rad_out;
         if (defer_colors) g.front[i] = 0;
-        g.tiles_touched[i] = touched;
+        if (!f.bin_v2) g.tiles_touched[i] = touched;
         g.rect[i] = rect;
         g.dkeys[0][i] = touched ? __float_as_uint(depth_key) : 0xFFFFFFFFu;
         if (!f.bin_v2) g.dvals[0][i] = (uint32_t)i;
@@ -322,14 +334,13 @@
 }
 
 __device__ __forceinline__ void backward_cov_and_mean(const Frame& f, float px, float py, float pz, const float* gr,
-                                                  float4 ca, float2 cb, float* dm, float* g6) {
+                                                  const float* c6, float* dm, float* g6) {
     float V[16], PM[16];
 #pragma unroll
     for (int k = 0; k < 16; ++k) { V[k] = f.view[k]; PM[k] = f.proj[k]; }
     float vx = affine3(V[0], V[4], V[8], V[12], px, py, pz);
     float vy = affine3(V[1], V[5], V[9], V[13], px, py, pz);
     float vz = affine3(V[2], V[6], V[10], V[14], px, py, pz);
-    float c6[6] = {ca.x, ca.y, ca.z, ca.w, cb.x, cb.y};
     Ewa e;
     ewa_setup(f, V, vx, vy, vz, e);
     float a, b, c;
@@ -387,14 +398,8 @@
 
 }
 
-__device__ __forceinline__ void backward_scale_rot(const Frame& f, const float* g6, float4 qrot, const float* sa_in, float* ds,
+__device__ __forceinline__ void backward_scale_rot(const Frame& f, const float* g6, float4 q, float nq, const float* sa_in, float* ds,
                                                    float* dq) {
-    float4 q = qrot;
-    float nq = 1.0f;
-    if (f.raw) {
-        nq = fmaxf(sqrtf(q.x * q.x + q.y * q.y + q.z * q.z + q.w * q.w), 1e-12f);
-        q = make_float4(q.x / nq, q.y / nq, q.z / nq, q.w / nq);
-    }
     float R[3][3];
     quat_to_rot(q.x, q.y, q.z, q.w, R);
     float sa[3] = {sa_in[0], sa_in[1], sa_in[2]};
@@ -458,19 +463,23 @@
     const float raw_o = (f.raw && in_range) ? rawx.raw_opacity[i] : 0.0f;
     const bool live = in_range && radii[i] > 0;
     float gr[9] = {0, 0, 0, 0, 0, 0, 0, 0, 0};
-    float4 ca = make_float4(0.f, 0.f, 0.f, 0.f), qrot = make_float4(1.f, 0.f, 0.f, 0.f);
-    float2 cb = make_float2(0.f, 0.f);
+    float4 qrot = make_float4(1.f, 0.f, 0.f, 0.f);
+    float c6[6] = {0, 0, 0, 0, 0, 0};
     uint32_t cl_bits = 0;
     if (live) {
         const float4* row = reinterpret_cast<const float4*>(grad_rows + (size_t)i * kGradRow);
         float4 a = row[0], b4 = row[1];
         gr[0] = a.x; gr[1] = a.y; gr[2] = a.z; gr[3] = a.w; gr[4] = b4.x; gr[5] = b4.y; gr[6] = b4.z; gr[7] = b4.w;
         gr[8] = grad_rows[(size_t)i * kGradRow + 8];
-        ca = g.cov_a[i];
-        cb = g.cov_b[i];
-        if (!cov3D_precomp) qrot = *reinterpret_cast<const float4*>(rotations + 4 * (size_t)i);
+        if (cov3D_precomp) {
+#pragma unroll
+            for (int k = 0; k < 6; ++k) c6[k] = cov3D_precomp[6 * (size_t)i + k];
+        } else {
+            qrot = *reinterpret_cast<const float4*>(rotations + 4 * (size_t)i);
+        }
         if (shs) cl_bits = g.clamped[i];
     }
+    const float nq = (f.raw && live) ? quat_normalize(qrot) : 1.0f;
     __syncthreads();
     s_dm2d[3 * tid] = gr[0]; s_dm2d[3 * tid + 1] = gr[1]; s_dm2d[3 * tid + 2] = 0.0f;
     if (in_range) {
@@ -489,7 +498,8 @@
     const int nb = (f.deg + 1) * (f.deg + 1);
     if (live) {
         const float px = s_mean[3 * tid], py = s_mean[3 * tid + 1], pz = s_mean[3 * tid + 2];
-        backward_cov_and_mean(f, px, py, pz, gr, ca, cb, dm, g6);
+        if (!cov3D_precomp) cov3d_from_scale_rot(f, qrot, s_scale + 3 * tid, c6);
+        backward_cov_and_mean(f, px, py, pz, gr, c6, dm, g6);
 
         if (shs) {
             float ox = px - f.campos[0], oy = py - f.campos[1], oz = pz - f.campos[2];
@@ -533,7 +543,7 @@
         float ds[3] = {0, 0, 0}, dq[4] = {0, 0, 0, 0};
         if (live) {
             const float sa_in[3] = {s_scale[3 * tid], s_scale[3 * tid + 1], s_scale[3 * tid + 2]};
-            backward_scale_rot(f, g6, qrot, sa_in, ds, dq);
+            backward_scale_rot(f, g6, qrot, nq, sa_in, ds, dq);
         }
         s_dscale[3 * tid] = ds[0]; s_dscale[3 * tid + 1] = ds[1]; s_dscale[3 * tid + 2] = ds[2];
         if (in_range) *reinterpret_cast<float4*>(dL_drots + 4 * (size_t)i) = make_float4(dq[0], dq[1], dq[2], dq[3]);
@@ -553,6 +563,8 @@
 }
 
 constexpr int kSparseBlock = 64;
+constexpr int kSparseFlags = MVI_SPARSE_FLAGS;
+template <int FLAGS>
 __global__ __launch_bounds__(kSparseBlock) void preprocess_backward_sparse_kernel(
     Frame f, const float* __restrict__ means3D, const float* __restrict__ shs, const float* __restrict__ scales,
     const float* __restrict__ rotations, const float* __restrict__ cov3D_precomp, GeomView g,
@@ -560,9 +572,33 @@
     float* __restrict__ dL_dopacity, float* __restrict__ dL_dcolors, float* __restrict__ dL_dshs,
     float* __restrict__ dL_dcov3D, float* __restrict__ dL_dscales, float* __restrict__ dL_drots, RawBackwardExtra rawx,
     int vec_ok) {
-    const uint32_t n_touched = *g.touched_count;
-    for (uint32_t slot = blockIdx.x * (uint32_t)kSparseBlock + threadIdx.x; slot < n_touched; slot += gridDim.x * (uint32_t)kSparseBlock) {
-    const int i = (int)g.touched_list[slot];
+    static_assert(FLAGS % 1024 == 0 && FLAGS <= 4096, "16-byte flag words per lane, one 64-bit mask per lane");
+    constexpr int kPer = FLAGS / kSparseBlock, kVec = kPer / 16;
+    __shared__ uint32_t s_list[FLAGS];
+    const int lane = threadIdx.x;
+    const int first = blockIdx.x * FLAGS + lane * kPer;
+    uint4 w[kVec];
+#pragma unroll
+    for (int v = 0; v < kVec; ++v)
+        w[v] = first + 16 * v < f.P ? *reinterpret_cast<const uint4*>(g.touched + first + 16 * v) : make_uint4(0u, 0u, 0u, 0u);
+    unsigned long long mask = 0ull;
+#pragma unroll
+    for (int v = 0; v < kVec; ++v) {
+        const uint32_t ww[4] = {w[v].x, w[v].y, w[v].z, w[v].w};
+#pragma unroll
+        for (int q = 0; q < 4; ++q)
+#pragma unroll
+            for (int k = 0; k < 4; ++k)
+                if (((ww[q] >> (8 * k)) & 0xFFu) && first + 16 * v + 4 * q + k < f.P) mask |= 1ull << (16 * v + 4 * q + k);
+    }
+    const uint32_t mine = (uint32_t)__popcll(mask);
+    const uint32_t incl = wave_incl_scan(mine, lane);
+    const uint32_t n_touched = (uint32_t)__shfl((int)incl, 63);
+    if (n_touched == 0) return;
+    for (uint32_t dst = incl - mine; mask; mask &= mask - 1ull) s_list[dst++] = (uint32_t)(first + __builtin_ctzll(mask));
+    __syncthreads();
+    for (uint32_t slot = lane; slot < n_touched; slot += kSparseBlock) {
+    const int i = (int)s_list[slot];
     const size_t si = (size_t)i;
     float gr[9];
     {
@@ -571,10 +607,24 @@
         gr[0] = a.x; gr[1] = a.y; gr[2] = a.z; gr[3] = a.w; gr[4] = b4.x; gr[5] = b4.y; gr[6] = b4.z; gr[7] = b4.w;
         gr[8] = grad_rows[si * kGradRow + 8];
     }
-    const float4 ca = g.cov_a[i];
-    const float2 cb = g.cov_b[i];
+    float c6[6];
+    float4 qrot = make_float4(1.f, 0.f, 0.f, 0.f);
+    float sa_in[3] = {0.f, 0.f, 0.f};
+    if (cov3D_precomp) {
+#pragma unroll
+        for (int k = 0; k < 6; ++k) c6[k] = cov3D_precomp[6 * si + k];
+    } else {
+        qrot = (vec_ok & 2) ? *reinterpret_cast<const float4*>(rotations + 4 * si)
+                            : make_float4(rotations[4 * si], rotations[4 * si + 1], rotations[4 * si + 2], rotations[4 * si + 3]);
+        sa_in[0] = scales[3 * si]; sa_in[1] = scales[3 * si + 1]; sa_in[2] = scales[3 * si + 2];
+    }
     const uint32_t cl = shs ? g.clamped[i] : 0u;
     const float px = means3D[3 * si], py = means3D[3 * si + 1], pz = means3D[3 * si + 2];
+    float nq = 1.0f;
+    if (!cov3D_precomp) {
+        if (f.raw) nq = quat_normalize(qrot);
+        cov3d_from_scale_rot(f, qrot, sa_in, c6);
+    }
     dL_dmeans2D[3 * si] = gr[0];
     dL_dmeans2D[3 * si + 1] = gr[1];
     {
@@ -589,7 +639,7 @@
     }
     float dm[3] = {0, 0, 0};
     float g6[6] = {0, 0, 0, 0, 0, 0};
-    backward_cov_and_mean(f, px, py, pz, gr, ca, cb, dm, g6);
+    backward_cov_and_mean(f, px, py, pz, gr, c6, dm, g6);
     if (shs) {
         const int M = f.M, nb = (f.deg + 1) * (f.deg + 1);
         float ox = px - f.campos[0], oy = py - f.campos[1], oz = pz - f.campos[2];
@@ -688,42 +738,12 @@
 #pragma unroll
         for (int k = 0; k < 6; ++k) dL_dcov3D[6 * si + k] = g6[k];
     } else {
-        const float4 qrot = (vec_ok & 2) ? *reinterpret_cast<const float4*>(rotations + 4 * si)
-                                         : make_float4(rotations[4 * si], rotations[4 * si + 1], rotations[4 * si + 2], rotations[4 * si + 3]);
-        const float sa_in[3] = {scales[3 * si], scales[3 * si + 1], scales[3 * si + 2]};
         float ds[3] = {0, 0, 0}, dq[4] = {0, 0, 0, 0};
-        backward_scale_rot(f, g6, qrot, sa_in, ds, dq);
+        backward_scale_rot(f, g6, qrot, nq, sa_in, ds, dq);
         dL_dscales[3 * si] = ds[0]; dL_dscales[3 * si + 1] = ds[1]; dL_dscales[3 * si + 2] = ds[2];
         dL_drots[4 * si] = dq[0]; dL_drots[4 * si + 1] = dq[1]; dL_drots[4 * si + 2] = dq[2]; dL_drots[4 * si + 3] = dq[3];
     }
     }
-}
-
-constexpr int kCompactThreads = 1024, kCompactPer = 16;
-__global__ __launch_bounds__(kCompactThreads) void compact_touched_kernel(int P, const uint8_t* __restrict__ touched,
-                                                                         uint32_t* __restrict__ list, uint32_t* __restrict__ count) {
-    __shared__ uint32_t s_wave[kCompactThreads / 64];
-    __shared__ uint32_t s_base;
-    const int tid = threadIdx.x;
-    const int i0 = (blockIdx.x * kCompactThreads + tid) * kCompactPer;
-    uint4 w = make_uint4(0u, 0u, 0u, 0u);
-    if (i0 < P) w = *reinterpret_cast<const uint4*>(touched + i0);
-    const uint32_t ww[4] = {w.x, w.y, w.z, w.w};
-    uint32_t mine = 0;
-#pragma unroll
-    for (int q = 0; q < 4; ++q)
-        mine += ((ww[q] & 0xFFu) != 0) + ((ww[q] & 0xFF00u) != 0) + ((ww[q] & 0xFF0000u) != 0) + ((ww[q] >> 24) != 0);
-    uint32_t total;
-    const uint32_t off = block_excl_scan<kCompactThreads / 64>(mine, tid, s_wave, &total);
-    if (total == 0) return;
-    if (tid == 0) s_base = atomicAdd(count, total);
-    __syncthreads();
-    uint32_t dst = s_base + off;
-#pragma unroll
-    for (int q = 0; q < 4; ++q)
-#pragma unroll
-        for (int k = 0; k < 4; ++k)
-            if (((ww[q] >> (8 * k)) & 0xFFu) && i0 + 4 * q + k < P) list[dst++] = (uint32_t)(i0 + 4 * q + k);
 }
 
 int launch_preprocess_backward_sparse(const Frame& f, const float* means3D, const float* shs, const float* scales,
@@ -732,13 +752,10 @@
                                       float* dL_dshs, float* dL_dcov3D, float* dL_dscales, float* dL_drots, hipStream_t st,
                                       RawBackwardExtra rawx) {
     if (f.P <= 0) return 0;
-    constexpr int kPerBlock = kCompactThreads * kCompactPer;
-    hipLaunchKernelGGL(compact_touched_kernel, dim3((f.P + kPerBlock - 1) / kPerBlock), dim3(kCompactThreads), 0, st, f.P, g.touched,
-                       g.touched_list, g.touched_count);
-    const int sparse_blocks = min((f.P + kSparseBlock - 1) / kSparseBlock, 2048);
+    const int sparse_blocks = (f.P + kSparseFlags - 1) / kSparseFlags;
     auto al16 = [](const void* p) { return ((uintptr_t)p & 15u) == 0; };
     const int vec_ok = ((al16(shs) && al16(dL_dshs)) ? 1 : 0) | (al16(rotations) ? 2 : 0);
-    hipLaunchKernelGGL(preprocess_backward_sparse_kernel, dim3(sparse_blocks), dim3(kSparseBlock), 0, st, f, means3D, shs, scales,
+    hipLaunchKernelGGL(preprocess_backward_sparse_kernel<kSparseFlags>, dim3(sparse_blocks), dim3(kSparseBlock), 0, st, f, means3D, shs, scales,
                        rotations, cov3D_precomp, g, grad_rows, dL_dmeans3D, dL_dmeans2D, dL_dopacity, dL_dcolors, dL_dshs,
                        dL_dcov3D, dL_dscales, dL_drots, rawx, vec_ok);
     return hipGetLastError() == hipSuccess ? 0 : MVI_EHIP;
@@ -837,7 +854,9 @@
     const ColorSource cs = *g.color_src;
     if (!cs.deferred) return;
     const int i = blockIdx.x * 256 + threadIdx.x;
-    if (i >= f.P || g.tiles_touched[i] == 0) return;
+    if (i >= f.P) return;
+    const uint32_t wh = g.rect[i].y;
+    if ((wh & 0xFFFFu) * (wh >> 16) == 0) return;
     const float4 cd = g.rgbd[i];
     if (color_pending(cd)) resolve_color(cs, f.campos, (uint32_t)i, cd.w, g.rgbd, g.clamped);
 }
@@ -847,6 +866,42 @@
     return hipGetLastError() == hipSuccess ? 0 : MVI_EHIP;
 }
 
+__global__ __launch_bounds__(256) void materialize_geom_views_kernel(Frame f, const float* __restrict__ means3D,
+                                                                     const float* __restrict__ scales,
+                                                                     const float* __restrict__ rotations,
+                                                                     const float* __restrict__ cov3D_precomp,
+                                                                     const int32_t* __restrict__ radii, GeomView g) {
+#pragma clang fp contract(off)
+    const int i = blockIdx.x * 256 + threadIdx.x;
+    if (i >= f.P) return;
+    const size_t si = (size_t)i;
+    f.raw = g.color_src->raw;
+    const uint32_t wh = g.rect[i].y;
+    g.tiles_touched[i] = (wh & 0xFFFFu) * (wh >> 16);
+    if (radii[i] > 0) g.depths[i] = g.rgbd[i].w;
+    const float vz = affine3(f.view[2], f.view[6], f.view[10], f.view[14], means3D[3 * si], means3D[3 * si + 1], means3D[3 * si + 2]);
+    if (vz <= kNearZ) return;
+    float c6[6];
+    if (cov3D_precomp) {
+#pragma unroll
+        for (int k = 0; k < 6; ++k) c6[k] = cov3D_precomp[6 * si + k];
+    } else {
+        float4 q = make_float4(rotations[4 * si], rotations[4 * si + 1], rotations[4 * si + 2], rotations[4 * si + 3]);
+        if (f.raw) quat_normalize(q);
+        const float sa_in[3] = {scales[3 * si], scales[3 * si + 1], scales[3 * si + 2]};
+        cov3d_from_scale_rot(f, q, sa_in, c6);
+    }
+    g.cov_a[i] = make_float4(c6[0], c6[1], c6[2], c6[3]);
+    g.cov_b[i] = make_float2(c6[4], c6[5]);
+}
+int launch_materialize_geom_views(const Frame& f, const float* means3D, const float* scales, const float* rotations,
+                                  const float* cov3D_precomp, const int32_t* radii, GeomView g, hipStream_t st) {
+    if (f.P <= 0) return 0;
+    hipLaunchKernelGGL(materialize_geom_views_kernel, dim3((f.P + 255) / 256), dim3(256), 0, st, f, means3D, scales, rotations,
+                       cov3D_precomp, radii, g);
+    return hipGetLastError() == hipSuccess ? 0 : MVI_EHIP;
+}
+
 int launch_color_factors(int P, const int32_t* radii, const float* grad_rows, const uint8_t* clamped, float* out, hipStream_t st) {
     if (P <= 0) return 0;
     hipLaunchKernelGGL(color_factor_kernel, dim3((P + 255) / 256), dim3(256), 0, st, P, radii, grad_rows, clamped, out);
diff --git a/multiview_inpaint_amd/csrc/raster_render.hip b/multiview_inpaint_amd/csrc/raster_render.hip
--- a/multiview_inpaint_amd/csrc/raster_render.hip
+++ b/multiview_inpaint_amd/csrc/raster_render.hip
@@ -202,7 +202,6 @@
     if (zero_rows) {
         z.add(zero_rows, (size_t)f.P * kGradRow);
         z.add(g.touched, ((size_t)f.P + 15) / 16 * 4);
-        z.add(g.touched_count, 1);
     }
     if (f.W <= 0 || f.H <= 0) return launch_zero_regions(z, st);
     const uint32_t* plist = b.vals[b.passes & 1];
diff --git a/multiview_inpaint_amd/raster/__init__.py b/multiview_inpaint_amd/raster/__init__.py
--- a/multiview_inpaint_amd/raster/__init__.py
+++ b/multiview_inpaint_amd/raster/__init__.py
@@ -46,7 +46,20 @@
 
 
 class RasterState:
-    __slots__ = ("P", "M", "D", "W", "H", "geom", "binning", "image", "radii", "grad_rows", "rows_clean", "frame", "sources")
+    __slots__ = ("P", "M", "D", "W", "H", "geom", "binning", "image", "radii", "grad_rows", "rows_clean", "frame", "sources",
+                 "cov_sources")
+    ON_DEMAND_GEOM_VIEWS = ("depths", "cov3D_a", "cov3D_b", "tiles_touched")
+
+    def materialize_geom_views(self):
+        if self.P == 0:
+            return
+        dev = self.geom.device
+        scales, rotations, cov3D_precomp = self.cov_sources
+        with torch.cuda.device(dev):
+            _lib.check(_lib.lib().mvi_raster_materialize_geom_views(
+                C.byref(self.frame.c), self.P, _ptr(self.sources[0]), _ptr(scales), _ptr(rotations), _ptr(cov3D_precomp),
+                _ptr(self.radii), _ptr(self.geom), C.c_void_p(torch.cuda.current_stream(dev).cuda_stream)),
+                "materialize_geom_views")
 
     def resolve_colors(self):
         if self.P == 0:
@@ -73,6 +86,8 @@
     def tensor(self, name, shape, dtype, _derive=True):
         v = self.views()
         addr = getattr(v, name)
+        if _derive and name in self.ON_DEMAND_GEOM_VIEWS:
+            self.materialize_geom_views()
         if _derive and name == "tile_ids_sorted" and self.D > 0 and self.binning is not None and self.image is not None:
             dev = self.binning.device
             with torch.cuda.device(dev):
@@ -125,6 +140,7 @@
     st = RasterState()
     st.P, st.M, st.W, st.H = P, M, W, H
     st.frame, st.sources = fr, (means3D, shs)
+    st.cov_sources = (scales, rotations, cov3D_precomp)
     u8 = dict(dtype=torch.uint8, device=dev)
     st.geom = torch.empty(L.mvi_raster_geom_bytes(P), **u8)
     st.image = torch.empty(L.mvi_raster_image_bytes(W, H), **u8)
@@ -299,6 +315,7 @@
     st = RasterState()
     st.P, st.M, st.W, st.H = P, M, W, H
     st.frame, st.sources = fr, (xyz, features_dc, features_rest)
+    st.cov_sources = (raw_scaling, raw_rotation, None)
     u8 = dict(dtype=torch.uint8, device=dev)
     st.geom = torch.empty(L.mvi_raster_geom_bytes(P), **u8)
     st.image = torch.empty(L.mvi_raster_image_bytes(W, H), **u8)
```

Result: faster. 2410 Mpix/s, median of 6 (+2.2%).
